# LiuZhu-CV/PAIF

Hardware: AMD Instinct MI355X
Metric: fused image-pairs/sec at 480x640 bs=8 per GPU (fusion-net forward) (higher is better)
Workload: dtype f16 (IEEE fp16 maps and conv weights, one fp16 MFMA per product, f32 accumulate; stems, guided filter and the last map fp32)

## Files before the change

### include/paif_hip.h

```cpp
#ifndef PAIF_HIP_H
#define PAIF_HIP_H

#include <stddef.h>
#include <stdint.h>

#ifdef __cplusplus
extern "C" {
#endif

#define PAIF_ABI_VERSION 1
#define PAIF_EINVAL (-1)
#define PAIF_ENOSUP (-2)

typedef void* paif_stream_t;

int paif_version(void);
const char* paif_last_error(void);
int paif_device_cus(void);


int paif_rgb2ycrcb_fwd(const float* rgb, float* ycc, int B, int H, int W, paif_stream_t stream);

int paif_ycrcb2rgb_fwd(const float* ycc, float* rgb, int B, int H, int W, paif_stream_t stream);

int paif_minmax_blocks(int B, int H, int W);
int paif_recompose_clamp_fwd(const float* fused, const float* ycc, float* rgb_out, float* minmax_partial,
                             int B, int H, int W, paif_stream_t stream);
int paif_fused_uint8_fwd(const float* rgb, const float* minmax_partial, int npartial, unsigned char* out, int B, int H, int W,
                         paif_stream_t stream);
int paif_minmax_normalize_fwd(const float* rgb, const float* minmax_partial, int npartial, float* out,
                              float* minmax_out, int B, int H, int W, paif_stream_t stream);


int paif_stem_fwd(const float* img, size_t img_bstride, const float* w, const float* prelu, float* feat, float* guide,
                  int B, int H, int W, paif_stream_t stream);
int paif_stem_fwd_twin(const float* img, size_t img_bstride, const float* w, const float* prelu, float* feat, float* feat_bf16,
                       float* guide, int B, int H, int W, paif_stream_t stream);
int paif_stem_fwd_twin_f16(const float* img, size_t img_bstride, const float* w, const float* prelu, float* feat, float* feat_f16,
                           float* guide, int B, int H, int W, paif_stream_t stream);
int paif_channel_residue_fwd(const float* x, float* guide, int B, int H, int W, paif_stream_t stream);

int paif_guided_filter_ab_fwd(const float* guide, const float* y, float* ab, float eps0, float eps1,
                              int B, int H, int W, paif_stream_t stream);
int paif_guided_filter_lf_fwd(const float* guide, const float* ab, float* lf, int B, int H, int W,
                              paif_stream_t stream);
int paif_guided_filter_taped_fits(int B, int H, int W);
int paif_guided_filter_taped_fwd(const float* guide, const float* y, float* mc, float* lf, float eps0, float eps1,
                                 float* workspace, int B, int H, int W, paif_stream_t stream);
size_t paif_guided_filter_fused_workspace_floats(int B, int H, int W);
int paif_guided_filter_fused_fwd(const float* guide, const float* y, float* lf, float eps0, float eps1, float* workspace,
                                 int B, int H, int W, paif_stream_t stream);
int paif_guided_filter_fused_fwd_bf16(const float* guide, const float* y, float* lf, float eps0, float eps1, float* workspace, int B,
                                      int H, int W, paif_stream_t stream);
int paif_guided_filter_fused_fwd_hf16(const float* guide, const float* y, float* hf, float eps0, float eps1, float* workspace, int B,
                                      int H, int W, paif_stream_t stream);

int paif_guided_filter_fused_fwd_hf16_y16(const float* guide, const float* y16, float* hf, float eps0, float eps1, float* workspace,
                                          int B, int H, int W, paif_stream_t stream);

typedef struct {
  const float* src[3];
  int nsrc;
  int cin;
  const float* wpk;
  int kh;
  int dil;
  int in_act;
  const float* in_prelu;
  const float* scale;
  const float* shift;
  int act;
  const float* prelu;
  float alpha;
  const float* res[3];
  float* out;
  int cout;
  float* pool_partial;
  int precision;
  float* aux_out;
  const float* in_aux;
  const float* in_scale;
  float in_alpha;
  const float* epi_aux;
  int epi_dact;
  int reverse_tiles;
  int storage;
  float* cpool;
} paif_conv_desc;
#define PAIF_ST_F32 0
#define PAIF_ST_BF16 1
#define PAIF_ST_F32_BF16 2
#define PAIF_ST_F16 3
#define PAIF_ST_F16_F32 4
#define PAIF_CONV_F32 0
#define PAIF_CONV_BF16X3 1
#define PAIF_CONV_BF16 2
#define PAIF_CONV_F16 4
#define PAIF_CONV_F16X2 5
#define PAIF_CONV_F16X3 6
#define PAIF_CONV_BF16X6 3

int paif_dwconv_fwd_bf16(const float* x, const float* w, float* out, int k, int dil, int in_relu, int B, int H, int W,
                         paif_stream_t stream);
int paif_channel_pool2_fwd_bf16(const float* ir, const float* vis, float* comp, int B, int H, int W, paif_stream_t stream);
int paif_spa_blend_fwd_bf16(const float* comp, const float* w, const float* ir, const float* vis, float* agg, int B, int H, int W,
                            paif_stream_t stream);
int paif_eca_finish_fwd_bf16(const float* o, const float* r, const float* pool_partial, const float* w1d, int k,
                             const float* prelu, float* gate, float* out, int B, int H, int W, paif_stream_t stream);
int paif_tail_fwd_bf16(const float* x, const float* w, const float* prelu, float* fused, int B, int H, int W, paif_stream_t stream);
int paif_add_fwd_bf16(const float* a, const float* b, float* out, size_t n, paif_stream_t stream);
int paif_cast_storage_fwd(const float* src, float* dst, size_t n, int mode, paif_stream_t stream);
int paif_dwconv_fwd_f16(const float* x, const float* w, float* out, int k, int dil, int in_relu, int B, int H, int W,
                        paif_stream_t stream);
int paif_channel_pool2_fwd_f16(const float* ir, const float* vis, float* comp, int B, int H, int W, paif_stream_t stream);
int paif_spa_blend_fwd_f16(const float* comp, const float* w, const float* ir, const float* vis, float* agg, int B, int H, int W,
                           paif_stream_t stream);
int paif_eca_finish_fwd_f16(const float* o, const float* r, const float* pool_partial, const float* w1d, int k,
                            const float* prelu, float* gate, float* out, int B, int H, int W, paif_stream_t stream);
int paif_tail_fwd_f16(const float* x, const float* w, const float* prelu, float* fused, int B, int H, int W, paif_stream_t stream);
int paif_add_fwd_f16(const float* a, const float* b, float* out, size_t n, paif_stream_t stream);

int paif_conv2d_blocks(int B, int H, int W);
int paif_conv2d_fwd(const paif_conv_desc* d, int B, int H, int W, paif_stream_t stream);
int paif_conv2d_can_cpool(const paif_conv_desc* d, int B, int H, int W);
int paif_channel_pool1_fwd(const float* x, float* comp_off, int B, int H, int W, paif_stream_t stream);
int paif_channel_pool1_fwd_bf16(const float* x, float* comp_off, int B, int H, int W, paif_stream_t stream);
int paif_channel_pool1_fwd_f16(const float* x, float* comp_off, int B, int H, int W, paif_stream_t stream);
int paif_conv2d_is_persistent(const paif_conv_desc* d, int B, int H, int W);
int paif_conv2d_kernel_name(const paif_conv_desc* d, int B, int H, int W, char* buf, int buflen);
size_t paif_conv_wpk_floats(int nsrc, int cin, int kh);
int paif_pack_conv_weight(const float* w, float* wpk, int cout, int nsrc, int cin, int kh, paif_stream_t stream);
int paif_pack_conv_weight_bf16x3(const float* w, float* wpk, int cout, int nsrc, int kh, paif_stream_t stream);
int paif_pack_conv_weight_f16x2(const float* w, float* wpk, int cout, int nsrc, int kh, paif_stream_t stream);
int paif_pack_conv_weight_bf16x6(const float* w, float* wpk, int cout, int nsrc, int kh, paif_stream_t stream);
int paif_compose_dw_pw_weight(const float* dw, const float* pw, float* out, int cout, int cin, int kh, paif_stream_t stream);
int paif_compose_pw_conv_weight(const float* pw, const float* w, float* out, int cout, int cmid, int cin, int kh, paif_stream_t stream);

size_t paif_rdb_fused_wpk_floats(void);
int paif_rdb_fused_pack(const float* w1, const float* w2, const float* w3, float* wpk, int f16, paif_stream_t stream);
int paif_rdb_fused_fwd(const float* x, const float* wpk, const float* prelu, float alpha, const float* res0, const float* res1, float* out,
                       float* cpool, int f16, int reverse_tiles, int B, int H, int W, paif_stream_t stream);

int paif_stem_out_pack_floats(void);
int paif_stem_out_pack(const float* w1, const float* w2, float* wpk, paif_stream_t stream);
int paif_stem_out_fwd_bf16(const float* x, const float* wpk, const float* prelu, float* fused, int B, int H, int W, paif_stream_t stream);
int paif_stem_out_fwd_f32(const float* x, const float* wpk, const float* prelu, float* fused, int B, int H, int W, paif_stream_t stream);
int paif_stem_out_fwd_guard(const float* x, int f32in, const float* wpk, const float* prelu, float* fused, unsigned* flag, int B, int H, int W,
                            paif_stream_t stream);
int paif_pack_decomp1x1_weight_bf16x6(const float* w, float* wpk, paif_stream_t stream);
int paif_pack_decomp1x1_weight_bf16x3(const float* w, float* wpk, paif_stream_t stream);
int paif_pack_decomp1x1_hf_weight_f16x2(const float* w, float* wpk, paif_stream_t stream);
int paif_pack_decomp1x1_weight(const float* w, float* wpk, paif_stream_t stream);
int paif_bn_fold(const float* gamma, const float* beta, const float* mean, const float* var, float eps,
                 float* scale, float* shift, int C, paif_stream_t stream);

int paif_dwconv_fwd(const float* x, const float* w, float* out, int k, int dil, int in_relu,
                    int B, int H, int W, paif_stream_t stream);

int paif_channel_pool2_fwd(const float* ir, const float* vis, float* comp, int B, int H, int W, paif_stream_t stream);
int paif_spa_blend_fwd(const float* comp, const float* w, const float* ir, const float* vis, float* agg,
                       float* scale_out, int B, int H, int W, paif_stream_t stream);

int paif_eca_finish_fwd(const float* o, const float* r, const float* pool_partial, const float* w1d, int k,
                        const float* prelu, float* gate , float* out,
                        float* u_out ,
                        int B, int H, int W, paif_stream_t stream);

int paif_tail_fwd(const float* x, const float* w, const float* prelu, float* fused,
                  float* z_out ,
                  int B, int H, int W, paif_stream_t stream);

int paif_add_fwd(const float* a, const float* b, float* out, size_t n, paif_stream_t stream);



int paif_gemm_fwd(const float* A, int lda, const float* W, const float* scale, const float* shift, int act,
                  const float* res, int ldres, float* C, int ldc, int M, int N, int K, int precision,
                  paif_stream_t stream);
int paif_gemm_splitk_plan(int M, int N, int K);
int paif_gemm_splitk_fwd(const float* A, int lda, const float* W, const float* scale, const float* shift, int act,
                         const float* res, int ldres, float* C, int ldc, int M, int N, int K, int splits,
                         float* workspace, paif_stream_t stream);
int paif_gemm_splitk_fwd_p(const float* A, int lda, const float* W, const float* scale, const float* shift, int act,
                         const float* res, int ldres, float* C, int ldc, int M, int N, int K, int splits,
                         float* workspace, int precision, paif_stream_t stream);

int paif_gemm_conv_fwd(const float* x, int B, int H, int W, int Cin, int k, int stride, int pad, const float* Wt,
                       const float* scale, const float* shift, int act, const float* res, int ldres, float* out, int ldc,
                       int N, int precision, int splits, float* workspace, paif_stream_t stream);

int paif_gemm_col2im_fwd(const float* dY, int lda, const float* Wt, float* dx, int B, int H, int W, int C, int sr, int K,
                         int precision, paif_stream_t stream);

int paif_timing_event_create(void** ev);
int paif_timing_event_record(void* ev, paif_stream_t stream);
int paif_timing_event_elapsed_ms(void* start, void* stop, float* ms);
int paif_timing_event_destroy(void* ev);

int paif_gemm2_plan(int M, int N, int K, int precision);
size_t paif_gemm2_packed_bytes(int N, int K, int precision);
int paif_gemm2_pack_weight(const float* W, void* out, int N, int K, int precision, paif_stream_t stream);
int paif_gemm2_fwd(const float* A, int lda, const void* W, const float* scale, const float* shift, int act,
                   const float* res, int ldres, float* C, int ldc, int M, int N, int K, int precision, int nt,
                   paif_stream_t stream);

int paif_layernorm_fwd(const float* x, const float* gamma, const float* beta, float* y, int M, int C, float eps,
                       paif_stream_t stream);

int paif_im2col_fwd(const float* x, float* col, int B, int H, int W, int Cin, int k, int stride, int pad, int Kpad,
                    paif_stream_t stream);
int paif_pack_conv_gemm_weight(const float* w, float* out, int Cout, int Cin, int k, int Kpad, paif_stream_t stream);

int paif_dwconv3_bias_gelu_fwd(const float* x, const float* w, const float* bias, float* y, int B, int H, int W, int C,
                               paif_stream_t stream);

int paif_sr_attention_fwd(const float* q, const float* kv, float* out, float* lse, int B, int N, int Nk, int C, int heads,
                          paif_stream_t stream);
int paif_sr_attention_split_fwd(const float* q, const float* kv, float* out, float* lse, int B, int N, int Nk, int C, int heads,
                                int precision, paif_stream_t stream);
int paif_sr_attention_bf16x3_fwd(const float* q, const float* kv, float* out, float* lse, int B, int N, int Nk, int C, int heads,
                          paif_stream_t stream);

int paif_resize_bilinear_into_fwd(const float* x, float* out, int B, int IH, int IW, int C, int OH, int OW, int ldo,
                                  int coff, paif_stream_t stream);

int paif_nhwc_to_nchw_fwd(const float* x, float* y, int B, int HW, int C, paif_stream_t stream);
int paif_nchw_to_nhwc_fwd(const float* x, float* y, int B, int HW, int C, paif_stream_t stream);
int paif_nchw_to_nhwc_pad_fwd(const float* x, float* y, int B, int HW, int C, int CP, paif_stream_t stream);


int paif_gemm_masked_fwd(const float* A, int lda, const float* a_mask, const float* a_scale, const float* W,
                         const float* scale, const float* shift, int act, const float* res, int ldres, float* C,
                         int ldc, int M, int N, int K, int precision, paif_stream_t stream);
int paif_transpose_pad_fwd(const float* w, float* wt, int N, int K, int Npad, paif_stream_t stream);

int paif_layernorm_bwd_input(const float* x, const float* gamma, const float* dy, const float* add, float* dx,
                             int M, int C, float eps, paif_stream_t stream);
int paif_dwconv3_bias_gelu_bwd_input(const float* x, const float* w, const float* bias, const float* dy, float* tmp,
                                     float* dx, int B, int H, int W, int C, paif_stream_t stream);
int paif_col2im_fwd(const float* dcol, float* dx, int B, int H, int W, int Cin, int k, int stride, int pad, int Kpad,
                    paif_stream_t stream);
int paif_resize_bilinear_adjoint_fwd(const float* dout, float* dx, int B, int IH, int IW, int C, int OH, int OW,
                                     int ldo, int coff, paif_stream_t stream);
int paif_sr_attention_bwd_chunks(int B, int N, int heads);
int paif_sr_attention_bwd_input(const float* q, const float* kv, const float* o, const float* dout, const float* lse,
                                float* delta, float* dq, float* dkv, float* dkv_partial, int B, int N, int Nk, int C,
                                int heads, paif_stream_t stream);
int paif_sr_attention_bwd_input_p(const float* q, const float* kv, const float* o, const float* dout, const float* lse,
                                float* delta, float* dq, float* dkv, float* dkv_partial, int B, int N, int Nk, int C,
                                int heads, int precision, paif_stream_t stream);

int paif_upsample_ce_blocks(int B, int OH, int OW);
int paif_upsample_ce_fwd(const float* logits, const long long* label, float* partial, float* loss_count, int B, int IH,
                         int IW, int C, int OH, int OW, int ignore_index, paif_stream_t stream);
int paif_upsample_ce_bwd(const float* logits, const long long* label, const float* gscale, float* dfull, int B, int IH,
                         int IW, int C, int OH, int OW, int ignore_index, int CP, paif_stream_t stream);

int paif_attack_loss_blocks(int B, int OH, int OW);
int paif_attack_loss_fwd(const float* logits, const long long* label, float* partial, float* coef, int way, float w_true,
                         float w_false, int B, int IH, int IW, int C, int OH, int OW, int ignore_index, paif_stream_t stream);
int paif_attack_loss_bwd(const float* logits, const long long* label, const float* coef, float* dfull, int way, float w_true,
                         float w_false, float upstream, int B, int IH, int IW, int C, int OH, int OW, int ignore_index, int CP,
                         paif_stream_t stream);

int paif_conv_weight_dgrad(const float* w, float* wt, int Co, int Ctot, int k, int coff, int cs, paif_stream_t stream);
int paif_fold_decomp1x1_weight(const float* w, float* wf, paif_stream_t stream);
int paif_tail_bwd_input(const float* dfused, const float* fused, const float* z, const float* w, const float* prelu,
                        float* dt16, int B, int H, int W, paif_stream_t stream);
int paif_stem_bwd_input(const float* dfeat, const float* feat, const float* w, const float* prelu, float* dimg,
                        int B, int H, int W, paif_stream_t stream);
int paif_dwconv_bwd_input(const float* dt, const float* w, const float* aux, const float* add, float* out, int k, int dil,
                          int B, int H, int W, paif_stream_t stream);
int paif_eca_bwd_blocks(int H, int W);
int paif_eca_bwd_input(const float* dout, const float* u, const float* o, const float* gate, const float* w1d, int k,
                       const float* prelu, float* partial, float* coef, float* d_o, float* d_r, int B, int H, int W,
                       paif_stream_t stream);
// ... 111 lines not shown
```

### paif_amd/_lib.py

```python
import ctypes
import os
from ctypes import POINTER, Structure, c_char_p, c_float, c_int, c_size_t, c_ulonglong, c_void_p

HERE = os.path.dirname(os.path.abspath(__file__))
LIB_PATH = os.environ.get("PAIF_LIB") or os.path.join(HERE, "lib", "libpaif_hip.so")

F = c_void_p


class ConvDesc(Structure):

    _fields_ = [
        ("src", F * 3), ("nsrc", c_int), ("cin", c_int), ("wpk", F), ("kh", c_int), ("dil", c_int),
        ("in_act", c_int), ("in_prelu", F), ("scale", F), ("shift", F), ("act", c_int), ("prelu", F),
        ("alpha", c_float), ("res", F * 3), ("out", F), ("cout", c_int), ("pool_partial", F),
        ("precision", c_int), ("aux_out", F), ("in_aux", F), ("in_scale", F), ("in_alpha", c_float), ("epi_aux", F),
        ("epi_dact", c_int), ("reverse_tiles", c_int), ("storage", c_int), ("cpool", F),
    ]


SIGNATURES = {
    "paif_version": (c_int, []),
    "paif_last_error": (c_char_p, []),
    "paif_device_cus": (c_int, []),
    "paif_rgb2ycrcb_fwd": (c_int, [F, F, c_int, c_int, c_int, F]),
    "paif_ycrcb2rgb_fwd": (c_int, [F, F, c_int, c_int, c_int, F]),
    "paif_minmax_blocks": (c_int, [c_int, c_int, c_int]),
    "paif_recompose_clamp_fwd": (c_int, [F, F, F, F, c_int, c_int, c_int, F]),
    "paif_fused_uint8_fwd": (c_int, [F, F, c_int, F, c_int, c_int, c_int, F]),
    "paif_minmax_normalize_fwd": (c_int, [F, F, c_int, F, F, c_int, c_int, c_int, F]),
    "paif_stem_fwd": (c_int, [F, c_size_t, F, F, F, F, c_int, c_int, c_int, F]),
    "paif_stem_fwd_twin": (c_int, [F, c_size_t, F, F, F, F, F, c_int, c_int, c_int, F]),
    "paif_stem_fwd_twin_f16": (c_int, [F, c_size_t, F, F, F, F, F, c_int, c_int, c_int, F]),
    "paif_channel_residue_fwd": (c_int, [F, F, c_int, c_int, c_int, F]),
    "paif_guided_filter_ab_fwd": (c_int, [F, F, F, c_float, c_float, c_int, c_int, c_int, F]),
    "paif_guided_filter_lf_fwd": (c_int, [F, F, F, c_int, c_int, c_int, F]),
    "paif_guided_filter_taped_fits": (c_int, [c_int, c_int, c_int]),
    "paif_guided_filter_taped_fwd": (c_int, [F, F, F, F, c_float, c_float, F, c_int, c_int, c_int, F]),
    "paif_guided_filter_fused_workspace_floats": (c_size_t, [c_int, c_int, c_int]),
    "paif_guided_filter_fused_fwd": (c_int, [F, F, F, c_float, c_float, F, c_int, c_int, c_int, F]),
    "paif_guided_filter_fused_fwd_bf16": (c_int, [F, F, F, c_float, c_float, F, c_int, c_int, c_int, F]),
    "paif_guided_filter_fused_fwd_hf16": (c_int, [F, F, F, c_float, c_float, F, c_int, c_int, c_int, F]),
    "paif_guided_filter_fused_fwd_hf16_y16": (c_int, [F, F, F, c_float, c_float, F, c_int, c_int, c_int, F]),
    "paif_conv2d_blocks": (c_int, [c_int, c_int, c_int]),
    "paif_conv2d_fwd": (c_int, [POINTER(ConvDesc), c_int, c_int, c_int, F]),
    "paif_conv2d_is_persistent": (c_int, [POINTER(ConvDesc), c_int, c_int, c_int]),
    "paif_conv2d_can_cpool": (c_int, [POINTER(ConvDesc), c_int, c_int, c_int]),
    "paif_rdb_fused_wpk_floats": (c_size_t, []),
    "paif_rdb_fused_pack": (c_int, [F, F, F, F, c_int, F]),
    "paif_rdb_fused_fwd": (c_int, [F, F, F, c_float, F, F, F, F, c_int, c_int, c_int, c_int, c_int, F]),
    "paif_channel_pool1_fwd": (c_int, [F, F, c_int, c_int, c_int, F]),
    "paif_channel_pool1_fwd_bf16": (c_int, [F, F, c_int, c_int, c_int, F]),
    "paif_channel_pool1_fwd_f16": (c_int, [F, F, c_int, c_int, c_int, F]),
    "paif_conv2d_kernel_name": (c_int, [POINTER(ConvDesc), c_int, c_int, c_int, c_char_p, c_int]),
    "paif_conv_wpk_floats": (c_size_t, [c_int, c_int, c_int]),
    "paif_pack_conv_weight": (c_int, [F, F, c_int, c_int, c_int, c_int, F]),
    "paif_pack_decomp1x1_weight": (c_int, [F, F, F]),
    "paif_pack_conv_weight_bf16x3": (c_int, [F, F, c_int, c_int, c_int, F]),
    "paif_pack_conv_weight_f16x2": (c_int, [F, F, c_int, c_int, c_int, F]),
    "paif_pack_conv_weight_bf16x6": (c_int, [F, F, c_int, c_int, c_int, F]),
    "paif_compose_dw_pw_weight": (c_int, [F, F, F, c_int, c_int, c_int, F]),
    "paif_compose_pw_conv_weight": (c_int, [F, F, F, c_int, c_int, c_int, c_int, F]),
    "paif_stem_out_pack_floats": (c_int, []),
    "paif_stem_out_pack": (c_int, [F, F, F, F]),
    "paif_stem_out_fwd_bf16": (c_int, [F, F, F, F, c_int, c_int, c_int, F]),
    "paif_stem_out_fwd_f32": (c_int, [F, F, F, F, c_int, c_int, c_int, F]),
    "paif_stem_out_fwd_guard": (c_int, [F, c_int, F, F, F, F, c_int, c_int, c_int, F]),
    "paif_pack_decomp1x1_weight_bf16x3": (c_int, [F, F, F]),
    "paif_pack_decomp1x1_hf_weight_f16x2": (c_int, [F, F, F]),
    "paif_pack_decomp1x1_weight_bf16x6": (c_int, [F, F, F]),
    "paif_bn_fold": (c_int, [F, F, F, F, c_float, F, F, c_int, F]),
    "paif_dwconv_fwd": (c_int, [F, F, F, c_int, c_int, c_int, c_int, c_int, c_int, F]),
    "paif_channel_pool2_fwd": (c_int, [F, F, F, c_int, c_int, c_int, F]),
    "paif_spa_blend_fwd": (c_int, [F, F, F, F, F, F, c_int, c_int, c_int, F]),
    "paif_eca_finish_fwd": (c_int, [F, F, F, F, c_int, F, F, F, F, c_int, c_int, c_int, F]),
    "paif_tail_fwd": (c_int, [F, F, F, F, F, c_int, c_int, c_int, F]),
    "paif_add_fwd": (c_int, [F, F, F, c_size_t, F]),
    "paif_gemm_fwd": (c_int, [F, c_int, F, F, F, c_int, F, c_int, F, c_int, c_int, c_int, c_int, c_int, F]),
    "paif_gemm_splitk_plan": (c_int, [c_int, c_int, c_int]),
    "paif_gemm_conv_fwd": (c_int, [F, c_int, c_int, c_int, c_int, c_int, c_int, c_int, F, F, F, c_int, F, c_int, F, c_int, c_int, c_int, c_int, F, F]),
    "paif_gemm_col2im_fwd": (c_int, [F, c_int, F, F, c_int, c_int, c_int, c_int, c_int, c_int, c_int, F]),
    "paif_timing_event_create": (c_int, [POINTER(c_void_p)]),
    "paif_timing_event_record": (c_int, [c_void_p, F]),
    "paif_timing_event_elapsed_ms": (c_int, [c_void_p, c_void_p, POINTER(c_float)]),
    "paif_timing_event_destroy": (c_int, [c_void_p]),
    "paif_gemm2_plan": (c_int, [c_int, c_int, c_int, c_int]),
    "paif_gemm2_packed_bytes": (c_size_t, [c_int, c_int, c_int]),
    "paif_gemm2_pack_weight": (c_int, [F, F, c_int, c_int, c_int, F]),
    "paif_gemm2_fwd": (c_int, [F, c_int, F, F, F, c_int, F, c_int, F, c_int, c_int, c_int, c_int, c_int, c_int, F]),
    "paif_conv2d_wgrad_workspace_floats": (c_size_t, [c_int, c_int, c_int, c_int]),
    "paif_conv2d_wgrad": (c_int, [POINTER(c_void_p), c_int, F, F, F, F, c_int, c_float, c_int, c_int, F, F, c_int, c_int, c_int, c_int, c_int, F]),
    "paif_gemm_wgrad_splits": (c_int, [c_int, c_int, c_int]),
    "paif_gemm_wgrad": (c_int, [F, c_int, F, c_int, F, F, c_int, c_int, c_int, c_int, F, c_int, F]),
    "paif_gemm_wgrad_p": (c_int, [F, c_int, F, c_int, F, F, c_int, c_int, c_int, c_int, F, c_int, c_int, c_float, F]),
    "paif_layernorm_wgrad_blocks": (c_int, [c_int]),
    "paif_layernorm_wgrad": (c_int, [F, F, F, F, F, c_int, c_int, c_float, c_int, F]),
    "paif_channel_affine_nchw_fwd": (c_int, [F, F, F, F, c_int, c_int, c_int, c_int, F]),
    "paif_image_loss_blocks": (c_int, []),
    "paif_image_loss_fwd": (c_int, [F, F, c_int, c_int, c_int, c_int, c_int, c_int, F, F, F]),
    "paif_image_loss_bwd": (c_int, [F, F, c_int, c_int, c_int, c_int, c_int, c_int, c_float, F, F]),
    "paif_ssim_l1_blocks": (c_int, [c_int, c_int, c_int]),
    "paif_ssim_l1_fwd": (c_int, [F, F, F, F, F, c_int, c_int, c_int, F]),
    "paif_ssim_l1_bwd_input": (c_int, [F, F, F, F, F, F, c_int, c_int, c_int, F]),
    "paif_gemm_splitk_fwd": (c_int, [F, c_int, F, F, F, c_int, F, c_int, F, c_int, c_int, c_int, c_int, c_int, F, F]),
    "paif_gemm_splitk_fwd_p": (c_int, [F, c_int, F, F, F, c_int, F, c_int, F, c_int, c_int, c_int, c_int, c_int, F, c_int, F]),
    "paif_layernorm_fwd": (c_int, [F, F, F, F, c_int, c_int, c_float, F]),
    "paif_im2col_fwd": (c_int, [F, F, c_int, c_int, c_int, c_int, c_int, c_int, c_int, c_int, F]),
    "paif_pack_conv_gemm_weight": (c_int, [F, F, c_int, c_int, c_int, c_int, F]),
    "paif_dwconv3_bias_gelu_fwd": (c_int, [F, F, F, F, c_int, c_int, c_int, c_int, F]),
    "paif_sr_attention_fwd": (c_int, [F, F, F, F, c_int, c_int, c_int, c_int, c_int, F]),
    "paif_sr_attention_bf16x3_fwd": (c_int, [F, F, F, F, c_int, c_int, c_int, c_int, c_int, F]),
    "paif_sr_attention_split_fwd": (c_int, [F, F, F, F, c_int, c_int, c_int, c_int, c_int, c_int, F]),
    "paif_resize_bilinear_into_fwd": (c_int, [F, F, c_int, c_int, c_int, c_int, c_int, c_int, c_int, c_int, F]),
    "paif_nhwc_to_nchw_fwd": (c_int, [F, F, c_int, c_int, c_int, F]),
    "paif_nchw_to_nhwc_fwd": (c_int, [F, F, c_int, c_int, c_int, F]),
    "paif_nchw_to_nhwc_pad_fwd": (c_int, [F, F, c_int, c_int, c_int, c_int, F]),
    "paif_gemm_masked_fwd": (c_int, [F, c_int, F, F, F, F, F, c_int, F, c_int, F, c_int, c_int, c_int, c_int, c_int, F]),
    "paif_transpose_pad_fwd": (c_int, [F, F, c_int, c_int, c_int, F]),
    "paif_layernorm_bwd_input": (c_int, [F, F, F, F, F, c_int, c_int, c_float, F]),
    "paif_dwconv3_bias_gelu_bwd_input": (c_int, [F, F, F, F, F, F, c_int, c_int, c_int, c_int, F]),
    "paif_col2im_fwd": (c_int, [F, F, c_int, c_int, c_int, c_int, c_int, c_int, c_int, c_int, F]),
    "paif_resize_bilinear_adjoint_fwd": (c_int, [F, F, c_int, c_int, c_int, c_int, c_int, c_int, c_int, c_int, F]),
    "paif_sr_attention_bwd_chunks": (c_int, [c_int, c_int, c_int]),
    "paif_sr_attention_bwd_input": (c_int, [F, F, F, F, F, F, F, F, F, c_int, c_int, c_int, c_int, c_int, F]),
    "paif_sr_attention_bwd_input_p": (c_int, [F, F, F, F, F, F, F, F, F, c_int, c_int, c_int, c_int, c_int, c_int, F]),
    "paif_upsample_ce_blocks": (c_int, [c_int, c_int, c_int]),
    "paif_upsample_ce_fwd": (c_int, [F, F, F, F, c_int, c_int, c_int, c_int, c_int, c_int, c_int, F]),
    "paif_dwconv_fwd_bf16": (c_int, [F, F, F, c_int, c_int, c_int, c_int, c_int, c_int, F]),
    "paif_channel_pool2_fwd_bf16": (c_int, [F, F, F, c_int, c_int, c_int, F]),
    "paif_spa_blend_fwd_bf16": (c_int, [F, F, F, F, F, c_int, c_int, c_int, F]),
    "paif_eca_finish_fwd_bf16": (c_int, [F, F, F, F, c_int, F, F, F, c_int, c_int, c_int, F]),
    "paif_tail_fwd_bf16": (c_int, [F, F, F, F, c_int, c_int, c_int, F]),
    "paif_add_fwd_bf16": (c_int, [F, F, F, c_size_t, F]),
    "paif_dwconv_fwd_f16": (c_int, [F, F, F, c_int, c_int, c_int, c_int, c_int, c_int, F]),
    "paif_channel_pool2_fwd_f16": (c_int, [F, F, F, c_int, c_int, c_int, F]),
    "paif_spa_blend_fwd_f16": (c_int, [F, F, F, F, F, c_int, c_int, c_int, F]),
    "paif_eca_finish_fwd_f16": (c_int, [F, F, F, F, c_int, F, F, F, c_int, c_int, c_int, F]),
    "paif_tail_fwd_f16": (c_int, [F, F, F, F, c_int, c_int, c_int, F]),
    "paif_add_fwd_f16": (c_int, [F, F, F, c_size_t, F]),
    "paif_cast_storage_fwd": (c_int, [F, F, c_size_t, c_int, F]),
    "paif_attack_loss_blocks": (c_int, [c_int, c_int, c_int]),
    "paif_attack_loss_fwd": (c_int, [F, F, F, F, c_int, c_float, c_float, c_int, c_int, c_int, c_int, c_int, c_int, c_int, F]),
    "paif_attack_loss_bwd": (c_int, [F, F, F, F, c_int, c_float, c_float, c_float, c_int, c_int, c_int, c_int, c_int, c_int, c_int, c_int, F]),
    "paif_conv_weight_dgrad": (c_int, [F, F, c_int, c_int, c_int, c_int, c_int, F]),
    "paif_fold_decomp1x1_weight": (c_int, [F, F, F]),
    "paif_tail_bwd_input": (c_int, [F, F, F, F, F, F, c_int, c_int, c_int, F]),
    "paif_stem_bwd_input": (c_int, [F, F, F, F, F, c_int, c_int, c_int, F]),
    "paif_dwconv_bwd_input": (c_int, [F, F, F, F, F, c_int, c_int, c_int, c_int, c_int, F]),
    "paif_eca_bwd_blocks": (c_int, [c_int, c_int]),
    "paif_eca_bwd_input": (c_int, [F, F, F, F, F, c_int, F, F, F, F, F, c_int, c_int, c_int, F]),
    "paif_spa_blend_bwd_input": (c_int, [F, F, F, F, F, F, F, F, F, F, c_int, c_int, c_int, F]),
    "paif_guided_filter_bwd_input": (c_int, [F, F, F, F, c_float, c_float, F, F, F, F, F, F, c_int, c_int, c_int, F]),
    "paif_guided_filter_bwd_input_mc": (c_int, [F, F, F, F, F, F, F, F, F, F, c_int, c_int, c_int, F]),
    "paif_upsample_argmax_fwd": (c_int, [F, F, c_int, c_int, c_int, c_int, c_int, c_int, F]),
    "paif_confusion_matrix_accum": (c_int, [F, F, F, c_size_t, c_int, F]),
    "paif_spa1_fwd": (c_int, [F, F, F, c_int, F, F, F, F, F, c_int, c_int, c_int, F]),
    "paif_spa1_bwd_input": (c_int, [F, F, F, F, F, c_int, F, F, F, F, c_int, c_int, c_int, F]),
    "paif_glue_bwd_blocks": (c_int, [c_int, c_int, c_int]),
    "paif_glue_bwd_input": (c_int, [F, F, F, F, F, F, F, F, c_int, c_int, c_int, F]),
    "paif_plane_minmax_blocks": (c_int, [c_size_t]),
    "paif_plane_clamp_minmax_fwd": (c_int, [F, F, F, F, c_size_t, F]),
    "paif_plane_clamp_minmax_bwd_input": (c_int, [F, F, F, F, F, c_size_t, F]),
    "paif_channel_sum_chunks_fwd": (c_int, [F, F, c_int, c_int, c_int, c_int, F]),
    "paif_rgb2ycrcb_bwd_input": (c_int, [F, F, F, c_int, c_int, c_int, F]),
    "paif_pgd_step": (c_int, [F, F, F, c_float, c_float, c_size_t, F]),
    "paif_axpy": (c_int, [F, F, c_float, c_size_t, F]),
    "paif_upsample_ce_bwd": (c_int, [F, F, F, F, c_int, c_int, c_int, c_int, c_int, c_int, c_int, c_int, F]),
    "paif_head_sum_fwd": (c_int, [F, F, F, F, POINTER(c_int), F, F, F, c_int, c_int, F]),
    "paif_relu_mask_scale_fwd": (c_int, [F, F, F, F, c_size_t, c_int, F]),
    "paif_u8_to_planes_fwd": (c_int, [F, F, c_int, c_int, c_int, F]),
    "paif_u8_to_i64_fwd": (c_int, [F, F, c_size_t, F]),
    "paif_nhwc_slice_to_nchw_fwd": (c_int, [F, F, c_int, c_int, c_int, c_int, F]),
    "paif_pad_channels_fwd": (c_int, [F, F, c_size_t, c_int, c_int, F]),
    "paif_decomp_cat_fwd": (c_int, [F, F, F, F, c_size_t, F]),
    "paif_row_reduce_workspace_floats": (c_size_t, [c_int, c_int, c_int]),
    "paif_bn_stats_fwd": (c_int, [F, c_int, c_int, F, F, c_float, c_float, F, F, F, F, F, F, F, F]),
    "paif_affine_act_res_fwd": (c_int, [F, F, F, c_int, F, F, F, F, F, c_size_t, c_int, F]),
    "paif_bn_act_bwd": (c_int, [F, F, F, F, F, F, c_int, F, F, F, F, F, F, F, c_int, c_int, c_int, F]),
    "paif_bn_eval_stats": (c_int, [F, F, F, F, c_float, c_int, F, F, F, F, F]),
    "paif_prelu_bwd": (c_int, [F, F, F, F, c_float, F, F, F, c_size_t, F]),
    "paif_tail_dz": (c_int, [F, F, F, F, F, F, F, c_size_t, F]),
    "paif_colsum": (c_int, [F, c_int, F, F, c_int, c_int, F]),
    "paif_dwconv_wgrad": (c_int, [F, F, F, F, F, c_int, c_int, c_int, c_int, c_int, c_int, c_int, F]),
    "paif_stem_wgrad": (c_int, [F, c_size_t, F, F, F, F, F, F, c_int, c_int, c_int, F]),
    "paif_corr1_wgrad": (c_int, [F, F, F, F, c_int, c_int, c_int, c_int, c_int, F]),
    "paif_eca_wgrad": (c_int, [F, F, c_int, F, c_int, F, F, c_int, c_int, c_int, F]),
    "paif_unfold_decomp1x1_wgrad": (c_int, [F, F, F]),
    "paif_unpack_conv_gemm_wgrad": (c_int, [F, F, c_int, c_int, c_int, c_int, F]),
    "paif_keep_mask": (c_int, [F, c_int, c_ulonglong, c_ulonglong, c_float, F]),
    "paif_rowscale_add_fwd": (c_int, [F, F, F, F, c_int, c_size_t, c_int, c_int, F]),
    "paif_adamw_step": (c_int, [F, F, F, F, F, c_size_t, c_int, POINTER(c_float), POINTER(c_float), c_float, c_float, c_float, c_float,
                                c_float, F]),
}

_lib = None


class PaifLibraryError(RuntimeError):
# ... 29 lines not shown
```

### paif_amd/csrc/conv_dma.h

```cpp
#pragma once
#include <hip/hip_runtime.h>

namespace paif_conv_dma {

struct Args {
  const void* src[3];
  const void* res[3];
  const void* wpk;
  const float* scale;
  const float* shift;
  const float* prelu;
  void* out;
  float alpha;
  int nsrc, nres, act, kh;
  int cout;
  int B, H, W, reverse;
  float* cpool;
  int f16;
  int dil;
  int in_relu;
};

bool eligible(int nsrc, int nres, int B, int H, int W, float alpha);
bool eligible16(int nsrc, int nres, int B, int H, int W, float alpha);
bool eligible7(int nsrc, int nres, int B, int H, int W, float alpha);
bool eligible_d2(int nsrc, int nres, int B, int H, int W, float alpha);
bool can_cpool(int nsrc, int nres, int kh, int cout, int dil);
int launch(const Args& a, hipStream_t st);

}
```

### paif_amd/csrc/conv_dma.hip

```cpp
#include <stdint.h>
#include <stdlib.h>

#include <type_traits>

#include "conv_dma.h"
#include "paif_common.h"

namespace paif_conv_dma {
namespace {

typedef float f32x16 __attribute__((ext_vector_type(16)));
typedef unsigned u32x4 __attribute__((ext_vector_type(4)));
constexpr int TW = 32, TH = 8;
#ifndef CD_PF
#define CD_PF 4
#endif
#ifndef CD_ST_AUX
#define CD_ST_AUX 2
#endif
#ifndef CD_EXP
#define CD_EXP 0
#endif
constexpr int PARK_WAVE = 2 * 32 * 32 * 4;
template <int DIL>
struct Geo {
  static constexpr int TWH = TW + 2 * DIL, THH = TH + 2 * DIL;
  static constexpr int NPIX = TWH * THH;
  static constexpr int DPW = (NPIX * 4 + 255) / 256;
  static constexpr int SLOT = 4 * DPW * 1024;
  static constexpr int PF = DIL == 1 ? CD_PF : 3;
  static constexpr int NSLOT = PF + 1;
  static constexpr int ROWB = TWH * 64;
  static constexpr int PARK_OFF = NSLOT * SLOT;
  static constexpr int LDS_BYTES = PARK_OFF + 4 * PARK_WAVE;
  static_assert(LDS_BYTES <= 160 * 1024, "ring + transposition buffers exceed LDS");
  static_assert(4 * DPW * 64 >= NPIX * 4, "DMA instructions do not cover the halo tile");
  static __device__ __forceinline__ int base_row(int w) { return DIL == 1 ? 2 * w : (w >> 1) * 4 + (w & 1); }
};
constexpr unsigned RSRC_W3 = 0x00020000u;
constexpr unsigned OOB = 0x80000000u;
constexpr int NSTORE = 4;
constexpr int VMCAP = 63;

#define CD_VMWAIT(n) asm volatile("s_waitcnt vmcnt(%0)" ::"n"((n) > VMCAP ? VMCAP : (n)) : "memory")
#define CD_RD128(dst, addr, off) asm volatile("ds_read_b128 %0, %1 offset:%2" : "=v"(dst) : "v"(addr), "n"(off) : "memory")
#define CD_WR32(addr, val, off) asm volatile("ds_write_b32 %0, %1 offset:%2" ::"v"(addr), "v"(val), "n"(off) : "memory")

__device__ __forceinline__ void dma16(__amdgpu_buffer_rsrc_t rsrc, unsigned voff, unsigned lds_off) {
  __builtin_amdgcn_raw_ptr_buffer_load_lds(rsrc, (__attribute__((address_space(3))) void*)(uintptr_t)lds_off, 16, voff, 0, 0, 0);
}

template <int NSRC, int NRES, int PF, int DPW>
struct Sched {
  static constexpr int RL = 4 * NRES;
  static constexpr int smod(int x) { return ((x % NSRC) + NSRC) % NSRC; }
  static constexpr int R_STAGE = smod(1 - PF);
  static constexpr int D = (R_STAGE + PF - 1 - NSRC) / NSRC;
  static constexpr int U = D + (R_STAGE == 0 ? 2 : 1);
  static_assert(PF >= 2 && D >= 0 && U <= 4, "prefetch distance out of the range the tile loop lists");
  static constexpr int n1 = DPW * (PF - 1);
};

template <int NSRC, int NRES, int F, bool CP = false, int DIL = 1, int IA = 0>
__global__ __launch_bounds__(256, 1) void conv3x3_h16_dma(Args a, int ntiles, int tilesX, int tilesY) {
  typedef Geo<DIL> G;
  constexpr int TWH = G::TWH, NPIX = G::NPIX, DPW = G::DPW, SLOT = G::SLOT, PF = G::PF, NSLOT = G::NSLOT, ROWB = G::ROWB, PARK_OFF = G::PARK_OFF;
  typedef Sched<NSRC, NRES, PF, DPW> SC;
  constexpr int U = SC::U, D = SC::D;
  __shared__ __attribute__((aligned(16))) unsigned char smem[G::LDS_BYTES];
  asm volatile("" ::"v"((unsigned)(uintptr_t)(__attribute__((address_space(3))) unsigned char*)smem) : "memory");

  const int tid = threadIdx.x, l = tid & 63;
  const int w = __builtin_amdgcn_readfirstlane(tid >> 6);
  const int p = l & 31, hh = l >> 5;
  const int wb = G::base_row(w);

  const int xcd = blockIdx.x & 7, wg = blockIdx.x >> 3, nwg = gridDim.x >> 3;
  const int tpx = (ntiles + 7) >> 3;
  const int t_beg = xcd * tpx, t_end = min(ntiles, t_beg + tpx);
  const int cnt = t_beg + wg < t_end ? (t_end - t_beg - wg + nwg - 1) / nwg : 0;
  if (cnt == 0) return;
  const int H = a.H, W = a.W;
  auto pack_tile = [&](int k) -> unsigned {
    const int pos = wg + min(k, cnt - 1) * nwg;
    int t = a.reverse ? t_end - 1 - pos : t_beg + pos;
    const int tx = t % tilesX;
    t /= tilesX;
    const int ty = t % tilesY;
    return ((unsigned)(t / tilesY) << 22) | ((unsigned)ty << 11) | (unsigned)tx;
  };
  const unsigned tab0 = pack_tile(l), tab1 = pack_tile(l + 64);
  auto tile_of = [&](int k, int& b, int& y0, int& x0) -> bool {
    const bool ok = k >= 0 && k < cnt;
    const int kk = ok ? k : 0;
    const unsigned lo = __builtin_amdgcn_readlane(tab0, kk & 63), hi = __builtin_amdgcn_readlane(tab1, kk & 63);
    const unsigned pk = kk < 64 ? lo : hi;
    b = pk >> 22; y0 = ((pk >> 11) & 2047) * TH; x0 = (pk & 2047) * TW;
    return ok;
  };

  const int map_bytes = a.B * H * W * 64;
  __amdgpu_buffer_rsrc_t rs_src[NSRC];
#pragma unroll
  for (int s = 0; s < NSRC; ++s) rs_src[s] = __builtin_amdgcn_make_buffer_rsrc(const_cast<void*>(a.src[s]), 0, map_bytes, RSRC_W3);
  __amdgpu_buffer_rsrc_t rs_res[NRES > 0 ? NRES : 1];
#pragma unroll
  for (int r = 0; r < NRES; ++r) rs_res[r] = __builtin_amdgcn_make_buffer_rsrc(const_cast<void*>(a.res[r]), 0, map_bytes, RSRC_W3);
  const int opitch = a.cout * 2;
  const __amdgpu_buffer_rsrc_t rs_out = __builtin_amdgcn_make_buffer_rsrc(a.out, 0, a.B * H * W * opitch, RSRC_W3);
  const __amdgpu_buffer_rsrc_t rs_null = __builtin_amdgcn_make_buffer_rsrc(a.out, 0, 0, RSRC_W3);
  const __amdgpu_buffer_rsrc_t rs_cp = __builtin_amdgcn_make_buffer_rsrc(CP ? (void*)a.cpool : a.out, 0, CP ? a.B * H * W * 16 - 8 : 0, RSRC_W3);

  u32x4 bw[NSRC][9][2];
  {
    const __amdgpu_buffer_rsrc_t rs_w = __builtin_amdgcn_make_buffer_rsrc(const_cast<void*>(a.wpk), 0, NSRC * 9 * 2 * 2 * 1024, RSRC_W3);
#pragma unroll
    for (int s = 0; s < NSRC; ++s)
#pragma unroll
      for (int tap = 0; tap < 9; ++tap)
#pragma unroll
        for (int ks = 0; ks < 2; ++ks)
          bw[s][tap][ks] = __builtin_amdgcn_raw_buffer_load_b128(rs_w, (unsigned)l * 16u, (((s * 9 + tap) * 2 + ks) * 2) * 1024, 0);
  }
  float esc[8], esh[8];
#pragma unroll
  for (int j = 0; j < 8; ++j) {
    const int c = 8 * (l & 3) + j;
    esc[j] = ((a.scale && c < a.cout) ? a.scale[c] : 1.f) * a.alpha;
    esh[j] = ((a.shift && c < a.cout) ? a.shift[c] : 0.f) * a.alpha;
  }
  const float e_slope = a.act == 1 ? *a.prelu : (a.act == 2 ? 0.f : 1.f);

  int d_rel[DPW];
  int d_rc[DPW];
#pragma unroll
  for (int i = 0; i < DPW; ++i) {
    const int n = (w * DPW + i) * 64 + l;
    const int pi = n >> 2;
    const int r = pi / TWH, c = pi - r * TWH;
    d_rel[i] = (r * W + c) * 64 + (((n & 3) ^ ((c >> 2) & 3)) * 16);
    d_rc[i] = pi < NPIX ? (r | (c << 8)) : -1;
  }
  unsigned d_voff[DPW];
  auto target = [&](int k) {
    int b, y0, x0;
    const bool ok = tile_of(k, b, y0, x0);
    const int org = ((b * H + y0 - DIL) * W + x0 - DIL) * 64;
#pragma unroll
    for (int i = 0; i < DPW; ++i) {
      const int gy = y0 - DIL + (d_rc[i] & 0xff), gx = x0 - DIL + (d_rc[i] >> 8);
      const bool in = !(CD_EXP & 4) && ok && d_rc[i] >= 0 && (unsigned)gy < (unsigned)H && (unsigned)gx < (unsigned)W;
      d_voff[i] = in ? (unsigned)(org + d_rel[i]) : OOB;
    }
  };
  unsigned a_rd[3][2];
#pragma unroll
  for (int dx = 0; dx < 3; ++dx)
#pragma unroll
    for (int ks = 0; ks < 2; ++ks) {
      const int c = p + dx * DIL;
      a_rd[dx][ks] = (unsigned)(wb * ROWB + c * 64 + (((2 * ks + hh) ^ ((c >> 2) & 3)) * 16));
    }
  const unsigned a_pw = PARK_OFF + w * PARK_WAVE + (4 * hh * 32 + p) * 4;
  const unsigned a_pr = PARK_OFF + w * PARK_WAVE + (l >> 2) * 128 + (l & 3) * 32;
  const unsigned e_lane = (unsigned)l * 16u;
  const unsigned o_lane = 8 * (l & 3) < a.cout ? (unsigned)((l >> 2) * opitch + (l & 3) * 16) : OOB;

  u32x4 rr[U][NRES > 0 ? NRES : 1][4];
  auto issue_res = [&](auto settag, int k) {
    constexpr int SET = decltype(settag)::value;
    int b, y0, x0;
    const bool ok = tile_of(k, b, y0, x0);
#pragma unroll
    for (int it = 0; it < 4; ++it) {
      const int y = y0 + wb + (it >> 1) * DIL, x = x0 + (it & 1) * 16 + (l >> 2);
      const bool in = ok && y < H && x < W;
      const unsigned soff = (unsigned)(((b * H + y) * W + x0 + (it & 1) * 16) * 64);
#pragma unroll
      for (int r = 0; r < NRES; ++r) rr[SET][r][it] = __builtin_amdgcn_raw_buffer_load_b128(rs_res[r], in ? e_lane : OOB, soff, 0);
    }
  };

  auto relu_frag = [](u32x4& f) {
    typedef short s16x8 __attribute__((ext_vector_type(8)));
    const s16x8 z = {0, 0, 0, 0, 0, 0, 0, 0};
    f = __builtin_bit_cast(u32x4, __builtin_elementwise_max(__builtin_bit_cast(s16x8, f), z));
  };
  f32x16 acc[2];
  u32x4 t[4][2];
#pragma unroll
  for (int it = 0; it < 4; ++it) t[it][0] = t[it][1] = u32x4{0, 0, 0, 0};
  float ev[8];
  float pmx = 0.f, psm = 0.f;
  int cur = NSLOT - PF;

  auto epi = [&](auto mtag, auto settag, bool pok, int pb, int py0, int px0) {
    constexpr int M = decltype(mtag)::value, SETP = decltype(settag)::value;
    constexpr int it = M / 9, j = M % 9;
    if constexpr (j < 8) {
      const unsigned raw = j < 4 ? t[it][0][j & 3] : t[it][1][j & 3];
      float v = __builtin_fmaf(__uint_as_float(raw), esc[j], esh[j]);
      v = __builtin_fmaf(e_slope, fminf(v, 0.f), fmaxf(v, 0.f));
#pragma unroll
      for (int r = 0; r < NRES; ++r) {
        const unsigned u = rr[SETP][r][it][j >> 1];
        if constexpr (F == 2) v += (float)__builtin_bit_cast(paif::f16x2_t, u)[j & 1];
        else v += __uint_as_float((j & 1) ? (u & 0xffff0000u) : (u << 16));
      }
      ev[j] = v;
      if constexpr (CP) {
        pmx = j == 0 ? v : fmaxf(pmx, v);
        psm = j == 0 ? v : psm + v;
      }
    } else {
      const uint2 o0 = paif::f32_to_h4<F>(make_float4(ev[0], ev[1], ev[2], ev[3]));
      const uint2 o1 = paif::f32_to_h4<F>(make_float4(ev[4], ev[5], ev[6], ev[7]));
      const int y = py0 + wb + (it >> 1) * DIL, x = px0 + (it & 1) * 16 + (l >> 2);
      const unsigned soff = (unsigned)(((pb * H + y) * W + px0 + (it & 1) * 16) * opitch);
      u32x4 od = {o0.x, o0.y, o1.x, o1.y};
      __builtin_amdgcn_raw_buffer_store_b128(od, rs_out, (!(CD_EXP & 1) && pok && y < H && x < W) ? o_lane : OOB, soff, CD_ST_AUX);
      asm volatile("s_nop 2" : "+v"(od));
      if constexpr (CP) {
        float mx = pmx, sm = psm;
        mx = fmaxf(mx, paif::dpp_f<0xB1>(mx)); sm += paif::dpp_f<0xB1>(sm);
        mx = fmaxf(mx, paif::dpp_f<0x4E>(mx)); sm += paif::dpp_f<0x4E>(sm);
        typedef float f32x2v __attribute__((ext_vector_type(2)));
        const f32x2v pv = {mx, sm * (1.0f / 32.0f)};
        const unsigned poff = (unsigned)(((pb * H + y) * W + px0 + (it & 1) * 16) * 16);
        __builtin_amdgcn_raw_buffer_store_b64(__builtin_bit_cast(unsigned __attribute__((ext_vector_type(2))), pv), rs_cp,
                                              (pok && y < H && x < W && (l & 3) == 0) ? (unsigned)((l >> 2) * 16) : OOB, poff, 0);
      }
    }
  };

  auto stage = [&](auto ktag, auto stag, auto virt, int k) {
    constexpr int K = decltype(ktag)::value, S = decltype(stag)::value;
    constexpr bool VIRT = decltype(virt)::value;
    constexpr int SETP = (K + U - 1) % U;
    const unsigned sb = (unsigned)cur * SLOT;
    const int fill = cur == 0 ? NSLOT - 1 : cur - 1;
    u32x4 A[2][4];
    unsigned ad[3][2];
    if constexpr (!VIRT) {
      CD_VMWAIT(SC::n1);
      asm volatile("s_barrier" ::: "memory");
#pragma unroll
      for (int dx = 0; dx < 3; ++dx)
#pragma unroll
        for (int ks = 0; ks < 2; ++ks) ad[dx][ks] = a_rd[dx][ks] + sb;
      if constexpr (S == 0) {
#pragma unroll
        for (int it = 0; it < 4; ++it) {
          CD_RD128(t[it][0], a_pr, it * 2048);
          CD_RD128(t[it][1], a_pr, it * 2048 + 16);
        }
      }
#pragma unroll
      for (int r = 0; r < 4; ++r) CD_RD128(A[0][r], ad[0][0], r * DIL * ROWB);
    }
    if constexpr (NRES > 0 && S == SC::R_STAGE) issue_res(std::integral_constant<int, (K + D) % U>{}, k + D);
    asm volatile("" ::: "memory");
    if constexpr ((S + PF) % NSRC == 0) target(k + (S + PF) / NSRC);
#pragma unroll
    for (int i = 0; i < DPW; ++i) dma16(rs_src[(S + PF) % NSRC], d_voff[i], (unsigned)(fill * SLOT + (w * DPW + i) * 1024));
    if constexpr (VIRT) {
      if constexpr (S == 0) {
#pragma unroll
        for (int it = 0; it < NSTORE; ++it) __builtin_amdgcn_raw_buffer_store_b128(u32x4{0, 0, 0, 0}, rs_null, 0, 0, 0);
      }
    } else {
      int pb = 0, py0 = 0, px0 = 0;
      bool pok = false;
      if constexpr (S == 0) pok = tile_of(k - 1, pb, py0, px0);
      auto mma = [&](auto gitag, auto dytag, auto jtag) {
        constexpr int gi = decltype(gitag)::value, dy = decltype(dytag)::value, j = decltype(jtag)::value;
        constexpr int ks = gi / 3, dx = gi % 3;
        if constexpr (!((CD_EXP & 2) && (dy > 0 || j > 0))) {
          const u32x4 av = A[gi & 1][j + dy], bv = bw[S][dy * 3 + dx][ks];
          if constexpr (S == 0 && gi == 0 && dy == 0) {
            const f32x16 z = {0.f, 0.f, 0.f, 0.f, 0.f, 0.f, 0.f, 0.f, 0.f, 0.f, 0.f, 0.f, 0.f, 0.f, 0.f, 0.f};
            acc[j] = paif::mfma16<F>(av, bv, z);
          } else {
            acc[j] = paif::mfma16<F>(av, bv, acc[j]);
          }
        }
        if constexpr (S == 0) epi(std::integral_constant<int, gi * 6 + dy * 2 + j>{}, std::integral_constant<int, SETP>{}, pok, pb, py0, px0);
        if constexpr (IA == 2) {
          constexpr int call = dy * 2 + j;
          if constexpr (call == 0) relu_frag(A[gi & 1][1]);
          if constexpr (call == 2) relu_frag(A[gi & 1][2]);
          if constexpr (call == 4) relu_frag(A[gi & 1][3]);
        }
        __builtin_amdgcn_sched_barrier(0);
      };
      auto group = [&](auto gitag) {
        constexpr int gi = decltype(gitag)::value;
        if constexpr (gi + 1 < 6) {
          constexpr int ks1 = (gi + 1) / 3, dx1 = (gi + 1) % 3;
#pragma unroll
          for (int r = 0; r < 4; ++r) CD_RD128(A[(gi + 1) & 1][r], ad[dx1][ks1], r * DIL * ROWB);
        }
        if constexpr (S == 0 && gi == 0) {
          asm volatile("s_waitcnt lgkmcnt(4)"
                       : "+v"(A[0][0]), "+v"(A[0][1]), "+v"(A[0][2]), "+v"(A[0][3]), "+v"(t[0][0]), "+v"(t[0][1]), "+v"(t[1][0]), "+v"(t[1][1]),
                         "+v"(t[2][0]), "+v"(t[2][1]), "+v"(t[3][0]), "+v"(t[3][1])::"memory");
        } else if constexpr (gi + 1 < 6) {
          asm volatile("s_waitcnt lgkmcnt(4)" : "+v"(A[gi & 1][0]), "+v"(A[gi & 1][1]), "+v"(A[gi & 1][2]), "+v"(A[gi & 1][3])::"memory");
        } else {
          asm volatile("s_waitcnt lgkmcnt(0)" : "+v"(A[gi & 1][0]), "+v"(A[gi & 1][1]), "+v"(A[gi & 1][2]), "+v"(A[gi & 1][3])::"memory");
        }
        if constexpr (IA == 2) relu_frag(A[gi & 1][0]);
        __builtin_amdgcn_sched_barrier(0);
        typedef std::integral_constant<int, 0> I0;
        typedef std::integral_constant<int, 1> I1;
        typedef std::integral_constant<int, 2> I2;
        mma(gitag, I0{}, I0{}); mma(gitag, I0{}, I1{});
        mma(gitag, I1{}, I0{}); mma(gitag, I1{}, I1{});
        mma(gitag, I2{}, I0{}); mma(gitag, I2{}, I1{});
      };
      group(std::integral_constant<int, 0>{});
      group(std::integral_constant<int, 1>{});
      group(std::integral_constant<int, 2>{});
      group(std::integral_constant<int, 3>{});
      group(std::integral_constant<int, 4>{});
      group(std::integral_constant<int, 5>{});
      if constexpr (S == NSRC - 1) {
        asm volatile("s_nop 15\n\ts_nop 7" ::: "memory");
#pragma unroll
        for (int j = 0; j < 2; ++j)
#pragma unroll
          for (int r = 0; r < 16; ++r) {
            const float v = acc[j][r];
            CD_WR32(a_pw, v, (j * 32 + (r & 3) + 8 * (r >> 2)) * 128);
          }
      }
    }
    cur = cur == NSLOT - 1 ? 0 : cur + 1;
  };
  auto drain = [&](auto ktag, int k) {
    constexpr int K = decltype(ktag)::value;
#pragma unroll
    for (int it = 0; it < 4; ++it) {
      CD_RD128(t[it][0], a_pr, it * 2048);
      CD_RD128(t[it][1], a_pr, it * 2048 + 16);
    }
    asm volatile("s_waitcnt lgkmcnt(0)"
                 : "+v"(t[0][0]), "+v"(t[0][1]), "+v"(t[1][0]), "+v"(t[1][1]), "+v"(t[2][0]), "+v"(t[2][1]), "+v"(t[3][0]), "+v"(t[3][1])::"memory");
    int pb, py0, px0;
    const bool pok = tile_of(k, pb, py0, px0);
#define CD_M(m) epi(std::integral_constant<int, m>{}, std::integral_constant<int, K>{}, pok, pb, py0, px0);
    CD_M(0) CD_M(1) CD_M(2) CD_M(3) CD_M(4) CD_M(5) CD_M(6) CD_M(7) CD_M(8) CD_M(9) CD_M(10) CD_M(11)
    CD_M(12) CD_M(13) CD_M(14) CD_M(15) CD_M(16) CD_M(17) CD_M(18) CD_M(19) CD_M(20) CD_M(21) CD_M(22) CD_M(23)
    CD_M(24) CD_M(25) CD_M(26) CD_M(27) CD_M(28) CD_M(29) CD_M(30) CD_M(31) CD_M(32) CD_M(33) CD_M(34) CD_M(35)
#undef CD_M
  };

  auto vstage = [&](auto jtag) {
    constexpr int J = decltype(jtag)::value;
    constexpr int T = (J - (NSRC - 1)) / NSRC;
    constexpr int S = J - T * NSRC;
    constexpr int K = ((T % U) + U) % U;
    stage(std::integral_constant<int, K>{}, std::integral_constant<int, S>{}, std::true_type{}, T);
  };
  static_assert(PF >= 1 && PF <= 4, "the prologue lists up to 4 virtual stages");
  if constexpr (PF >= 4) vstage(std::integral_constant<int, -4>{});
  if constexpr (PF >= 3) vstage(std::integral_constant<int, -3>{});
  if constexpr (PF >= 2) vstage(std::integral_constant<int, -2>{});
  vstage(std::integral_constant<int, -1>{});

  auto tile_step = [&](auto ktag, int k) {
    stage(ktag, std::integral_constant<int, 0>{}, std::false_type{}, k);
    if constexpr (NSRC > 1) stage(ktag, std::integral_constant<int, 1>{}, std::false_type{}, k);
    if constexpr (NSRC > 2) stage(ktag, std::integral_constant<int, 2>{}, std::false_type{}, k);
  };
  for (int k = 0;; k += U) {
    tile_step(std::integral_constant<int, 0>{}, k);
    if (k + 1 >= cnt) { drain(std::integral_constant<int, 0>{}, k); break; }
    if constexpr (U > 1) {
      tile_step(std::integral_constant<int, 1 % U>{}, k + 1);
      if (k + 2 >= cnt) { drain(std::integral_constant<int, 1 % U>{}, k + 1); break; }
    }
    if constexpr (U > 2) {
      tile_step(std::integral_constant<int, 2 % U>{}, k + 2);
      if (k + 3 >= cnt) { drain(std::integral_constant<int, 2 % U>{}, k + 2); break; }
    }
    if constexpr (U > 3) {
      tile_step(std::integral_constant<int, 3 % U>{}, k + 3);
      if (k + 4 >= cnt) { drain(std::integral_constant<int, 3 % U>{}, k + 3); break; }
    }
  }
  CD_VMWAIT(0);
}

namespace k7 {
constexpr int P = 3;
constexpr int TWH = TW + 2 * P, THH = TH + 2 * P;
constexpr int NPIX = TWH * THH;
constexpr int DPW = 9;
constexpr int SLOT = 4 * DPW * 1024;
constexpr int NSLOT = 2;
constexpr int ROWB = TWH * 64;
constexpr int WB_OFF = NSLOT * SLOT;
constexpr int WB_BYTES = 49 * 1024;
constexpr int PARK_OFF = WB_OFF + WB_BYTES;
constexpr int LDS_BYTES = PARK_OFF + 4 * PARK_WAVE;
static_assert(LDS_BYTES <= 160 * 1024, "7x7: ring + weights + transposition buffers exceed LDS");
static_assert(4 * DPW * 64 >= NPIX * 4, "7x7: DMA instructions do not cover the halo tile");
}

#define CD_WR128(addr, val, off) asm volatile("ds_write_b128 %0, %1 offset:%2" ::"v"(addr), "v"(val), "n"(off) : "memory")

template <int F>
__global__ __launch_bounds__(256, 1) void conv7x7_h16_dma(Args a, int ntiles, int tilesX, int tilesY) {
  constexpr int P = k7::P, TWH = k7::TWH, NPIX = k7::NPIX, DPW = k7::DPW, SLOT = k7::SLOT, ROWB = k7::ROWB, WB_OFF = k7::WB_OFF,
                PARK_OFF = k7::PARK_OFF;
  __shared__ __attribute__((aligned(16))) unsigned char smem[k7::LDS_BYTES];
  asm volatile("" ::"v"((unsigned)(uintptr_t)(__attribute__((address_space(3))) unsigned char*)smem) : "memory");

  const int tid = threadIdx.x, l = tid & 63;
  const int w = __builtin_amdgcn_readfirstlane(tid >> 6);
  const int p = l & 31, hh = l >> 5;
  const int xcd = blockIdx.x & 7, wg = blockIdx.x >> 3, nwg = gridDim.x >> 3;
  const int tpx = (ntiles + 7) >> 3;
  const int t_beg = xcd * tpx, t_end = min(ntiles, t_beg + tpx);
  const int cnt = t_beg + wg < t_end ? (t_end - t_beg - wg + nwg - 1) / nwg : 0;
  if (cnt == 0) return;
  const int H = a.H, W = a.W;
  auto pack_tile = [&](int k) -> unsigned {
    const int pos = wg + min(k, cnt - 1) * nwg;
    int t = a.reverse ? t_end - 1 - pos : t_beg + pos;
    const int tx = t % tilesX;
    t /= tilesX;
    const int ty = t % tilesY;
    return ((unsigned)(t / tilesY) << 22) | ((unsigned)ty << 11) | (unsigned)tx;
  };
  const unsigned tab0 = pack_tile(l), tab1 = pack_tile(l + 64);
  auto tile_of = [&](int k, int& b, int& y0, int& x0) -> bool {
    const bool ok = k >= 0 && k < cnt;
    const int kk = ok ? k : 0;
    const unsigned lo = __builtin_amdgcn_readlane(tab0, kk & 63), hi = __builtin_amdgcn_readlane(tab1, kk & 63);
    const unsigned pk = kk < 64 ? lo : hi;
    b = pk >> 22; y0 = ((pk >> 11) & 2047) * TH; x0 = (pk & 2047) * TW;
    return ok;
  };
  const int map_bytes = a.B * H * W * 64;
  const __amdgpu_buffer_rsrc_t rs_src = __builtin_amdgcn_make_buffer_rsrc(const_cast<void*>(a.src[0]), 0, map_bytes, RSRC_W3);
  const __amdgpu_buffer_rsrc_t rs_out = __builtin_amdgcn_make_buffer_rsrc(a.out, 0, map_bytes, RSRC_W3);
  const __amdgpu_buffer_rsrc_t rs_w = __builtin_amdgcn_make_buffer_rsrc(const_cast<void*>(a.wpk), 0, 49 * 2 * 2 * 1024, RSRC_W3);

  u32x4 bw0[49];
#pragma unroll
  for (int tap = 0; tap < 49; ++tap) bw0[tap] = __builtin_amdgcn_raw_buffer_load_b128(rs_w, (unsigned)l * 16u, ((tap * 2 + 0) * 2) * 1024, 0);
#pragma unroll 1
  for (int i = tid; i < 49 * 64; i += 256) {
    const int tap = i >> 6, ln = i & 63;
    const u32x4 v = __builtin_amdgcn_raw_buffer_load_b128(rs_w, (unsigned)ln * 16u, ((tap * 2 + 1) * 2) * 1024, 0);
    const unsigned dst = WB_OFF + (unsigned)i * 16u;
    CD_WR128(dst, v, 0);
  }
  float esc[8], esh[8];
#pragma unroll
  for (int j = 0; j < 8; ++j) {
    const int c = 8 * (l & 3) + j;
    esc[j] = (a.scale ? a.scale[c] : 1.f) * a.alpha;
    esh[j] = (a.shift ? a.shift[c] : 0.f) * a.alpha;
  }
  const float e_slope = a.act == 1 ? *a.prelu : (a.act == 2 ? 0.f : 1.f);

  int d_rel[DPW], d_rc[DPW];
#pragma unroll
  for (int i = 0; i < DPW; ++i) {
    const int n = (w * DPW + i) * 64 + l;
    const int pi = n >> 2;
    const int r = pi / TWH, c = pi - r * TWH;
    d_rel[i] = (r * W + c) * 64 + (((n & 3) ^ ((c >> 2) & 3)) * 16);
    d_rc[i] = pi < NPIX ? (r | (c << 8)) : -1;
  }
  unsigned d_voff[DPW];
  auto target = [&](int k) {
    int b, y0, x0;
    const bool ok = tile_of(k, b, y0, x0);
    const int org = ((b * H + y0 - P) * W + x0 - P) * 64;
#pragma unroll
    for (int i = 0; i < DPW; ++i) {
      const int gy = y0 - P + (d_rc[i] & 0xff), gx = x0 - P + (d_rc[i] >> 8);
      const bool in = ok && d_rc[i] >= 0 && (unsigned)gy < (unsigned)H && (unsigned)gx < (unsigned)W;
      d_voff[i] = in ? (unsigned)(org + d_rel[i]) : OOB;
    }
  };
  unsigned a_rd[7][2];
#pragma unroll
  for (int dx = 0; dx < 7; ++dx)
#pragma unroll
    for (int ks = 0; ks < 2; ++ks) {
      const int c = p + dx;
      a_rd[dx][ks] = (unsigned)(2 * w * ROWB + c * 64 + (((2 * ks + hh) ^ ((c >> 2) & 3)) * 16));
    }
  const unsigned a_wb = WB_OFF + (unsigned)l * 16u;
  const unsigned a_pw = PARK_OFF + w * PARK_WAVE + (4 * hh * 32 + p) * 4;
  const unsigned a_pr = PARK_OFF + w * PARK_WAVE + (l >> 2) * 128 + (l & 3) * 32;
  const unsigned e_lane = (unsigned)l * 16u;

  f32x16 acc[2];
  u32x4 t[4][2];
#pragma unroll
  for (int it = 0; it < 4; ++it) t[it][0] = t[it][1] = u32x4{0, 0, 0, 0};
  float ev[8];
  auto epi = [&](auto mtag, bool pok, int pb, int py0, int px0) {
    constexpr int M = decltype(mtag)::value;
    constexpr int it = M / 9, j = M % 9;
    if constexpr (j < 8) {
      const unsigned raw = j < 4 ? t[it][0][j & 3] : t[it][1][j & 3];
      float v = __builtin_fmaf(__uint_as_float(raw), esc[j], esh[j]);
      ev[j] = __builtin_fmaf(e_slope, fminf(v, 0.f), fmaxf(v, 0.f));
    } else {
      const uint2 o0 = paif::f32_to_h4<F>(make_float4(ev[0], ev[1], ev[2], ev[3]));
      const uint2 o1 = paif::f32_to_h4<F>(make_float4(ev[4], ev[5], ev[6], ev[7]));
      const int y = py0 + 2 * w + (it >> 1), x = px0 + (it & 1) * 16 + (l >> 2);
      const unsigned soff = (unsigned)(((pb * H + y) * W + px0 + (it & 1) * 16) * 64);
      u32x4 od = {o0.x, o0.y, o1.x, o1.y};
      __builtin_amdgcn_raw_buffer_store_b128(od, rs_out, (pok && y < H && x < W) ? e_lane : OOB, soff, CD_ST_AUX);
      asm volatile("s_nop 2" : "+v"(od));
    }
  };

  asm volatile("s_waitcnt lgkmcnt(0)" ::: "memory");
  target(0);
#pragma unroll
  for (int i = 0; i < DPW; ++i) dma16(rs_src, d_voff[i], (unsigned)((w * DPW + i) * 1024));
  int cur = 0;
  for (int k = 0; k < cnt; ++k) {
    const unsigned sb = (unsigned)cur * SLOT;
    CD_VMWAIT(0);
    asm volatile("s_barrier" ::: "memory");
    unsigned ad[7][2];
#pragma unroll
    for (int dx = 0; dx < 7; ++dx)
#pragma unroll
      for (int ks = 0; ks < 2; ++ks) ad[dx][ks] = a_rd[dx][ks] + sb;
    u32x4 A[2][8], BL[7];
#pragma unroll
    for (int it = 0; it < 4; ++it) {
      CD_RD128(t[it][0], a_pr, it * 2048);
      CD_RD128(t[it][1], a_pr, it * 2048 + 16);
    }
#pragma unroll
    for (int r = 0; r < 8; ++r) CD_RD128(A[0][r], ad[0][0], r * ROWB);
    target(k + 1);
#pragma unroll
    for (int i = 0; i < DPW; ++i) dma16(rs_src, d_voff[i], (unsigned)((cur ^ 1) * SLOT + (w * DPW + i) * 1024));
    int pb, py0, px0;
    const bool pok = tile_of(k - 1, pb, py0, px0);
    auto mma = [&](auto gitag, auto dytag, auto jtag) {
      constexpr int gi = decltype(gitag)::value, dy = decltype(dytag)::value, j = decltype(jtag)::value;
      constexpr int dx = gi >> 1, ks = gi & 1;
      const u32x4 av = A[gi & 1][j + dy];
      const u32x4 bv = ks == 0 ? bw0[dy * 7 + dx] : BL[dy];
      if constexpr (gi == 0 && dy == 0) {
        const f32x16 z = {0.f, 0.f, 0.f, 0.f, 0.f, 0.f, 0.f, 0.f, 0.f, 0.f, 0.f, 0.f, 0.f, 0.f, 0.f, 0.f};
        acc[j] = paif::mfma16<F>(av, bv, z);
      } else {
        acc[j] = paif::mfma16<F>(av, bv, acc[j]);
      }
      constexpr int m = gi * 14 + dy * 2 + j;
      if constexpr (m < 36) epi(std::integral_constant<int, m>{}, pok, pb, py0, px0);
      __builtin_amdgcn_sched_barrier(0);
    };
    auto group = [&](auto gitag) {
      constexpr int gi = decltype(gitag)::value;
      if constexpr (gi + 1 < 14) {
        constexpr int dx1 = (gi + 1) >> 1, ks1 = (gi + 1) & 1;
#pragma unroll
        for (int r = 0; r < 8; ++r) CD_RD128(A[(gi + 1) & 1][r], ad[dx1][ks1], r * ROWB);
        if constexpr (ks1 == 1) {
#pragma unroll
          for (int dy = 0; dy < 7; ++dy) CD_RD128(BL[dy], a_wb, (dy * 7 + dx1) * 1024);
        }
      }
      if constexpr (gi == 0) {
        asm volatile("s_waitcnt lgkmcnt(15)"
                     : "+v"(A[0][0]), "+v"(A[0][1]), "+v"(A[0][2]), "+v"(A[0][3]), "+v"(A[0][4]), "+v"(A[0][5]), "+v"(A[0][6]), "+v"(A[0][7]),
                       "+v"(t[0][0]), "+v"(t[0][1]), "+v"(t[1][0]), "+v"(t[1][1]), "+v"(t[2][0]), "+v"(t[2][1]), "+v"(t[3][0])::"memory");
        asm volatile("" : "+v"(t[3][1])::"memory");
      } else if constexpr (gi + 1 >= 14) {
        asm volatile("s_waitcnt lgkmcnt(0)"
                     : "+v"(A[1][0]), "+v"(A[1][1]), "+v"(A[1][2]), "+v"(A[1][3]), "+v"(A[1][4]), "+v"(A[1][5]), "+v"(A[1][6]), "+v"(A[1][7]),
                       "+v"(BL[0]), "+v"(BL[1]), "+v"(BL[2]), "+v"(BL[3]), "+v"(BL[4]), "+v"(BL[5]), "+v"(BL[6])::"memory");
      } else if constexpr ((gi & 1) == 1) {
        asm volatile("s_waitcnt lgkmcnt(8)"
                     : "+v"(A[1][0]), "+v"(A[1][1]), "+v"(A[1][2]), "+v"(A[1][3]), "+v"(A[1][4]), "+v"(A[1][5]), "+v"(A[1][6]), "+v"(A[1][7]),
                       "+v"(BL[0]), "+v"(BL[1]), "+v"(BL[2]), "+v"(BL[3]), "+v"(BL[4]), "+v"(BL[5]), "+v"(BL[6])::"memory");
      } else {
        asm volatile("s_waitcnt lgkmcnt(15)"
                     : "+v"(A[0][0]), "+v"(A[0][1]), "+v"(A[0][2]), "+v"(A[0][3]), "+v"(A[0][4]), "+v"(A[0][5]), "+v"(A[0][6]), "+v"(A[0][7])::"memory");
      }
      __builtin_amdgcn_sched_barrier(0);
      typedef std::integral_constant<int, 0> J0;
      typedef std::integral_constant<int, 1> J1;
#define CD_DY(d) mma(gitag, std::integral_constant<int, d>{}, J0{}); mma(gitag, std::integral_constant<int, d>{}, J1{});
      CD_DY(0) CD_DY(1) CD_DY(2) CD_DY(3) CD_DY(4) CD_DY(5) CD_DY(6)
#undef CD_DY
    };
#define CD_G(g) group(std::integral_constant<int, g>{});
    CD_G(0) CD_G(1) CD_G(2) CD_G(3) CD_G(4) CD_G(5) CD_G(6) CD_G(7) CD_G(8) CD_G(9) CD_G(10) CD_G(11) CD_G(12) CD_G(13)
#undef CD_G
    asm volatile("s_nop 15\n\ts_nop 7" ::: "memory");
#pragma unroll
    for (int j = 0; j < 2; ++j)
#pragma unroll
      for (int r = 0; r < 16; ++r) {
        const float v = acc[j][r];
        CD_WR32(a_pw, v, (j * 32 + (r & 3) + 8 * (r >> 2)) * 128);
      }
    cur ^= 1;
  }
  {
#pragma unroll
    for (int it = 0; it < 4; ++it) {
      CD_RD128(t[it][0], a_pr, it * 2048);
      CD_RD128(t[it][1], a_pr, it * 2048 + 16);
    }
    asm volatile("s_waitcnt lgkmcnt(0)"
                 : "+v"(t[0][0]), "+v"(t[0][1]), "+v"(t[1][0]), "+v"(t[1][1]), "+v"(t[2][0]), "+v"(t[2][1]), "+v"(t[3][0]), "+v"(t[3][1])::"memory");
    int pb, py0, px0;
    const bool pok = tile_of(cnt - 1, pb, py0, px0);
#define CD_M(m) epi(std::integral_constant<int, m>{}, pok, pb, py0, px0);
    CD_M(0) CD_M(1) CD_M(2) CD_M(3) CD_M(4) CD_M(5) CD_M(6) CD_M(7) CD_M(8) CD_M(9) CD_M(10) CD_M(11)
    CD_M(12) CD_M(13) CD_M(14) CD_M(15) CD_M(16) CD_M(17) CD_M(18) CD_M(19) CD_M(20) CD_M(21) CD_M(22) CD_M(23)
    CD_M(24) CD_M(25) CD_M(26) CD_M(27) CD_M(28) CD_M(29) CD_M(30) CD_M(31) CD_M(32) CD_M(33) CD_M(34) CD_M(35)
#undef CD_M
  }
  CD_VMWAIT(0);
}

int launch_7(const Args& a, hipStream_t st) {
  const int tilesX = (a.W + TW - 1) / TW, tilesY = (a.H + TH - 1) / TH;
  if (a.f16) hipLaunchKernelGGL(conv7x7_h16_dma<2>, dim3(256), dim3(256), 0, st, a, a.B * tilesX * tilesY, tilesX, tilesY);
  else hipLaunchKernelGGL(conv7x7_h16_dma<1>, dim3(256), dim3(256), 0, st, a, a.B * tilesX * tilesY, tilesX, tilesY);
  hipError_t e = hipGetLastError();
  if (e != hipSuccess) {
    paif::set_error("conv2d(bf16 dma 7x7): launch failed: %s", hipGetErrorString(e));
    return (int)e;
  }
  return 0;
}

template <int NSRC, int NRES>
int launch_n(const Args& a, hipStream_t st) {
  const int tilesX = (a.W + TW - 1) / TW, tilesY = (a.H + TH - 1) / TH;
  if (a.cpool) {
    if constexpr (NSRC == 3 && (NRES == 1 || NRES == 3)) {
      if (a.f16) hipLaunchKernelGGL((conv3x3_h16_dma<NSRC, NRES, 2, true>), dim3(256), dim3(256), 0, st, a, a.B * tilesX * tilesY, tilesX, tilesY);
      else hipLaunchKernelGGL((conv3x3_h16_dma<NSRC, NRES, 1, true>), dim3(256), dim3(256), 0, st, a, a.B * tilesX * tilesY, tilesX, tilesY);
    } else {
      paif::set_error("conv2d(dma): the fused ChannelPool is built for 3 sources with 1 or 3 residual maps");
      return PAIF_ENOSUP;
    }
  } else if (a.f16) hipLaunchKernelGGL((conv3x3_h16_dma<NSRC, NRES, 2>), dim3(256), dim3(256), 0, st, a, a.B * tilesX * tilesY, tilesX, tilesY);
  else hipLaunchKernelGGL((conv3x3_h16_dma<NSRC, NRES, 1>), dim3(256), dim3(256), 0, st, a, a.B * tilesX * tilesY, tilesX, tilesY);
  hipError_t e = hipGetLastError();
  if (e != hipSuccess) {
    paif::set_error("conv2d(h16 dma): launch failed: %s", hipGetErrorString(e));
    return (int)e;
  }
  return 0;
}

template <int NRES, bool CP>
int launch_d2(const Args& a, hipStream_t st) {
  const int tilesX = (a.W + TW - 1) / TW, tilesY = (a.H + TH - 1) / TH;
  if (a.f16) hipLaunchKernelGGL((conv3x3_h16_dma<1, NRES, 2, CP, 2, 2>), dim3(256), dim3(256), 0, st, a, a.B * tilesX * tilesY, tilesX, tilesY);
  else hipLaunchKernelGGL((conv3x3_h16_dma<1, NRES, 1, CP, 2, 2>), dim3(256), dim3(256), 0, st, a, a.B * tilesX * tilesY, tilesX, tilesY);
  hipError_t e = hipGetLastError();
  if (e != hipSuccess) {
    paif::set_error("conv2d(h16 dma, dilation 2): launch failed: %s", hipGetErrorString(e));
    return (int)e;
  }
  return 0;
}

}

bool eligible(int nsrc, int nres, int B, int H, int W, float alpha) {
  static const bool on = [] {
    const char* e = getenv("PAIF_CONV_DMA");
    return !(e && e[0] == '0');
  }();
  if (!on || nsrc < 1 || nsrc > 3 || nres < 0 || nres > 3 || !(alpha > 0.f)) return false;
  if (nsrc == 1 && nres > 1) return false;
  const long long tiles = (long long)B * ((H + TH - 1) / TH) * ((W + TW - 1) / TW);
  return tiles >= 1024 && tiles <= 128 * 256 && B < 1024 && H < 2048 * TH && W < 2048 * TW && (long long)B * H * W * 64 < (1ll << 31);
}

bool eligible_d2(int nsrc, int nres, int B, int H, int W, float alpha) {
  static const bool on = [] {
    const char* e = getenv("PAIF_CONV_DMA_D2");
    return !(e && e[0] == '0');
  }();
  return on && nsrc == 1 && (nres == 1 || nres == 3) && eligible(1, 1, B, H, W, alpha);
}

bool eligible16(int nsrc, int nres, int B, int H, int W, float alpha) { return nsrc == 1 && nres == 0 && eligible(1, 0, B, H, W, alpha); }
bool eligible7(int nsrc, int nres, int B, int H, int W, float alpha) { return nsrc == 1 && nres == 0 && eligible(1, 0, B, H, W, alpha); }

bool can_cpool(int nsrc, int nres, int kh, int cout, int dil) {
  return kh == 3 && cout == 32 && ((dil == 1 && nsrc == 3 && (nres == 1 || nres == 3)) || (dil == 2 && nsrc == 1 && (nres == 1 || nres == 3)));
}

int launch(const Args& a, hipStream_t st) {
  if (a.cpool && !can_cpool(a.nsrc, a.nres, a.kh, a.cout, a.dil)) {
    paif::set_error("conv2d(dma): no fused ChannelPool for this form");
    return PAIF_ENOSUP;
  }
  if (a.kh == 7) return launch_7(a, st);
  if (a.dil == 2) {
    if (a.nsrc == 1 && a.in_relu && a.nres == 1) return a.cpool ? launch_d2<1, true>(a, st) : launch_d2<1, false>(a, st);
    if (a.nsrc == 1 && a.in_relu && a.nres == 3) return a.cpool ? launch_d2<3, true>(a, st) : launch_d2<3, false>(a, st);
    paif::set_error("conv2d(h16 dma): dilation 2 is built for one source behind an input ReLU with 1 or 3 residual maps");
    return PAIF_ENOSUP;
  }
  if (a.in_relu) {
    paif::set_error("conv2d(h16 dma): the input ReLU is built for the dilation-2 form");
    return PAIF_ENOSUP;
  }
  switch (a.nsrc * 10 + a.nres) {
    case 10: return launch_n<1, 0>(a, st);
    case 11: return launch_n<1, 1>(a, st);
    case 20: return launch_n<2, 0>(a, st);
    case 21: return launch_n<2, 1>(a, st);
    case 22: return launch_n<2, 2>(a, st);
    case 23: return launch_n<2, 3>(a, st);
    case 30: return launch_n<3, 0>(a, st);
    case 31: return launch_n<3, 1>(a, st);
    case 32: return launch_n<3, 2>(a, st);
    case 33: return launch_n<3, 3>(a, st);
    default: break;
  }
  paif::set_error("conv2d(bf16 dma): %d sources / %d residual maps not built", a.nsrc, a.nres);
  return PAIF_ENOSUP;
}

}
```

### paif_amd/csrc/conv_mfma.hip

```cpp
#include <stdlib.h>

#include "conv_dma.h"
#include "paif_common.h"
#include <type_traits>

#ifndef PAIF_UB_HOOKS
#define PAIF_UB_HOOKS 3
#endif
#ifndef PAIF_UB
#define PAIF_UB 11
#endif

namespace {

typedef float f32x16 __attribute__((ext_vector_type(16)));

#ifndef PAIF_TH
#define PAIF_TH 8
#endif
constexpr int TH = PAIF_TH;
constexpr int TW = 32;
constexpr int NTHREADS = 256;
constexpr int SEGS_PER_WAVE = TH / 4;

struct ConvArgs {
  const float* src[3];
  const float* res[3];
  const float4* wpk;
  const float* in_prelu;
  const float* scale;
  const float* shift;
  const float* prelu;
  float* out;
  float* pool_partial;
  float* cpool;
  float* aux_out;
  const float* in_aux;
  const float* in_scale;
  const float* epi_aux;
  float alpha, in_alpha;
  int nsrc, in_act, act, cout, epi_dact;
  int B, H, W, tilesX, tilesY, nblk;
  int reverse;
  int st;
  int wl0;
};

template <bool HOOKS>
__device__ __forceinline__ float4 stage_xform(const ConvArgs& a, float4 v, float4 aux, float slope, int q) {
  if (a.in_act == 0) return v;
  if (a.in_act == 1) {
    v.x = paif::prelu_f(v.x, slope); v.y = paif::prelu_f(v.y, slope);
    v.z = paif::prelu_f(v.z, slope); v.w = paif::prelu_f(v.w, slope);
    return v;
  }
  if (a.in_act == 2) {
    v.x = fmaxf(v.x, 0.f); v.y = fmaxf(v.y, 0.f); v.z = fmaxf(v.z, 0.f); v.w = fmaxf(v.w, 0.f);
    return v;
  }
  if (!HOOKS) return v;
  float4 f = make_float4(a.in_alpha, a.in_alpha, a.in_alpha, a.in_alpha);
  if (a.in_scale) {
    const float4 s4 = *reinterpret_cast<const float4*>(a.in_scale + q * 4);
    f.x *= s4.x; f.y *= s4.y; f.z *= s4.z; f.w *= s4.w;
  }
  if (a.in_act == 3) {
    f.x *= aux.x >= 0.f ? 1.f : slope; f.y *= aux.y >= 0.f ? 1.f : slope;
    f.z *= aux.z >= 0.f ? 1.f : slope; f.w *= aux.w >= 0.f ? 1.f : slope;
  } else if (a.in_act == 4) {
    f.x *= aux.x > 0.f ? 1.f : 0.f; f.y *= aux.y > 0.f ? 1.f : 0.f;
    f.z *= aux.z > 0.f ? 1.f : 0.f; f.w *= aux.w > 0.f ? 1.f : 0.f;
  }
  return make_float4(v.x * f.x, v.y * f.y, v.z * f.z, v.w * f.w);
}

struct EpiParams {
  float4 sc, sh;
  float slope;
};
__device__ const float k_ones[32] = {1.f, 1.f, 1.f, 1.f, 1.f, 1.f, 1.f, 1.f, 1.f, 1.f, 1.f, 1.f, 1.f, 1.f, 1.f, 1.f,
                                     1.f, 1.f, 1.f, 1.f, 1.f, 1.f, 1.f, 1.f, 1.f, 1.f, 1.f, 1.f, 1.f, 1.f, 1.f, 1.f};
__device__ const float k_zeros[32] = {};

template <bool HOOKS>
__device__ __forceinline__ EpiParams load_epi_params(const ConvArgs& a, int lane) {
  const int q = lane & 7;
  EpiParams e;
  const bool want_slope = a.act == 1 || (HOOKS && a.epi_dact == 1);
  const float* pp = want_slope ? a.prelu : k_zeros;
  if (a.cout == 32) {
    const float* sp = a.scale ? a.scale : k_ones;
    const float* hp = a.shift ? a.shift : k_zeros;
    e.sc = *reinterpret_cast<const float4*>(sp + 4 * q);
    e.sh = *reinterpret_cast<const float4*>(hp + 4 * q);
  } else {
    float scv[4], shv[4];
#pragma unroll
    for (int j = 0; j < 4; ++j) {
      const int c = 4 * q + j;
      scv[j] = (a.scale && c < a.cout) ? a.scale[c] : 1.f;
      shv[j] = (a.shift && c < a.cout) ? a.shift[c] : 0.f;
    }
    e.sc = make_float4(scv[0], scv[1], scv[2], scv[3]);
    e.sh = make_float4(shv[0], shv[1], shv[2], shv[3]);
  }
  e.slope = *pp;
  return e;
}

template <bool FULL, bool HOOKS, int NRES, int SEGS, int CH = SEGS * 32 * 8 / 64, int BFO = 0, int BFR = BFO>
__device__ __forceinline__ float4 epilogue_lds_n(const ConvArgs& a, const EpiParams& ep_par, const f32x16 (&acc)[SEGS],
                                                 float* lds, int b, int y0, int x0, int wave, int lane) {
  float* ep = lds + wave * (SEGS * 32 * 32);
  const int h = lane >> 5, n = lane & 31;
#pragma unroll
  for (int sg = 0; sg < SEGS; ++sg)
#pragma unroll
    for (int r = 0; r < 16; ++r) ep[(sg * 32 + (r & 3) + 8 * (r >> 2) + 4 * h) * 32 + n] = acc[sg][r];
  const int q = lane & 7;
  const bool qvalid = FULL || (4 * q < a.cout);
  const float4 sc = ep_par.sc, sh = ep_par.sh;
  const float slope = ep_par.slope;
  constexpr int nres = NRES;
  float4 psum = make_float4(0.f, 0.f, 0.f, 0.f);
  constexpr int NITER = SEGS * 32 * 8 / 64;
  static_assert(NITER % CH == 0, "chunk must divide the element count");
  float4 r0[CH], r1[CH], r2[CH], ea[CH];
  const unsigned lane_off = (unsigned)(lane >> 3) * 32u + 4u * (unsigned)q;
  auto locate = [&](int it, size_t& off) -> bool {
    if constexpr (FULL) {
      const int sg = it >> 2;
      const size_t rowbase = ((size_t)(b * a.H + y0 + wave * SEGS + sg) * a.W + x0) * 32;
      off = rowbase + (size_t)((it & 3) * 256) + lane_off;
      return true;
    } else {
      const int pix = it * 8 + (lane >> 3);
      const int sg = pix >> 5, px = pix & 31;
      const int y = y0 + wave * SEGS + sg, x = x0 + px;
      off = ((size_t)(b * a.H + y) * a.W + x) * a.cout + 4 * q;
      return qvalid && y < a.H && x < a.W;
    }
  };
#pragma unroll
  for (int it0 = 0; it0 < NITER; it0 += CH) {
#pragma unroll
  for (int it = it0; it < it0 + CH; ++it) {
    size_t off;
    const bool ok = locate(it, off);
    const float4 z4 = make_float4(0.f, 0.f, 0.f, 0.f);
    r0[it - it0] = (nres > 0 && ok) ? paif::ldq_nt<BFR>(a.res[0], off) : z4;
    r1[it - it0] = (nres > 1 && ok) ? paif::ldq_nt<BFR>(a.res[1], off) : z4;
    r2[it - it0] = (nres > 2 && ok) ? paif::ldq_nt<BFR>(a.res[2], off) : z4;
    ea[it - it0] = (HOOKS && a.epi_dact && ok) ? *reinterpret_cast<const float4*>(a.epi_aux + off) : z4;
  }
#pragma unroll
  for (int it = it0; it < it0 + CH; ++it) {
    size_t off;
    const bool ok = locate(it, off);
    const int pix = it * 8 + (lane >> 3);
    float4 v = *reinterpret_cast<const float4*>(ep + pix * 32 + 4 * q);
    v.x = v.x * sc.x + sh.x; v.y = v.y * sc.y + sh.y; v.z = v.z * sc.z + sh.z; v.w = v.w * sc.w + sh.w;
    if (HOOKS && a.aux_out && ok) *reinterpret_cast<float4*>(a.aux_out + off) = v;
    if (a.act == 1) {
      v.x = paif::prelu_f(v.x, slope); v.y = paif::prelu_f(v.y, slope); v.z = paif::prelu_f(v.z, slope); v.w = paif::prelu_f(v.w, slope);
    } else if (a.act == 2) {
      v.x = fmaxf(v.x, 0.f); v.y = fmaxf(v.y, 0.f); v.z = fmaxf(v.z, 0.f); v.w = fmaxf(v.w, 0.f);
    }
    v.x *= a.alpha; v.y *= a.alpha; v.z *= a.alpha; v.w *= a.alpha;
    if (HOOKS && a.epi_dact == 1) {
      v.x *= ea[it - it0].x >= 0.f ? 1.f : slope; v.y *= ea[it - it0].y >= 0.f ? 1.f : slope;
      v.z *= ea[it - it0].z >= 0.f ? 1.f : slope; v.w *= ea[it - it0].w >= 0.f ? 1.f : slope;
    } else if (HOOKS && a.epi_dact == 2) {
      v.x *= ea[it - it0].x > 0.f ? 1.f : 0.f; v.y *= ea[it - it0].y > 0.f ? 1.f : 0.f;
      v.z *= ea[it - it0].z > 0.f ? 1.f : 0.f; v.w *= ea[it - it0].w > 0.f ? 1.f : 0.f;
    }
    if (nres > 0) { v.x += r0[it - it0].x; v.y += r0[it - it0].y; v.z += r0[it - it0].z; v.w += r0[it - it0].w; }
    if (nres > 1) { v.x += r1[it - it0].x; v.y += r1[it - it0].y; v.z += r1[it - it0].z; v.w += r1[it - it0].w; }
    if (nres > 2) { v.x += r2[it - it0].x; v.y += r2[it - it0].y; v.z += r2[it - it0].z; v.w += r2[it - it0].w; }
    if (ok) {
      paif::stq_nt<BFO>(a.out, off, v);
      psum.x += v.x; psum.y += v.y; psum.z += v.z; psum.w += v.w;
    }
    if (a.cpool) {
      float mx = fmaxf(fmaxf(v.x, v.y), fmaxf(v.z, v.w)), sm = (v.x + v.y) + (v.z + v.w);
      paif::pix8_max_sum(mx, sm);
      if (ok && q == 0) *reinterpret_cast<float2*>(a.cpool + (off >> 5) * 4) = make_float2(mx, sm * (1.0f / 32.0f));
    }
  }
  }
  return psum;
}

template <bool FULL, bool HOOKS, int SEGS = SEGS_PER_WAVE, int CH = SEGS * 32 * 8 / 64, int BFO = 0, int BFR = BFO>
__device__ __forceinline__ float4 epilogue_lds(const ConvArgs& a, const EpiParams& ep_par, const f32x16 (&acc)[SEGS], float* lds,
                                               int b, int y0, int x0, int wave, int lane) {
  if (!a.res[0]) return epilogue_lds_n<FULL, HOOKS, 0, SEGS, CH, BFO, BFR>(a, ep_par, acc, lds, b, y0, x0, wave, lane);
  if (!a.res[1]) return epilogue_lds_n<FULL, HOOKS, 1, SEGS, CH, BFO, BFR>(a, ep_par, acc, lds, b, y0, x0, wave, lane);
  if (!a.res[2]) return epilogue_lds_n<FULL, HOOKS, 2, SEGS, CH, BFO, BFR>(a, ep_par, acc, lds, b, y0, x0, wave, lane);
// ... 1120 lines not shown
    const int q = t & 7, px = t >> 3;
    const float4 sc = *reinterpret_cast<const float4*>((a.scale ? a.scale : k_ones) + 4 * q);
    const float4 sh = *reinterpret_cast<const float4*>((a.shift ? a.shift : k_zeros) + 4 * q);
    const float slope = *(a.act == 1 ? a.prelu : k_zeros);
    const int nres = a.res[0] ? (a.res[1] ? (a.res[2] ? 3 : 2) : 1) : 0;
    const unsigned lane_off = (unsigned)px * 32u + 4u * (unsigned)q;
    auto run = [&](auto nres_c) {
      constexpr int NR = decltype(nres_c)::value;
      float4 r[NR > 0 ? NR : 1][8];
      auto request = [&](int i) {
        int b, y0, x0;
        tile_of(min(i, cnt - 1), b, y0, x0);
        const size_t base = ((size_t)(b * a.H + y0) * a.W + x0) * 32;
        const unsigned lo = x0 + px < a.W ? lane_off : 0u;
#pragma unroll
        for (int k = 0; k < NR; ++k)
#pragma unroll
          for (int j = 0; j < 8; ++j) {
            const int yy = min(y0 + j, a.H - 1) - y0;
            r[k][j] = paif::ldq_nt<BFR>(a.res[k], base + (size_t)yy * a.W * 32 + lo);
          }
      };
      if (cnt > 0) request(0);
      int s2 = 0, i2 = 0;
      for (int g = 0; g <= S + 1; ++g) {
        if (g >= 2) {
          if (s2 == nsrc - 1) {
            int b, y0, x0;
            tile_of(i2, b, y0, x0);
            float4 o[8];
#pragma unroll
            for (int j = 0; j < 8; ++j) o[j] = *reinterpret_cast<const float4*>(outbuf + (j * 32 + px) * 32 + 4 * q);
            const size_t base = ((size_t)(b * a.H + y0) * a.W + x0) * 32;
            const bool colok = x0 + px < a.W;
#pragma unroll
            for (int j = 0; j < 8; ++j) {
              float4 v = o[j];
              v.x = v.x * sc.x + sh.x; v.y = v.y * sc.y + sh.y; v.z = v.z * sc.z + sh.z; v.w = v.w * sc.w + sh.w;
              if (a.act == 1) {
                v.x = paif::prelu_f(v.x, slope); v.y = paif::prelu_f(v.y, slope);
                v.z = paif::prelu_f(v.z, slope); v.w = paif::prelu_f(v.w, slope);
              } else if (a.act == 2) {
                v.x = fmaxf(v.x, 0.f); v.y = fmaxf(v.y, 0.f); v.z = fmaxf(v.z, 0.f); v.w = fmaxf(v.w, 0.f);
              }
              v.x *= a.alpha; v.y *= a.alpha; v.z *= a.alpha; v.w *= a.alpha;
#pragma unroll
              for (int k = 0; k < NR; ++k) { v.x += r[k][j].x; v.y += r[k][j].y; v.z += r[k][j].z; v.w += r[k][j].w; }
              if (colok && y0 + j < a.H)
                paif::stq_nt<BFO>(a.out, base + (size_t)j * a.W * 32 + lane_off, v);
              if (a.cpool) {
                float mx = fmaxf(fmaxf(v.x, v.y), fmaxf(v.z, v.w)), sm = (v.x + v.y) + (v.z + v.w);
                paif::pix8_max_sum(mx, sm);
                if (colok && y0 + j < a.H && q == 0)
                  *reinterpret_cast<float2*>(a.cpool + ((base + (size_t)j * a.W * 32) >> 5) * 4 + (size_t)px * 4) = make_float2(mx, sm * (1.0f / 32.0f));
              }
            }
            if (NR > 0) request(i2 + 1);
          }
          if (++s2 == nsrc) { s2 = 0; ++i2; }
        }
        lds_barrier();
        lds_barrier();
      }
    };
    if (nres == 0) run(std::integral_constant<int, 0>{});
    else if (nres == 1) run(std::integral_constant<int, 1>{});
    else if (nres == 2) run(std::integral_constant<int, 2>{});
    else run(std::integral_constant<int, 3>{});
  }
}

template <int KH, int DIL, int ST = 0>
__global__ __launch_bounds__(WS_THREADS, 1) void conv_bf16x3_ws(ConvArgs a, int ntiles) { conv_ws_body<KH, DIL, ST, false>(a, ntiles); }
template <int KH, int DIL, int ST = 0>
__global__ __launch_bounds__(WS_THREADS, 1) void conv_bf16x3_wsr(ConvArgs a, int ntiles) { conv_ws_body<KH, DIL, ST, true>(a, ntiles); }

template <int KH, int DIL, int ST = 0>
int launch_bf16x3_ws(const ConvArgs& a, hipStream_t st) {
  constexpr int P = DIL * (KH - 1) / 2;
  constexpr size_t lds_bytes = 2 * (size_t)(TH + 2 * P) * (TW + 2 * P) * 144 + 8 * 32 * 32 * 4;
  static_assert(lds_bytes <= 160 * 1024, "two tile buffers + the parked tile do not fit LDS");
  static bool raised = false;
  constexpr bool HAS_RELU = KH == 3 && DIL == 2 && paif::st_in(ST) != 0 && paif::st_low(ST) != 7;
  if (!raised) {
    hipError_t e = hipFuncSetAttribute(reinterpret_cast<const void*>(&conv_bf16x3_ws<KH, DIL, ST>),
                                       hipFuncAttributeMaxDynamicSharedMemorySize, (int)lds_bytes);
    if constexpr (HAS_RELU) {
      if (e == hipSuccess)
        e = hipFuncSetAttribute(reinterpret_cast<const void*>(&conv_bf16x3_wsr<KH, DIL, ST>), hipFuncAttributeMaxDynamicSharedMemorySize,
                                (int)lds_bytes);
    }
    if (e != hipSuccess) {
      paif::set_error("conv2d(bf16x3 ws): cannot raise dynamic LDS to %zu: %s", lds_bytes, hipGetErrorString(e));
      return (int)e;
    }
    raised = true;
  }
  if (a.in_act == 2) {
    if constexpr (HAS_RELU) {
      hipLaunchKernelGGL((conv_bf16x3_wsr<KH, DIL, ST>), dim3(256), dim3(WS_THREADS), lds_bytes, st, a, a.nblk);
      PAIF_LAUNCH_CHECK("conv2d(bf16x3 wsr)");
      return 0;
    }
    paif::set_error("conv2d(bf16x3 ws): input ReLU is built for the bf16-stored dilation-2 3x3 only");
    return PAIF_ENOSUP;
  }
  hipLaunchKernelGGL((conv_bf16x3_ws<KH, DIL, ST>), dim3(256), dim3(WS_THREADS), lds_bytes, st, a, a.nblk);
  PAIF_LAUNCH_CHECK("conv2d(bf16x3 ws)");
  return 0;
}

static inline bool ws_enabled() {
  static const bool on = [] {
    const char* e = getenv("PAIF_CONV_WS");
    return !(e && e[0] == '0');
  }();
  return on;
}
static inline bool st_h16(const ConvArgs& a) { return a.st == 1 || a.st == 3; }
static inline bool st_is_f16(const ConvArgs& a) { return a.st >= 3; }
static inline bool ws_eligible(const ConvArgs& a) {
  return ws_enabled() && a.nblk >= 1024 && !a.pool_partial && a.cout == 32 && (a.in_act == 0 || (a.in_act == 2 && st_h16(a))) &&
         (size_t)a.H * a.W * 128 < ((size_t)1 << 32);
}

static inline bool res_eligible(const ConvArgs& a) {
  static const bool on = [] {
    const char* e = getenv("PAIF_CONV_RES");
    return !(e && e[0] == '0');
  }();
  static const int ms_res = [] {
    const char* e = getenv("PAIF_CONV_RES_NSRC");
    return e ? atoi(e) : 1;
  }();
  return on && !st_is_f16(a) && (a.nsrc == 1 || (a.wl0 && a.st == 1 && a.in_act == 0 && a.nsrc <= ms_res)) && a.nblk >= 2048 && a.cout == 32 && a.in_act <= 2 && (PAIF_RES_ROWS == 8 || !a.pool_partial) &&
         (size_t)a.B * a.H * a.W * 128 < ((size_t)1 << 31);
}

static inline bool needs_hooks(const ConvArgs& a) { return a.in_act >= 3 || a.aux_out || a.epi_dact; }

static inline bool takes_ws(const ConvArgs& a, int kh, int dil) {
#if PAIF_TH == 8
  if (needs_hooks(a) || kh > 3 || !ws_eligible(a)) return false;
  if (a.st == 4) return dil == 2 && a.nsrc == 1 && a.in_act == 0;
  if (kh == 1) return !a.res[0] && a.in_act == 0;
  return dil == 2 && a.nsrc == 1 && st_h16(a);
#else
  return false;
#endif
}

enum ConvVariant { CV_PLAIN, CV_HOOKS, CV_WS, CV_RES, CV_MS, CV_DMA };
static inline int res_count(const ConvArgs& a) { return a.res[0] ? (a.res[1] ? (a.res[2] ? 3 : 2) : 1) : 0; }
static inline ConvVariant bf16x3_variant(const ConvArgs& a, int kh, int dil) {
  if (needs_hooks(a)) return CV_HOOKS;
  if (dil == 1 && st_h16(a) && a.wl0 && a.in_act == 0 && !a.pool_partial &&
      ((kh == 3 && a.cout == 32 && paif_conv_dma::eligible(a.nsrc, res_count(a), a.B, a.H, a.W, a.alpha)) ||
       (kh == 3 && a.cout == 16 && paif_conv_dma::eligible16(a.nsrc, res_count(a), a.B, a.H, a.W, a.alpha)) ||
       (kh == 7 && a.cout == 32 && paif_conv_dma::eligible7(a.nsrc, res_count(a), a.B, a.H, a.W, a.alpha))))
    return CV_DMA;
  if (kh == 3 && dil == 2 && st_h16(a) && a.wl0 && a.in_act == 2 && !a.pool_partial && a.cout == 32 &&
      paif_conv_dma::eligible_d2(a.nsrc, res_count(a), a.B, a.H, a.W, a.alpha))
    return CV_DMA;
  if (takes_ws(a, kh, dil)) return CV_WS;
  if (kh == 3 && dil == 1 && !st_is_f16(a)) {
    if (res_eligible(a)) return CV_RES;
    if (ms_enabled() && a.nsrc >= 2 && a.cout == 32 && a.in_act == 0 && !a.pool_partial &&
        (size_t)a.B * a.H * a.W * 128 < ((size_t)1 << 32))
      return CV_MS;
  }
  return CV_PLAIN;
}

static inline bool variant_can_cpool(const ConvArgs& a, int kh, int dil) {
  if (a.cout != 32 || needs_hooks(a)) return false;
  if (bf16x3_variant(a, kh, dil) == CV_DMA) return paif_conv_dma::can_cpool(a.nsrc, res_count(a), kh, a.cout, dil);
  return true;
}

template <int KH, int DIL, int ST>
int launch_bf16x3_st(const ConvArgs& a, hipStream_t st) {
  switch (bf16x3_variant(a, KH, DIL)) {
    case CV_DMA: {
      paif_conv_dma::Args d{};
      for (int s = 0; s < 3; ++s) { d.src[s] = a.src[s]; d.res[s] = a.res[s]; }
      d.wpk = a.wpk; d.scale = a.scale; d.shift = a.shift; d.prelu = a.prelu; d.out = a.out; d.alpha = a.alpha;
      d.nsrc = a.nsrc; d.nres = res_count(a); d.act = a.act; d.B = a.B; d.H = a.H; d.W = a.W; d.reverse = a.reverse; d.kh = KH; d.cout = a.cout;
      d.f16 = paif::st_f16(ST) ? 1 : 0;
      d.cpool = a.cpool;
      d.dil = DIL; d.in_relu = a.in_act == 2 ? 1 : 0;
      return paif_conv_dma::launch(d, st);
    }
    case CV_HOOKS:
      if constexpr (ST == 0) return launch_bf16x3_h<KH, DIL, true>(a, st);
      paif::set_error("conv2d: the gradient hooks (in_act >= 3, aux_out, epi_dact) are built for fp32 storage only");
      return PAIF_ENOSUP;
    case CV_WS:
#if PAIF_TH == 8
      if constexpr (KH <= 3) return launch_bf16x3_ws<KH, DIL, ST>(a, st);
#endif
      break;
    case CV_RES:
      if constexpr (KH == 3 && DIL == 1 && !paif::st_f16(ST)) {
        if constexpr (ST == 4) {
          if (a.nsrc == 2) return launch_bf16x3_res<3, 1, 2, ST>(a, st);
          if (a.nsrc == 3) return launch_bf16x3_res<3, 1, 3, ST>(a, st);
        }
        return launch_bf16x3_res<3, 1, 1, ST>(a, st);
      }
      break;
    case CV_MS:
      if constexpr (KH == 3 && DIL == 1 && !paif::st_f16(ST)) return a.nsrc == 2 ? launch_bf16x3_ms<3, 1, 2, ST>(a, st) : launch_bf16x3_ms<3, 1, 3, ST>(a, st);
      break;
    default: break;
  }
  return launch_bf16x3_h<KH, DIL, false, ST>(a, st);
}

static inline int kernel_st(const ConvArgs& a) {
  if (a.st == 4) return 15;
  const int st = a.st == 3 ? 1 : a.st;
  const int base = st == 1 ? (a.in_act == 1 ? 3 : 1) : st;
  const int code = (a.wl0 && base) ? base + 3 : base;
  return a.st >= 3 ? code + 8 : code;
}

template <int KH, int DIL>
int launch_bf16x6(const ConvArgs& a, hipStream_t st) {
  if (a.st != 0) {
    paif::set_error("conv2d: precision bf16x6 is built for fp32-stored maps");
    return PAIF_ENOSUP;
  }
  return needs_hooks(a) ? launch_bf16x3_h<KH, DIL, true, 0, 3>(a, st) : launch_bf16x3_h<KH, DIL, false, 0, 3>(a, st);
}

template <int KH, int DIL>
int launch_f16x3(const ConvArgs& a, hipStream_t st) {
  if (a.st != 0) {
    paif::set_error("conv2d: precision f16x3 is built for fp32-stored maps");
    return PAIF_ENOSUP;
  }
  return needs_hooks(a) ? launch_bf16x3_h<KH, DIL, true, 0, 2, 1>(a, st) : launch_bf16x3_h<KH, DIL, false, 0, 2, 1>(a, st);
}

template <int KH, int DIL>
int launch_bf16x3(const ConvArgs& a, hipStream_t st) {
  const int code = kernel_st(a);
  if (code == 0) return launch_bf16x3_st<KH, DIL, 0>(a, st);
  if constexpr ((KH == 1 || KH == 3 || KH == 7) && (DIL == 1 || (KH == 3 && DIL == 2))) {
    switch (code) {
      case 1: return launch_bf16x3_st<KH, DIL, 1>(a, st);
      case 3: return launch_bf16x3_st<KH, DIL, 3>(a, st);
      case 4: return launch_bf16x3_st<KH, DIL, 4>(a, st);
      case 6: return launch_bf16x3_st<KH, DIL, 6>(a, st);
      default: break;
    }
    if constexpr (KH == 1) {
      if (code == 2) return launch_bf16x3_st<KH, DIL, 2>(a, st);
      if (code == 5) return launch_bf16x3_st<KH, DIL, 5>(a, st);
    }
    switch (code) {
      case 12: return launch_bf16x3_st<KH, DIL, 12>(a, st);
      case 14: return launch_bf16x3_st<KH, DIL, 14>(a, st);
      default: break;
    }
    if constexpr (KH == 1) {
      if (code == 9) return launch_bf16x3_st<KH, DIL, 9>(a, st);
    }
    if constexpr (KH == 3 && DIL == 2) {
      if (code == 15) return launch_bf16x3_st<KH, DIL, 15>(a, st);
    }
  }
  paif::set_error("conv2d: storage %d is not built for the %dx%d dilation-%d kernel", a.st, KH, KH, DIL);
  return PAIF_ENOSUP;
}

__global__ void pack_weight_bf16x3_kernel(const float* __restrict__ w, unsigned short* __restrict__ wpk, int cout, int nsrc,
                                          int kh) {
  const int ntap = kh * kh;
  const int total = nsrc * ntap * 2 * 2 * 64 * 8;
  for (int idx = blockIdx.x * blockDim.x + threadIdx.x; idx < total; idx += gridDim.x * blockDim.x) {
    const int j = idx & 7, lane = (idx >> 3) & 63, part = (idx >> 9) & 1, ks = (idx >> 10) & 1;
    int rest = idx >> 11;
    const int tap = rest % ntap;
    const int s = rest / ntap;
    const int n = lane & 31, hh = lane >> 5;
    const int c = s * 32 + 16 * ks + 8 * hh + j;
    const float v = (n < cout) ? w[((size_t)n * (nsrc * 32) + c) * ntap + tap] : 0.f;
    const __bf16 hi = (__bf16)v;
    const __bf16 out = part == 0 ? hi : (__bf16)(v - (float)hi);
    wpk[idx] = __builtin_bit_cast(unsigned short, out);
  }
}

__global__ void compose_dw_pw_kernel(const float* __restrict__ dw, const float* __restrict__ pw, float* __restrict__ out, int cout,
                                     int cin, int ntap) {
  const int total = cout * cin * ntap;
  for (int idx = blockIdx.x * blockDim.x + threadIdx.x; idx < total; idx += gridDim.x * blockDim.x) {
    const int tap = idx % ntap, ci = (idx / ntap) % cin, co = idx / (ntap * cin);
    out[idx] = pw[co * cin + ci] * dw[ci * ntap + tap];
  }
}

__global__ void compose_pw_conv_kernel(const float* __restrict__ pw, const float* __restrict__ w, float* __restrict__ out, int cout, int cmid,
                                       int cin, int ntap) {
  const int total = cout * cin * ntap;
  for (int idx = blockIdx.x * blockDim.x + threadIdx.x; idx < total; idx += gridDim.x * blockDim.x) {
    const int rest = idx % (cin * ntap), co = idx / (cin * ntap);
    double acc = 0.0;
    for (int m = 0; m < cmid; ++m) acc = fma((double)pw[co * cmid + m], (double)w[(size_t)m * cin * ntap + rest], acc);
    out[idx] = (float)acc;
  }
}

__device__ __forceinline__ unsigned short bf16x6_piece(float v, int part) {
  const __bf16 hi = (__bf16)v;
  const float r1 = v - (float)hi;
  const __bf16 mid = (__bf16)r1;
  const __bf16 out = part == 0 ? hi : (part == 1 ? mid : (__bf16)(r1 - (float)mid));
  return __builtin_bit_cast(unsigned short, out);
}
__global__ void pack_weight_bf16x6_kernel(const float* __restrict__ w, unsigned short* __restrict__ wpk, int cout, int nsrc, int kh) {
  const int ntap = kh * kh;
  const int total = nsrc * ntap * 2 * 3 * 64 * 8;
  for (int idx = blockIdx.x * blockDim.x + threadIdx.x; idx < total; idx += gridDim.x * blockDim.x) {
    const int j = idx & 7, lane = (idx >> 3) & 63;
    int rest = idx >> 9;
    const int part = rest % 3; rest /= 3;
    const int ks = rest & 1; rest >>= 1;
    const int tap = rest % ntap;
    const int s = rest / ntap;
    const int n = lane & 31, hh = lane >> 5;
    const int c = s * 32 + 16 * ks + 8 * hh + j;
    const float v = (n < cout) ? w[((size_t)n * (nsrc * 32) + c) * ntap + tap] : 0.f;
    wpk[idx] = bf16x6_piece(v, part);
  }
}
__global__ void pack_decomp1x1_bf16x6_kernel(const float* __restrict__ w, unsigned short* __restrict__ wpk) {
  const int total = 3 * 2 * 3 * 64 * 8;
  for (int idx = blockIdx.x * blockDim.x + threadIdx.x; idx < total; idx += gridDim.x * blockDim.x) {
    const int j = idx & 7, lane = (idx >> 3) & 63;
    int rest = idx >> 9;
    const int part = rest % 3; rest /= 3;
    const int ks = rest & 1;
    const int s = rest >> 1;
    const int n = lane & 31, hh = lane >> 5;
    const int c = 16 * ks + 8 * hh + j;
    const float* wn = w + n * 128;
    float v;
    if (s == 0) v = wn[64 + c] + wn[96 + c];
    else if (s == 1) v = wn[c] - wn[64 + c];
    else v = wn[32 + c] - wn[96 + c];
    wpk[idx] = bf16x6_piece(v, part);
  }
}

__global__ void pack_decomp1x1_bf16x3_kernel(const float* __restrict__ w, unsigned short* __restrict__ wpk) {
  const int total = 3 * 2 * 2 * 64 * 8;
  for (int idx = blockIdx.x * blockDim.x + threadIdx.x; idx < total; idx += gridDim.x * blockDim.x) {
    const int j = idx & 7, lane = (idx >> 3) & 63, part = (idx >> 9) & 1, ks = (idx >> 10) & 1, s = idx >> 11;
    const int n = lane & 31, hh = lane >> 5;
    const int c = 16 * ks + 8 * hh + j;
    const float* wn = w + n * 128;
    float v;
    if (s == 0) v = wn[64 + c] + wn[96 + c];
    else if (s == 1) v = wn[c] - wn[64 + c];
    else v = wn[32 + c] - wn[96 + c];
    const __bf16 hi = (__bf16)v;
    const __bf16 out = part == 0 ? hi : (__bf16)(v - (float)hi);
    wpk[idx] = __builtin_bit_cast(unsigned short, out);
  }
}

__device__ __forceinline__ unsigned short f16x2_piece(float v, int part) {
  const _Float16 hi = (_Float16)v;
  const _Float16 out = part == 0 ? hi : (_Float16)(v - (float)hi);
  return __builtin_bit_cast(unsigned short, out);
}
__global__ void pack_weight_f16x2_kernel(const float* __restrict__ w, unsigned short* __restrict__ wpk, int cout, int nsrc, int kh) {
  const int ntap = kh * kh;
  const int total = nsrc * ntap * 2 * 2 * 64 * 8;
  for (int idx = blockIdx.x * blockDim.x + threadIdx.x; idx < total; idx += gridDim.x * blockDim.x) {
    const int j = idx & 7, lane = (idx >> 3) & 63, part = (idx >> 9) & 1, ks = (idx >> 10) & 1;
    int rest = idx >> 11;
    const int tap = rest % ntap;
    const int s = rest / ntap;
    const int n = lane & 31, hh = lane >> 5;
    const int c = s * 32 + 16 * ks + 8 * hh + j;
    const float v = (n < cout) ? w[((size_t)n * (nsrc * 32) + c) * ntap + tap] : 0.f;
    wpk[idx] = f16x2_piece(v, part);
  }
}
__global__ void pack_decomp1x1_hf_f16x2_kernel(const float* __restrict__ w, unsigned short* __restrict__ wpk) {
  const int total = 3 * 2 * 2 * 64 * 8;
  for (int idx = blockIdx.x * blockDim.x + threadIdx.x; idx < total; idx += gridDim.x * blockDim.x) {
    const int j = idx & 7, lane = (idx >> 3) & 63, part = (idx >> 9) & 1, ks = (idx >> 10) & 1, s = idx >> 11;
    const int n = lane & 31, hh = lane >> 5;
    const int c = 16 * ks + 8 * hh + j;
    const float* wn = w + n * 128;
    float v;
    if (s == 0) v = wn[c] + wn[32 + c];
    else if (s == 1) v = wn[64 + c] - wn[c];
    else v = wn[96 + c] - wn[32 + c];
    wpk[idx] = f16x2_piece(v, part);
  }
}

template <int KH, int DIL, int CIN, bool HOOKS>
int launch_h(const ConvArgs& a, hipStream_t st) {
  constexpr int P = DIL * (KH - 1) / 2;
  constexpr size_t tile_bytes = (size_t)(TH + 2 * P) * (TW + 2 * P) * (CIN + 4) * 4;
  constexpr size_t epi_bytes = (size_t)TH * 32 * 32 * 4;
  constexpr size_t lds_bytes = tile_bytes > epi_bytes ? tile_bytes : epi_bytes;
  static_assert(lds_bytes <= 160 * 1024, "tile does not fit LDS");
  if (lds_bytes > 64 * 1024) {
    hipError_t e = hipFuncSetAttribute(reinterpret_cast<const void*>(&conv_mfma_f32<KH, DIL, CIN, HOOKS>),
                                       hipFuncAttributeMaxDynamicSharedMemorySize, (int)lds_bytes);
    if (e != hipSuccess) {
      paif::set_error("conv2d: cannot raise dynamic LDS to %zu: %s", lds_bytes, hipGetErrorString(e));
      return (int)e;
    }
  }
  hipLaunchKernelGGL((conv_mfma_f32<KH, DIL, CIN, HOOKS>), dim3(a.nblk), dim3(NTHREADS), lds_bytes, st, a);
  PAIF_LAUNCH_CHECK("conv2d");
  return 0;
}

template <int KH, int DIL, int CIN>
int launch(const ConvArgs& a, hipStream_t st) {
  return needs_hooks(a) ? launch_h<KH, DIL, CIN, true>(a, st) : launch_h<KH, DIL, CIN, false>(a, st);
}

__global__ void pack_weight_kernel(const float* __restrict__ w, float* __restrict__ wpk, int cout, int nsrc, int cin,
                                   int kh) {
  const int ntap = kh * kh, no = cin / 8;
  const int total = nsrc * ntap * no * 256;
  for (int idx = blockIdx.x * blockDim.x + threadIdx.x; idx < total; idx += gridDim.x * blockDim.x) {
    const int i = idx & 3, lane = (idx >> 2) & 63;
    int rest = idx >> 8;
    const int o = rest % no; rest /= no;
    const int tap = rest % ntap;
    const int s = rest / ntap;
    const int n = lane & 31, h = lane >> 5;
    const int c = s * cin + 8 * o + 4 * h + i;
    wpk[idx] = (n < cout) ? w[((size_t)n * (nsrc * cin) + c) * ntap + tap] : 0.f;
  }
}

__global__ void pack_decomp1x1_kernel(const float* __restrict__ w, float* __restrict__ wpk) {
  const int total = 3 * 4 * 256;
  for (int idx = blockIdx.x * blockDim.x + threadIdx.x; idx < total; idx += gridDim.x * blockDim.x) {
    const int i = idx & 3, lane = (idx >> 2) & 63;
    const int o = (idx >> 8) & 3, s = idx >> 10;
    const int n = lane & 31, h = lane >> 5;
    const int c = 8 * o + 4 * h + i;
    const float* wn = w + n * 128;
    float v;
    if (s == 0) v = wn[64 + c] + wn[96 + c];
    else if (s == 1) v = wn[c] - wn[64 + c];
    else v = wn[32 + c] - wn[96 + c];
    wpk[idx] = v;
  }
}

__global__ void bn_fold_kernel(const float* g, const float* bta, const float* mean, const float* var, float eps,
                               float* scale, float* shift, int C) {
  const int c = blockIdx.x * blockDim.x + threadIdx.x;
  if (c < C) {
    const float s = g[c] / sqrtf(var[c] + eps);
    scale[c] = s;
    shift[c] = bta[c] - mean[c] * s;
  }
}

}

extern "C" {

int paif_conv2d_blocks(int B, int H, int W) { return B * ((H + TH - 1) / TH) * ((W + TW - 1) / TW); }

size_t paif_conv_wpk_floats(int nsrc, int cin, int kh) { return (size_t)nsrc * kh * kh * (cin / 8) * 256; }

int paif_conv2d_is_persistent(const paif_conv_desc* d, int B, int H, int W) {
  if (!d || (d->precision != PAIF_CONV_BF16X3 && d->precision != PAIF_CONV_BF16 && d->precision != PAIF_CONV_F16 && d->precision != PAIF_CONV_F16X2) ||
      d->cin != 32 || B <= 0 || H <= 0 || W <= 0)
    return 0;
  ConvArgs a{};
  for (int s = 0; s < 3; ++s) a.res[s] = d->res[s];
  a.pool_partial = d->pool_partial; a.nsrc = d->nsrc; a.in_act = d->in_act; a.cout = d->cout;
  a.aux_out = d->aux_out; a.epi_dact = d->epi_dact; a.st = d->storage;
  a.H = H; a.W = W;
  a.nblk = B * ((W + TW - 1) / TW) * ((H + TH - 1) / TH);
  return takes_ws(a, d->kh, d->dil) ? 1 : 0;
}

int paif_conv2d_can_cpool(const paif_conv_desc* d, int B, int H, int W) {
  if (!d || d->cout != 32 || d->cin != 32 || B <= 0 || H <= 0 || W <= 0 || d->precision == PAIF_CONV_F32 || d->precision == PAIF_CONV_BF16X6 || d->precision == PAIF_CONV_F16X3) return 0;
  ConvArgs a{};
  for (int s = 0; s < 3; ++s) a.res[s] = d->res[s];
  a.pool_partial = d->pool_partial; a.nsrc = d->nsrc; a.in_act = d->in_act; a.cout = d->cout;
  a.aux_out = d->aux_out; a.epi_dact = d->epi_dact;
  a.B = B; a.H = H; a.W = W;
  a.nblk = B * ((W + TW - 1) / TW) * ((H + TH - 1) / TH);
  a.st = d->storage; a.wl0 = (d->precision == PAIF_CONV_BF16 || d->precision == PAIF_CONV_F16) ? 1 : 0; a.alpha = d->alpha;
  return variant_can_cpool(a, d->kh, d->dil) ? 1 : 0;
}

int paif_conv2d_kernel_name(const paif_conv_desc* d, int B, int H, int W, char* buf, int buflen) {
  PAIF_REQUIRE(d && buf && buflen > 0 && B > 0 && H > 0 && W > 0, PAIF_EINVAL, "conv2d_kernel_name: bad arguments");
  ConvArgs a{};
  for (int s = 0; s < 3; ++s) a.res[s] = d->res[s];
  a.pool_partial = d->pool_partial; a.nsrc = d->nsrc; a.in_act = d->in_act; a.cout = d->cout;
  a.aux_out = d->aux_out; a.epi_dact = d->epi_dact;
  a.B = B; a.H = H; a.W = W;
  a.nblk = B * ((W + TW - 1) / TW) * ((H + TH - 1) / TH);
  a.st = d->storage; a.wl0 = (d->precision == PAIF_CONV_BF16 || d->precision == PAIF_CONV_F16) ? 1 : 0; a.alpha = d->alpha;
  const int code = kernel_st(a);
  if (d->precision == PAIF_CONV_BF16X6 && d->cin == 32) {
    snprintf(buf, buflen, "conv_mfma_bf16x6<%d, %d, %s, 0>", d->kh, d->dil, needs_hooks(a) ? "true" : "false");
    return 0;
  }
  if (d->precision == PAIF_CONV_F16X3 && d->cin == 32) {
    snprintf(buf, buflen, "conv_mfma_f16x3<%d, %d, %s, 0>", d->kh, d->dil, needs_hooks(a) ? "true" : "false");
    return 0;
  }
  if (d->precision != PAIF_CONV_BF16X3 && d->precision != PAIF_CONV_BF16 && d->precision != PAIF_CONV_F16 && d->precision != PAIF_CONV_F16X2) {
    snprintf(buf, buflen, "conv_mfma_f32<%d, %d, %d, %s>", d->kh, d->dil, d->cin, needs_hooks(a) ? "true" : "false");
    return 0;
  }
  if (d->cin != 32) {
    snprintf(buf, buflen, "conv_mfma_f32<%d, %d, %d, %s>", d->kh, d->dil, d->cin, needs_hooks(a) ? "true" : "false");
    return 0;
  }
  switch (bf16x3_variant(a, d->kh, d->dil)) {
    case CV_DMA:
      if (d->kh == 7) snprintf(buf, buflen, "conv7x7_h16_dma<%d>", a.st >= 3 ? 2 : 1);
      else snprintf(buf, buflen, "conv3x3_h16_dma<%d, %d, %d, %s, %d, %d>", d->nsrc, res_count(a), a.st >= 3 ? 2 : 1, d->cpool ? "true" : "false",
                    d->dil, d->dil == 2 ? 2 : 0);
      break;
    case CV_WS: snprintf(buf, buflen, "conv_bf16x3_ws%s<%d, %d, %d>", d->in_act == 2 ? "r" : "", d->kh, d->dil, code); break;
    case CV_RES: snprintf(buf, buflen, "conv_bf16x3_res<%d, %d, %d, %d, %d>", d->kh, d->dil, d->nsrc, PAIF_RES_ROWS, code); break;
    case CV_MS: snprintf(buf, buflen, "conv_bf16x3_ms<%d, %d, %d, %d>", d->kh, d->dil, d->nsrc, code); break;
    case CV_HOOKS: snprintf(buf, buflen, "conv_mfma_bf16x3<%d, %d, true, %d>", d->kh, d->dil, code); break;
    default: snprintf(buf, buflen, "conv_mfma_bf16x3<%d, %d, false, %d>", d->kh, d->dil, code); break;
  }
  return 0;
}

int paif_conv2d_fwd(const paif_conv_desc* d, int B, int H, int W, paif_stream_t stream) {
  PAIF_REQUIRE(d && d->out && d->wpk, PAIF_EINVAL, "conv2d: null descriptor/out/wpk");
  PAIF_REQUIRE(d->nsrc >= 1 && d->nsrc <= 3, PAIF_EINVAL, "conv2d: nsrc=%d", d->nsrc);
  for (int s = 0; s < d->nsrc; ++s) PAIF_REQUIRE(d->src[s], PAIF_EINVAL, "conv2d: src[%d] null", s);
  PAIF_REQUIRE(d->cout == 32 || d->cout == 16, PAIF_ENOSUP, "conv2d: cout=%d", d->cout);
  PAIF_REQUIRE(B > 0 && H > 0 && W > 0, PAIF_EINVAL, "conv2d: empty shape %dx%dx%d", B, H, W);
  PAIF_REQUIRE(d->in_act != 1 || d->in_prelu, PAIF_EINVAL, "conv2d: in_act=PReLU without slope");
  PAIF_REQUIRE(d->act != 1 || d->prelu, PAIF_EINVAL, "conv2d: act=PReLU without slope");
  ConvArgs a;
  for (int s = 0; s < 3; ++s) {
    a.src[s] = s < d->nsrc ? d->src[s] : nullptr;
    a.res[s] = d->res[s];
  }
  a.wpk = reinterpret_cast<const float4*>(d->wpk);
  a.in_prelu = d->in_prelu; a.scale = d->scale; a.shift = d->shift; a.prelu = d->prelu;
  a.out = d->out; a.pool_partial = d->pool_partial; a.cpool = d->cpool; a.alpha = d->alpha;
  a.nsrc = d->nsrc; a.in_act = d->in_act; a.act = d->act; a.cout = d->cout;
  a.aux_out = d->aux_out; a.in_aux = d->in_aux; a.in_scale = d->in_scale; a.in_alpha = d->in_alpha;
  a.epi_aux = d->epi_aux; a.epi_dact = d->epi_dact;
  PAIF_REQUIRE(d->in_act >= 0 && d->in_act <= 5, PAIF_EINVAL, "conv2d: in_act=%d", d->in_act);
  PAIF_REQUIRE(!(d->in_act == 3 || d->in_act == 4) || (d->in_aux && d->nsrc == 1), PAIF_EINVAL,
               "conv2d: in_act=%d needs in_aux and a single source", d->in_act);
  PAIF_REQUIRE(d->in_act != 3 || d->in_prelu, PAIF_EINVAL, "conv2d: in_act=3 without slope");
  PAIF_REQUIRE(d->epi_dact >= 0 && d->epi_dact <= 2 && (!d->epi_dact || d->epi_aux), PAIF_EINVAL, "conv2d: epi_dact=%d", d->epi_dact);
  PAIF_REQUIRE(d->epi_dact != 1 || d->prelu, PAIF_EINVAL, "conv2d: epi_dact=PReLU without slope");
  a.B = B; a.H = H; a.W = W;
  a.tilesX = (W + TW - 1) / TW; a.tilesY = (H + TH - 1) / TH; a.nblk = B * a.tilesX * a.tilesY;
  a.reverse = d->reverse_tiles ? 1 : 0;
  a.st = d->storage;
  a.wl0 = (d->precision == PAIF_CONV_BF16 || d->precision == PAIF_CONV_F16) ? 1 : 0;
  PAIF_REQUIRE(d->storage >= 0 && d->storage <= 4, PAIF_EINVAL, "conv2d: storage=%d", d->storage);
  const bool st_bf = d->storage == PAIF_ST_BF16 || d->storage == PAIF_ST_F32_BF16, st_hf = d->storage == PAIF_ST_F16 || d->storage == PAIF_ST_F16_F32;
  PAIF_REQUIRE(!st_bf || ((d->precision == PAIF_CONV_BF16X3 || d->precision == PAIF_CONV_BF16) && d->cin == 32), PAIF_ENOSUP,
               "conv2d: bf16 storage needs the split-bf16 kernels (cin 32)");
  PAIF_REQUIRE(!st_hf || ((d->precision == PAIF_CONV_F16 || d->precision == PAIF_CONV_F16X2) && d->cin == 32), PAIF_ENOSUP,
               "conv2d: fp16 storage takes precision F16 / F16X2 (cin 32)");
  PAIF_REQUIRE(d->precision != PAIF_CONV_BF16 || st_bf, PAIF_ENOSUP, "conv2d: precision bf16 is built for bf16-stored maps only");
  PAIF_REQUIRE((d->precision != PAIF_CONV_F16 && d->precision != PAIF_CONV_F16X2) || st_hf, PAIF_ENOSUP,
               "conv2d: precision fp16 is built for fp16-stored maps only");
  PAIF_REQUIRE(d->storage != PAIF_ST_F16_F32 || d->precision == PAIF_CONV_F16, PAIF_ENOSUP, "conv2d: fp16 in / fp32 out takes plain fp16 weights");
  hipStream_t st = paif::as_stream(stream);
  PAIF_REQUIRE(!d->cpool || paif_conv2d_can_cpool(d, B, H, W), PAIF_ENOSUP, "conv2d: no fused ChannelPool for this descriptor (paif_conv2d_can_cpool)");
  PAIF_REQUIRE(d->cin == 32 || d->cin == 16, PAIF_ENOSUP, "conv2d: cin=%d", d->cin);
  PAIF_REQUIRE(d->precision == PAIF_CONV_F32 || d->precision == PAIF_CONV_BF16X3 || d->precision == PAIF_CONV_BF16 ||
                   d->precision == PAIF_CONV_BF16X6 || d->precision == PAIF_CONV_F16 || d->precision == PAIF_CONV_F16X2 ||
                   d->precision == PAIF_CONV_F16X3, PAIF_EINVAL,
               "conv2d: precision=%d", d->precision);
  PAIF_REQUIRE((d->precision != PAIF_CONV_BF16X6 && d->precision != PAIF_CONV_F16X3) || d->cin == 32, PAIF_ENOSUP, "conv2d: bf16x6 / f16x3 need 32-channel sources");
  const int key = d->kh * 100 + d->dil * 10 + (d->cin == 32 ? 0 : 1);
  if (d->precision == PAIF_CONV_F16X3) {
    switch (key) {
      case 110: return launch_f16x3<1, 1>(a, st);
      case 310: return launch_f16x3<3, 1>(a, st);
      case 320: return launch_f16x3<3, 2>(a, st);
      case 510: return launch_f16x3<5, 1>(a, st);
      case 710: return launch_f16x3<7, 1>(a, st);
      default: break;
    }
    paif::set_error("conv2d(f16x3): kernel %dx%d dil %d cin %d not built", d->kh, d->kh, d->dil, d->cin);
    return PAIF_ENOSUP;
  }
  if (d->precision == PAIF_CONV_BF16X6) {
    switch (key) {
      case 110: return launch_bf16x6<1, 1>(a, st);
      case 310: return launch_bf16x6<3, 1>(a, st);
      case 320: return launch_bf16x6<3, 2>(a, st);
      case 510: return launch_bf16x6<5, 1>(a, st);
      case 710: return launch_bf16x6<7, 1>(a, st);
      default: break;
    }
    paif::set_error("conv2d(bf16x6): kernel %dx%d dil %d cin %d not built", d->kh, d->kh, d->dil, d->cin);
    return PAIF_ENOSUP;
  }
  if (d->precision == PAIF_CONV_BF16X3 || d->precision == PAIF_CONV_BF16 || d->precision == PAIF_CONV_F16 || d->precision == PAIF_CONV_F16X2) {
    switch (key) {
      case 110: return launch_bf16x3<1, 1>(a, st);
      case 310: return launch_bf16x3<3, 1>(a, st);
      case 320: return launch_bf16x3<3, 2>(a, st);
      case 510: return launch_bf16x3<5, 1>(a, st);
      case 520: return launch_bf16x3<5, 2>(a, st);
      case 710: return launch_bf16x3<7, 1>(a, st);
      case 720: return launch_bf16x3<7, 2>(a, st);
      default: break;
    }
    paif::set_error("conv2d(bf16x3): kernel %dx%d dil %d cin %d not built", d->kh, d->kh, d->dil, d->cin);
    return PAIF_ENOSUP;
  }
  switch (key) {
    case 110: return launch<1, 1, 32>(a, st);
    case 310: return launch<3, 1, 32>(a, st);
    case 320: return launch<3, 2, 32>(a, st);
    case 510: return launch<5, 1, 32>(a, st);
    case 520: return launch<5, 2, 32>(a, st);
    case 710: return launch<7, 1, 32>(a, st);
    case 720: return launch<7, 2, 32>(a, st);
    case 311: return launch<3, 1, 16>(a, st);
    default: break;
  }
  paif::set_error("conv2d: kernel %dx%d dil %d cin %d not built", d->kh, d->kh, d->dil, d->cin);
  return PAIF_ENOSUP;
}

int paif_pack_conv_weight_bf16x3(const float* w, float* wpk, int cout, int nsrc, int kh, paif_stream_t stream) {
  PAIF_REQUIRE(w && wpk, PAIF_EINVAL, "pack_conv_weight_bf16x3: null pointer");
  PAIF_REQUIRE(cout >= 1 && cout <= 32 && nsrc >= 1 && nsrc <= 3 && kh >= 1 && kh <= 7, PAIF_ENOSUP,
               "pack_conv_weight_bf16x3: cout=%d nsrc=%d kh=%d", cout, nsrc, kh);
  const int total = nsrc * kh * kh * 2048;
  hipLaunchKernelGGL(pack_weight_bf16x3_kernel, dim3((total + 255) / 256), dim3(256), 0, paif::as_stream(stream), w,
                     reinterpret_cast<unsigned short*>(wpk), cout, nsrc, kh);
  PAIF_LAUNCH_CHECK("pack_conv_weight_bf16x3");
  return 0;
}

int paif_pack_conv_weight_f16x2(const float* w, float* wpk, int cout, int nsrc, int kh, paif_stream_t stream) {
  PAIF_REQUIRE(w && wpk, PAIF_EINVAL, "pack_conv_weight_f16x2: null pointer");
  PAIF_REQUIRE(cout >= 1 && cout <= 32 && nsrc >= 1 && nsrc <= 3 && kh >= 1 && kh <= 7, PAIF_ENOSUP,
               "pack_conv_weight_f16x2: cout=%d nsrc=%d kh=%d", cout, nsrc, kh);
  const int total = nsrc * kh * kh * 2048;
  hipLaunchKernelGGL(pack_weight_f16x2_kernel, dim3((total + 255) / 256), dim3(256), 0, paif::as_stream(stream), w,
                     reinterpret_cast<unsigned short*>(wpk), cout, nsrc, kh);
  PAIF_LAUNCH_CHECK("pack_conv_weight_f16x2");
  return 0;
}

int paif_pack_decomp1x1_hf_weight_f16x2(const float* w, float* wpk, paif_stream_t stream) {
  PAIF_REQUIRE(w && wpk, PAIF_EINVAL, "pack_decomp1x1_hf_weight_f16x2: null pointer");
  hipLaunchKernelGGL(pack_decomp1x1_hf_f16x2_kernel, dim3(24), dim3(256), 0, paif::as_stream(stream), w,
                     reinterpret_cast<unsigned short*>(wpk));
  PAIF_LAUNCH_CHECK("pack_decomp1x1_hf_weight_f16x2");
  return 0;
}

int paif_pack_conv_weight_bf16x6(const float* w, float* wpk, int cout, int nsrc, int kh, paif_stream_t stream) {
  PAIF_REQUIRE(w && wpk, PAIF_EINVAL, "pack_conv_weight_bf16x6: null pointer");
  PAIF_REQUIRE(cout >= 1 && cout <= 32 && nsrc >= 1 && nsrc <= 3 && kh >= 1 && kh <= 7, PAIF_ENOSUP,
               "pack_conv_weight_bf16x6: cout=%d nsrc=%d kh=%d", cout, nsrc, kh);
  const int total = nsrc * kh * kh * 3072;
  hipLaunchKernelGGL(pack_weight_bf16x6_kernel, dim3((total + 255) / 256), dim3(256), 0, paif::as_stream(stream), w,
                     reinterpret_cast<unsigned short*>(wpk), cout, nsrc, kh);
  PAIF_LAUNCH_CHECK("pack_conv_weight_bf16x6");
  return 0;
}

int paif_compose_dw_pw_weight(const float* dw, const float* pw, float* out, int cout, int cin, int kh, paif_stream_t stream) {
  PAIF_REQUIRE(dw && pw && out && cout >= 1 && cin >= 1 && kh >= 1 && kh <= 7, PAIF_EINVAL, "compose_dw_pw_weight: bad arguments");
  const int total = cout * cin * kh * kh;
  hipLaunchKernelGGL(compose_dw_pw_kernel, dim3((total + 255) / 256), dim3(256), 0, paif::as_stream(stream), dw, pw, out, cout, cin, kh * kh);
  PAIF_LAUNCH_CHECK("compose_dw_pw_weight");
  return 0;
}

int paif_compose_pw_conv_weight(const float* pw, const float* w, float* out, int cout, int cmid, int cin, int kh, paif_stream_t stream) {
  PAIF_REQUIRE(pw && w && out && cout >= 1 && cmid >= 1 && cin >= 1 && kh >= 1 && kh <= 7, PAIF_EINVAL, "compose_pw_conv_weight: bad arguments");
  const int total = cout * cin * kh * kh;
  hipLaunchKernelGGL(compose_pw_conv_kernel, dim3((total + 255) / 256), dim3(256), 0, paif::as_stream(stream), pw, w, out, cout, cmid, cin, kh * kh);
  PAIF_LAUNCH_CHECK("compose_pw_conv_weight");
  return 0;
}

int paif_pack_decomp1x1_weight_bf16x6(const float* w, float* wpk, paif_stream_t stream) {
  PAIF_REQUIRE(w && wpk, PAIF_EINVAL, "pack_decomp1x1_weight_bf16x6: null pointer");
  hipLaunchKernelGGL(pack_decomp1x1_bf16x6_kernel, dim3(36), dim3(256), 0, paif::as_stream(stream), w,
                     reinterpret_cast<unsigned short*>(wpk));
  PAIF_LAUNCH_CHECK("pack_decomp1x1_weight_bf16x6");
  return 0;
}

int paif_pack_decomp1x1_weight_bf16x3(const float* w, float* wpk, paif_stream_t stream) {
  PAIF_REQUIRE(w && wpk, PAIF_EINVAL, "pack_decomp1x1_weight_bf16x3: null pointer");
  hipLaunchKernelGGL(pack_decomp1x1_bf16x3_kernel, dim3(24), dim3(256), 0, paif::as_stream(stream), w,
                     reinterpret_cast<unsigned short*>(wpk));
  PAIF_LAUNCH_CHECK("pack_decomp1x1_weight_bf16x3");
// ... 32 lines not shown
```

### paif_amd/operations_m.py

```python
import torch
import torch.nn as nn

from . import ops


class _NeverCalled:
    def forward(self, *a, **k):
        raise RuntimeError("%s is a parameter holder; the HIP path must be used" % type(self).__name__)


class Conv2dParams(_NeverCalled, nn.Conv2d):
    pass


class Conv1dParams(_NeverCalled, nn.Conv1d):
    pass


class BatchNormParams(_NeverCalled, nn.BatchNorm2d):
    pass


class PReLUParams(_NeverCalled, nn.PReLU):
    pass
# ... 314 lines not shown
            tape.append(dict(x=x))
        return ops.conv2d([t], w, 1, 1, scale=scale, shift=shift, res=(x,) + tuple(res), cpool=cpool)

    def backward_nhwc(self, g, t, wgrad=False):
        op = self.op
        if "c" in t:
            bn = op[3]
            d_c = ops.bn_act_bwd(g, t["c"], t["stats"], ops.ACT_NONE, None,
                                 ops.grad_of(bn.weight) if wgrad and bn.affine else None,
                                 ops.grad_of(bn.bias) if wgrad and bn.affine else None, None, training=t["bn_training"])
            d_t = ops.conv2d([d_c], self._dgrad_w("c1x1", op[2].weight), 1, 1)
            if wgrad:
                gw = ops.grad_of(op[2].weight)
                if gw is not None:
                    ops.conv2d_wgrad([t["t"]], d_c, 1, 1, out=gw)
                gd = ops.grad_of(op[1].conv.weight)
                if gd is not None:
                    ops.dwconv_wgrad(t["x"], d_t, self.k, self.d, True, gd)
            return ops.dwconv_bwd(d_t, op[1].conv.weight, self.k, self.d, aux=t["x"], add=g)
        scale, _ = _bn_scale_shift(op[3], self._packs)
        d_t = ops.conv2d([g], self._dgrad_w("c1x1", op[2].weight), 1, 1, in_act=ops.IN_SCALE, in_scale=scale)
        return ops.dwconv_bwd(d_t, op[1].conv.weight, self.k, self.d, aux=t["x"], add=g)


def _bn_split(bn, c, act, slope, res):
    g, b = (bn.weight, bn.bias) if bn.affine else (None, None)
    if bn.training:
        if bn.momentum is None or not bn.track_running_stats:
            raise NotImplementedError("BatchNorm with momentum=None / track_running_stats=False is not used by the reference")
        stats = ops.bn_stats(c, g, b, bn.eps, bn.momentum, bn.running_mean, bn.running_var)
        bn.num_batches_tracked.add_(1)
    else:
        stats = ops.bn_eval_stats(g, b, bn.running_mean, bn.running_var, bn.eps)
    return ops.affine_act_res(c, stats[2], stats[3], act, slope, res), stats


def _bn_scale_shift(bn, cache=None, name="bn"):
    if bn.training:
        raise RuntimeError("_bn_scale_shift folds RUNNING statistics: train-mode BatchNorm goes through _bn_split (batch statistics)")

    def build():
        if bn.affine:
            return ops.bn_fold(bn.weight, bn.bias, bn.running_mean, bn.running_var, bn.eps)
        one = torch.ones_like(bn.running_mean)
        return ops.bn_fold(one, torch.zeros_like(one), bn.running_mean, bn.running_var, bn.eps)

    if cache is None:
        return build()
    keys = [bn.running_mean, bn.running_var] + ([bn.weight, bn.bias] if bn.affine else [])
    return cache.get(name, keys, build)


class SepConv(_HipOp):

    def __init__(self, C_in, C_out, kernel_size, stride, padding, affine=True):
        super().__init__()
        if stride != 1 or padding != kernel_size // 2:
            raise NotImplementedError("SepConv is only reachable with stride 1, padding k//2 (OPS registry)")
        self.k = kernel_size
        self.op = nn.Sequential(
            nn.ReLU(inplace=False),
            Conv2dParams(C_in, C_in, kernel_size=kernel_size, stride=stride, padding=padding, groups=C_in, bias=False),
            Conv2dParams(C_in, C_in, kernel_size=1, padding=0, bias=False),
            BatchNormParams(C_in, affine=affine),
            nn.ReLU(inplace=False),
            Conv2dParams(C_in, C_in, kernel_size=kernel_size, stride=1, padding=padding, groups=C_in, bias=False),
            Conv2dParams(C_in, C_out, kernel_size=1, padding=0, bias=False),
            BatchNormParams(C_out, affine=affine),
        )

    def backward_nhwc(self, g, t, wgrad=False):
        op = self.op
        if "c2" in t:
            go = lambda p_: ops.grad_of(p_) if wgrad else None
            aff = lambda bn: (go(bn.weight), go(bn.bias)) if bn.affine else (None, None)
            d_c2 = ops.bn_act_bwd(g, t["c2"], t["stats2"], ops.ACT_NONE, None, *aff(op[7]), None, training=t["bn_training"])
            d_t2 = ops.conv2d([d_c2], self._dgrad_w("c6", op[6].weight), 1, 1)
            d_a = ops.dwconv_bwd(d_t2, op[5].weight, self.k, 1)
            d_c1 = ops.bn_act_bwd(d_a, t["c1"], t["stats1"], ops.ACT_RELU, None, *aff(op[3]), None, training=t["bn_training"])
            d_t = ops.conv2d([d_c1], self._dgrad_w("c2", op[2].weight), 1, 1)
            if wgrad:
                for w, src, dout in ((op[6].weight, t["t2"], d_c2), (op[2].weight, t["t"], d_c1)):
                    gw = ops.grad_of(w)
                    if gw is not None:
                        ops.conv2d_wgrad([src], dout, 1, 1, out=gw)
                for w, src, dout, relu in ((op[5].weight, t["a"], d_t2, False), (op[1].weight, t["x"], d_t, True)):
                    gw = ops.grad_of(w)
                    if gw is not None:
                        ops.dwconv_wgrad(src, dout, self.k, 1, relu, gw)
            return ops.dwconv_bwd(d_t, op[1].weight, self.k, 1, aux=t["x"])
        s1, _ = _bn_scale_shift(op[3], self._packs, 'bn1')
        s2, _ = _bn_scale_shift(op[7], self._packs, 'bn2')
        d_t5 = ops.conv2d([g], self._dgrad_w("c6", op[6].weight), 1, 1, in_act=ops.IN_SCALE, in_scale=s2)
        d_z3 = ops.dwconv_bwd(d_t5, op[5].weight, self.k, 1, aux=t["z3"])
        d_t1 = ops.conv2d([d_z3], self._dgrad_w("c2", op[2].weight), 1, 1, in_act=ops.IN_SCALE, in_scale=s1)
        return ops.dwconv_bwd(d_t1, op[1].weight, self.k, 1, aux=t["x"])

    def forward_nhwc(self, x, res=(), tape=None):
        op = self.op
        t = ops.dwconv(x, op[1].weight, self.k, 1, in_relu=True)
        w1 = self._packs.get("w1", [op[2].weight], lambda: ops.pack_conv_weight(op[2].weight, 1, 32, 1))
        w2 = self._packs.get("w2", [op[6].weight], lambda: ops.pack_conv_weight(op[6].weight, 1, 32, 1))
        if op[3].training or (tape is not None and ops.taping_wgrad()):
            c1 = ops.conv2d([t], w1, 1, 1)
            a, stats1 = _bn_split(op[3], c1, ops.ACT_RELU, None, ())
            t2 = ops.dwconv(a, op[5].weight, self.k, 1, in_relu=False)
            c2 = ops.conv2d([t2], w2, 1, 1)
            out, stats2 = _bn_split(op[7], c2, ops.ACT_NONE, None, tuple(res))
            if tape is not None:
                tape.append(dict(x=x, t=t, c1=c1, a=a, t2=t2, c2=c2, stats1=stats1, stats2=stats2, bn_training=op[3].training))
            return out
        s1, b1 = _bn_scale_shift(op[3], self._packs, 'bn1')
        if tape is not None:
            t, z3 = ops.conv2d([t], w1, 1, 1, scale=s1, shift=b1, act=ops.ACT_RELU, want_aux=True)
            tape.append(dict(x=x, z3=z3))
        else:
            t = ops.conv2d([t], w1, 1, 1, scale=s1, shift=b1, act=ops.ACT_RELU)
        t = ops.dwconv(t, op[5].weight, self.k, 1, in_relu=False)
        s2, b2 = _bn_scale_shift(op[7], self._packs, 'bn2')
        return ops.conv2d([t], w2, 1, 1, scale=s2, shift=b2, res=res)


class eca_layer(nn.Module):

    def __init__(self, channel, c_out, stride, k_size=3):
        super().__init__()
        self.k_size = k_size
        self.conv = Conv1dParams(1, 1, kernel_size=k_size, padding=(k_size - 1) // 2, bias=False)

    def forward(self, x):
        ops.require_no_grad(x)
        if x.shape[1] != 32:
            raise NotImplementedError("eca_layer: the HIP kernels are built for the 32-channel maps of the search space")
        with torch.no_grad():
            return ops.to_nchw_view(ops.eca_layer_fwd(ops.to_nhwc(x), self.conv.weight, self.k_size))


class ECABasicBlock(_HipOp):

    def __init__(self, inplanes, planes, kernel=3, dilation=1, stride=1, reduction=64, with_norm=False):
        super().__init__()
        if with_norm:
            raise NotImplementedError("ECABasicBlock(with_norm=True) is never constructed by the reference")
        self.with_norm = with_norm
        self.k = kernel
        self.conv1 = conv3x3(inplanes, planes, stride)
        self.conv2 = BasicConv(inplanes, inplanes, kernel, relu=False)
        self.se = eca_layer(planes, planes, stride, k_size=kernel)
        self.relu = PReLUParams()

    def forward_nhwc(self, x, res=(), tape=None):
        a = self.relu.weight
        w1 = self._packs.get("w1", [self.conv1.weight], lambda: ops.pack_conv_weight(self.conv1.weight, 1, 32, 3))
        r = ops.conv2d([x], w1, 3, 1)
        o, partial = ops.conv2d([r], self.conv2.wpk(1, 32), self.k, 1, in_act=ops.ACT_PRELU, in_prelu=a, pool=True)
        if tape is None:
            out = ops.eca_finish(o, r, partial, self.se.conv.weight, self.k, a)
        else:
            out, u, gate = ops.eca_finish(o, r, partial, self.se.conv.weight, self.k, a, save=True)
            tape.append(dict(r=r, o=o, u=u, gate=gate, x=x, pool=partial) if ops.taping_wgrad() else dict(r=r, o=o, u=u, gate=gate))
        return self._add_res(out, res)

    bwd_takes_res = True

    def backward_nhwc(self, g, t, wgrad=False, res=()):
        a = self.relu.weight
        if not wgrad:
            d_o, d_r = ops.eca_bwd(g, t["u"], t["o"], t["gate"], self.se.conv.weight, self.k, a)
            d_r = ops.conv2d([d_o], self._dgrad_w("c2", self.conv2.conv.weight), self.k, 1, epi_dact=1, epi_aux=t["r"], prelu=a, res=(d_r,))
            return ops.conv2d([d_r], self._dgrad_w("c1", self.conv1.weight), 3, 1, res=tuple(res))
        B, H, W, _ = g.shape
        ds = ops.grad_of(a)
        if ds is not None:
            ops.prelu_bwd(g, t["u"], a, ds)
        d_o, d_r, dgate = ops.eca_bwd(g, t["u"], t["o"], t["gate"], self.se.conv.weight, self.k, a, want_partial=True)
        g1d = ops.grad_of(self.se.conv.weight)
        if g1d is not None:
            ops.eca_wgrad(t["pool"], dgate, t["gate"], self.k, g1d, B, H, W)
        gw2 = ops.grad_of(self.conv2.conv.weight)
        if gw2 is not None:
            ops.conv2d_wgrad([ops.affine_act_res(t["r"], None, None, ops.ACT_PRELU, a)], d_o, self.k, 1, out=gw2)
        tt = ops.conv2d([d_o], self._dgrad_w("c2", self.conv2.conv.weight), self.k, 1)
        d_r = ops.prelu_bwd(tt, t["r"], a, ds, add=d_r, want_dx=True)
        gw1 = ops.grad_of(self.conv1.weight)
        if gw1 is not None:
            ops.conv2d_wgrad([t["x"]], d_r, 3, 1, out=gw1)
        return ops.conv2d([d_r], self._dgrad_w("c1", self.conv1.weight), 3, 1, res=tuple(res))


class Spatial_BasicBlock(_HipOp):

    def __init__(self, inplanes, planes, kernel=3, dilation=1, stride=1, reduction=64, with_norm=False):
        super().__init__()
        self.k = kernel
        self.conv1 = conv3x3(inplanes, planes, stride)
        self.conv2 = BasicConv(inplanes, inplanes, kernel, relu=False)
        self.se = spatial_attn_layer(kernel)
        self.relu = PReLUParams()

    def forward_nhwc(self, x, res=(), tape=None):
        a = self.relu.weight
        w1 = self._packs.get("w1", [self.conv1.weight], lambda: ops.pack_conv_weight(self.conv1.weight, 1, 32, 3))
        r = ops.conv2d([x], w1, 3, 1)
        o = ops.conv2d([r], self.conv2.wpk(1, 32), self.k, 1, in_act=ops.ACT_PRELU, in_prelu=a)
        wsp = self.se.spatial.conv.weight
        if tape is None:
            out = ops.spa1(o, r, wsp, self.k, a)
        elif ops.taping_wgrad():
            out, u, s, comp = ops.spa1(o, r, wsp, self.k, a, save=True, want_comp=True)
            tape.append(dict(r=r, o=o, u=u, s=s, x=x, comp=comp))
        else:
            out, u, s = ops.spa1(o, r, wsp, self.k, a, save=True)
            tape.append(dict(r=r, o=o, u=u, s=s))
        return self._add_res(out, res)

    def backward_nhwc(self, g, t, wgrad=False):
        a = self.relu.weight
        wsp = self.se.spatial.conv.weight
        if not wgrad:
            d_o, d_r = ops.spa1_bwd(g, t["u"], t["o"], t["s"], wsp, self.k, a)
            d_r = ops.conv2d([d_o], self._dgrad_w("c2", self.conv2.conv.weight), self.k, 1, epi_dact=1, epi_aux=t["r"], prelu=a, res=(d_r,))
            return ops.conv2d([d_r], self._dgrad_w("c1", self.conv1.weight), 3, 1)
        ds = ops.grad_of(a)
        if ds is not None:
            ops.prelu_bwd(g, t["u"], a, ds)
        d_o, d_r, dpre = ops.spa1_bwd(g, t["u"], t["o"], t["s"], wsp, self.k, a, want_dpre=True)
        gsp = ops.grad_of(wsp)
        if gsp is not None:
            tmp = torch.zeros(4 * self.k * self.k, device=g.device, dtype=torch.float32)
            ops.corr1_wgrad(dpre, ops.pad_channels(t["comp"], 4), self.k, tmp)
            ops.axpy_(gsp.view(-1), tmp[:2 * self.k * self.k])
        gw2 = ops.grad_of(self.conv2.conv.weight)
        if gw2 is not None:
            ops.conv2d_wgrad([ops.affine_act_res(t["r"], None, None, ops.ACT_PRELU, a)], d_o, self.k, 1, out=gw2)
        tt = ops.conv2d([d_o], self._dgrad_w("c2", self.conv2.conv.weight), self.k, 1)
        d_r = ops.prelu_bwd(tt, t["r"], a, ds, add=d_r, want_dx=True)
        gw1 = ops.grad_of(self.conv1.weight)
        if gw1 is not None:
            ops.conv2d_wgrad([t["x"]], d_r, 3, 1, out=gw1)
        return ops.conv2d([d_r], self._dgrad_w("c1", self.conv1.weight), 3, 1)


class ChannelPool(nn.Module):

    def forward(self, x):
        ops.require_no_grad(x)
        if x.shape[1] != 32:
            raise NotImplementedError("ChannelPool: the HIP kernels are built for the 32-channel maps of the search space")
        with torch.no_grad():
            xh = ops.to_nhwc(x)
            one = torch.ones(1, device=x.device, dtype=torch.float32)
            comp = ops.spa1(xh, torch.zeros_like(xh), torch.zeros(1, 2, 3, 3, device=x.device), 3, one, save=True, want_comp=True)[3]
            return comp.permute(0, 3, 1, 2).contiguous()


class spatial_attn_layer(nn.Module):

    def __init__(self, kernel_size=5):
        super().__init__()
        self.compress = ChannelPool()
        self.spatial = BasicConv(2, 1, kernel_size, relu=False)

    def forward(self, x):
        ops.require_no_grad(x)
        if x.shape[1] != 32:
            raise NotImplementedError("spatial_attn_layer: the HIP kernels are built for the 32-channel maps of the search space")
        with torch.no_grad():
            xh = ops.to_nhwc(x)
            one = torch.ones(1, device=x.device, dtype=torch.float32)
            k = self.spatial.conv.weight.shape[-1]
            return ops.to_nchw_view(ops.spa1(xh, torch.zeros_like(xh), self.spatial.conv.weight, k, one))


def _selfpath(*a, **k):
    raise NotImplementedError("SelAttention/SelfPath is unreachable from MixedOp in the reference (SURVEY.md 8(a) F4)")


OPS = {
    'Denseblocks': lambda C, kernel, dialtion, affine: ResidualDenseBlock(C, kernel, dialtion),
    'Residualblocks': lambda C, kernel, dialtion, affine: ResidualModule(C, kernel, dialtion),
    'ECAattention': lambda C, kernel, dialtion, affine: ECABasicBlock(C, C, kernel, dialtion),
    'SPAattention': lambda C, kernel, dialtion, affine: Spatial_BasicBlock(C, C, kernel, dialtion),
    'DilConv': lambda C, kernel, dialtion, affine: DilConv(C, C, kernel, dialtion),
    'SepConv': lambda C, kernel, dialtion, affine: SepConv(C, C, kernel, 1, kernel // 2),
    'SelAttention': lambda C, kernel, dialtion, affine: _selfpath(),
}
```

### paif_amd/ops.py

```python
import ctypes
import weakref
import os

import torch

from . import _lib

ACT_NONE, ACT_PRELU, ACT_RELU = 0, 1, 2
ACT_GELU = 1

def _env_switch(name, default="1"):
    v = os.environ.get(name, default)
    if v not in ("0", "1", "gemm"):
        raise ValueError("%s=%r: expected 0, 1 or gemm" % (name, v))
    return {"0": False, "1": True, "gemm": "gemm"}[v]


GEMM_PRECISIONS = ("f32", "bf16x3", "auto", "bf16x6", "auto6", "f16x3", "auto6h")


def _env_gemm_precision():
    v = os.environ.get("PAIF_GEMM_PRECISION", "auto")
    if v not in GEMM_PRECISIONS:
        raise ValueError("PAIF_GEMM_PRECISION=%r: expected one of %s" % (v, GEMM_PRECISIONS))
# ... 518 lines not shown
            raise NotImplementedError("guided filter: an fp16 target map is built for the fp16 configuration's high-frequency output only")
        fn = (L.paif_guided_filter_fused_fwd_hf16_y16 if y16 else L.paif_guided_filter_fused_fwd_hf16 if hf16 else
              L.paif_guided_filter_fused_fwd_bf16 if out_bf16 else L.paif_guided_filter_fused_fwd)
        _lib.check(fn(_p(guide), _pa(y) if y16 else _p(y), _pa(lf), eps[0], eps[1], _p(ws), B, H, W, _stream()), "guided_filter_fused")
        if e0 is not None:
            TIMER.stop(tag, e0, 650 * B * H * W * 32, B * H * W * (4 + (2 if y16 else 4) * 32 + (2 if out_bf16 else 4) * 64))
        return lf
    assert not out_bf16, "bf16 low-frequency maps are an inference (fused-form) output"
    lf = torch.empty((2, B, H, W, 32), device=y.device, dtype=torch.float32)
    import os
    assert tape in (None, "mc", "ab"), tape
    if tape is None:
        tape = os.environ.get("PAIF_GF_TAPE")
        if tape not in (None, "mc", "ab"):
            raise ValueError("PAIF_GF_TAPE must be 'mc' or 'ab', got %r" % tape)
    if tape is None:
        tape = "mc" if os.environ.get("PAIF_GF_BWD") != "v1" and L.paif_guided_filter_taped_fits(B, H, W) else "ab"
    if want_ab and tape == "mc":
        mc = torch.empty((2, B, H, W, 32), device=y.device, dtype=torch.float32)
        stats = torch.empty(L.paif_guided_filter_fused_workspace_floats(B, H, W), device=y.device, dtype=torch.float32)
        _lib.check(L.paif_guided_filter_taped_fwd(_p(guide), _p(y), _p(mc), _p(lf), eps[0], eps[1], _p(stats), B, H, W, _stream()),
                   "guided_filter_taped")
        return lf, GfTape(mc, stats)
    ab = torch.empty((4, B, H, W, 32), device=y.device, dtype=torch.float32)
    _lib.check(L.paif_guided_filter_ab_fwd(_p(guide), _p(y), _p(ab), eps[0], eps[1], B, H, W, _stream()), "guided_filter_ab")
    _lib.check(L.paif_guided_filter_lf_fwd(_p(guide), _p(ab), _p(lf), B, H, W, _stream()), "guided_filter_lf")
    return (lf, ab) if want_ab else lf


def pack_conv_weight(w, nsrc, cin, kh, precision=None):
    cout = w.shape[0]
    assert tuple(w.shape) == (cout, nsrc * cin, kh, kh), (tuple(w.shape), nsrc, cin, kh)
    precision = precision or pack_precision()
    if cin != 32:
        precision = "f32"
    L = lib()
    nfl = L.paif_conv_wpk_floats(nsrc, cin, kh)
    wpk = torch.empty(nfl * 3 // 2 if precision == "bf16x6" else nfl, device=w.device, dtype=torch.float32)
    wc = w.detach().contiguous()
    if precision in ("f16", "f16x2"):
        _lib.check(L.paif_pack_conv_weight_f16x2(_p(wc), _p(wpk), cout, nsrc, kh, _stream()), "pack_conv_weight_f16x2")
    elif precision == "f16x3":
        _lib.check(L.paif_pack_conv_weight_f16x2(_p(wc * F16X3_WSCALE), _p(wpk), cout, nsrc, kh, _stream()), "pack_conv_weight_f16x2")
    elif precision == "bf16x6":
        _lib.check(L.paif_pack_conv_weight_bf16x6(_p(wc), _p(wpk), cout, nsrc, kh, _stream()), "pack_conv_weight_bf16x6")
    elif precision == "bf16x3":
        _lib.check(L.paif_pack_conv_weight_bf16x3(_p(wc), _p(wpk), cout, nsrc, kh, _stream()), "pack_conv_weight_bf16x3")
    else:
        _lib.check(L.paif_pack_conv_weight(_p(wc), _p(wpk), cout, nsrc, cin, kh, _stream()), "pack_conv_weight")
    return PackedWeight(wpk, precision)


def compose_dw_pw_weight(dw, pw):
    C, _, k, _ = dw.shape
    Co = pw.shape[0]
    assert tuple(dw.shape) == (C, 1, k, k) and tuple(pw.shape) == (Co, C, 1, 1)
    out = torch.empty((Co, C, k, k), device=dw.device, dtype=torch.float32)
    _lib.check(lib().paif_compose_dw_pw_weight(_p(dw.detach().contiguous()), _p(pw.detach().contiguous()), _p(out), Co, C, k, _stream()),
               "compose_dw_pw_weight")
    return out


def compose_pw_conv_weight(pw, w):
    Cm, Ci, k, _ = w.shape
    Co = pw.shape[0]
    assert tuple(pw.shape) == (Co, Cm, 1, 1)
    out = torch.empty((Co, Ci, k, k), device=w.device, dtype=torch.float32)
    _lib.check(lib().paif_compose_pw_conv_weight(_p(pw.detach().contiguous()), _p(w.detach().contiguous()), _p(out), Co, Cm, Ci, k, _stream()),
               "compose_pw_conv_weight")
    return out


def pack_decomp1x1_weight(w, precision=None):
    assert tuple(w.shape) == (32, 128, 1, 1)
    precision = precision or CONFIG["conv_precision"]
    L = lib()
    nfl = L.paif_conv_wpk_floats(3, 32, 1)
    wpk = torch.empty(nfl * 3 // 2 if precision == "bf16x6" else nfl, device=w.device, dtype=torch.float32)
    wc = w.detach().contiguous()
    if precision == "f16x3":
        w2 = wc.view(32, 128)
        fold = torch.cat([w2[:, 64:96] + w2[:, 96:128], w2[:, 0:32] - w2[:, 64:96], w2[:, 32:64] - w2[:, 96:128]], dim=1).contiguous()
        _lib.check(L.paif_pack_conv_weight_f16x2(_p(fold * F16X3_WSCALE), _p(wpk), 32, 3, 1, _stream()), "pack_conv_weight_f16x2")
    elif precision == "bf16x6":
        _lib.check(L.paif_pack_decomp1x1_weight_bf16x6(_p(wc), _p(wpk), _stream()), "pack_decomp1x1_weight_bf16x6")
    elif precision == "bf16x3":
        _lib.check(L.paif_pack_decomp1x1_weight_bf16x3(_p(wc), _p(wpk), _stream()), "pack_decomp1x1_weight_bf16x3")
    else:
        _lib.check(L.paif_pack_decomp1x1_weight(_p(wc), _p(wpk), _stream()), "pack_decomp1x1_weight")
    return PackedWeight(wpk, precision)


def rdb_fused_pack(w1, w2, w3, dtype):
    assert tuple(w1.shape) == (32, 32, 3, 3) and tuple(w2.shape) == (32, 64, 3, 3) and tuple(w3.shape) == (32, 96, 3, 3) and dtype in H16
    L = lib()
    wpk = torch.empty(L.paif_rdb_fused_wpk_floats(), device=w1.device, dtype=torch.float32)
    _lib.check(L.paif_rdb_fused_pack(_p(w1.detach().contiguous()), _p(w2.detach().contiguous()), _p(w3.detach().contiguous()), _p(wpk),
                                     int(dtype == torch.float16), _stream()), "rdb_fused_pack")
    return PackedWeight(wpk, "rdb_f16" if dtype == torch.float16 else "rdb_bf16")


def rdb_fused(x, wpk, prelu, alpha=0.333333, res=(), cpool=None):
    B, H, W, C = x.shape
    assert C == 32 and x.dtype in H16 and x.is_contiguous() and len(res) <= 2
    assert wpk.precision == ("rdb_f16" if x.dtype == torch.float16 else "rdb_bf16")
    res = [cast_storage(r, x.dtype) for r in res]
    out = torch.empty_like(x)
    cp = None
    if cpool is not None:
        comp, coff = cpool
        assert comp.dtype == torch.float32 and tuple(comp.shape) == (B, H, W, 4) and comp.is_contiguous() and coff in (0, 2)
        cp = ctypes.c_void_p(comp.data_ptr() + 4 * coff)
    if CONFIG.get("serpentine", True):
        _SERP[0] ^= 1
    tag = "rdb_fused_kernel"
    e0 = TIMER.start(tag) if TIMER is not None else None
    _lib.check(lib().paif_rdb_fused_fwd(_pa(x), _p(wpk.data), _p(prelu), float(alpha), _pa(res[0]) if len(res) > 0 else None,
                                        _pa(res[1]) if len(res) > 1 else None, _pa(out), cp, int(x.dtype == torch.float16),
                                        _SERP[0] if CONFIG.get("serpentine", True) else 0, B, H, W, _stream()), "rdb_fused")
    if e0 is not None:
        px = B * H * W
        TIMER.stop(tag, e0, 2 * px * 9 * 32 * 32 * 6, px * 2 * 32 * 9, px * 2 * 32 * len(res))
    return out


def pack_decomp1x1_hf_weight(w):
    assert tuple(w.shape) == (32, 128, 1, 1)
    L = lib()
    wpk = torch.empty(L.paif_conv_wpk_floats(3, 32, 1), device=w.device, dtype=torch.float32)
    _lib.check(L.paif_pack_decomp1x1_hf_weight_f16x2(_p(w.detach().contiguous()), _p(wpk), _stream()), "pack_decomp1x1_hf_weight_f16x2")
    return PackedWeight(wpk, "f16x2" if CONFIG.get("f16_decomp_split", False) else "f16")


def bn_fold(weight, bias, mean, var, eps):
    C = weight.shape[0]
    scale = torch.empty(C, device=weight.device, dtype=torch.float32)
    shift = torch.empty(C, device=weight.device, dtype=torch.float32)
    _lib.check(lib().paif_bn_fold(_p(weight.detach()), _p(bias.detach()), _p(mean), _p(var), eps, _p(scale), _p(shift), C, _stream()),
               "bn_fold")
    return scale, shift


IN_DPRELU, IN_DRELU, IN_SCALE = 3, 4, 5


def conv2d_kernel_name(desc, B, H, W):
    buf = ctypes.create_string_buffer(96)
    _lib.check(lib().paif_conv2d_kernel_name(ctypes.byref(desc), B, H, W, buf, len(buf)), "conv2d_kernel_name")
    return buf.value.decode()


def conv2d(srcs, wpk, kh, dil=1, cin=32, cout=32, in_act=ACT_NONE, in_prelu=None, scale=None, shift=None,
           act=ACT_NONE, prelu=None, alpha=1.0, res=(), pool=False, want_aux=False, in_aux=None, in_scale=None,
           in_alpha=1.0, epi_dact=0, epi_aux=None, out=None, out_f32=False, cpool=None):
    B, H, W, C = srcs[0].shape
    assert C == cin and 1 <= len(srcs) <= 3
    res = [r for r in res if r is not None]
    extra = res[3:]
    res = res[:3]
    sdt = srcs[0].dtype
    src16 = sdt in H16
    assert all(s_.dtype == sdt for s_ in srcs), "mixed source storage"
    if out is not None:
        odt = out.dtype
    elif src16:
        want32 = (out_f32 and sdt == torch.float16 and kh == 3 and dil == 2 and len(srcs) == 1 and in_act == ACT_NONE and not pool and cout == 32
                  and wpk.precision == "f16")
        odt = torch.float32 if want32 else sdt
    else:
        odt = torch.bfloat16 if (_ACT_BF16[0] is torch.bfloat16 and kh == 1 and not want_aux and in_act < 3 and not epi_dact) else torch.float32
    out16 = odt in H16
    if src16:
        storage = (3 if out16 else 4) if sdt == torch.float16 else 1
        if not out16 and sdt != torch.float16:
            raise NotImplementedError("bf16 sources with an fp32 output are not built")
    else:
        storage = 0 if not out16 else 2
        if odt == torch.float16:
            raise NotImplementedError("fp32 sources with an fp16 output are not built (the fp16 forward hands the 1x1 fp16 maps)")
    if storage and (want_aux or in_act >= 3 or epi_dact or in_aux is not None):
        raise NotImplementedError("16-bit activation storage is built for the inference forward (no gradient hooks)")
    if wpk.precision == "f16x3" and storage:
        raise NotImplementedError("the fp16-pair conv arithmetic is built for fp32 maps")
    if (sdt == torch.float16) != (wpk.precision in ("f16", "f16x2")):
        raise RuntimeError("conv2d: fp16 maps need an fp16 weight pack and vice versa (sources %s, pack %s)" % (sdt, wpk.precision))
    if out is None:
        out = torch.empty((B, H, W, cout), device=srcs[0].device, dtype=odt)
    else:
        assert tuple(out.shape) == (B, H, W, cout) and out.is_contiguous()
    rdt = sdt if storage == 4 else odt
    res = [cast_storage(r, rdt) for r in res]
    extra = [cast_storage(r, odt) for r in extra]
    src_bf, out_bf = src16, out16
    L = lib()
    d = _lib.ConvDesc()
    d.storage = storage
    for i in range(3):
        d.src[i] = _pa(srcs[i]) if i < len(srcs) else None
        d.res[i] = _pa(res[i]) if i < len(res) else None
    for r in res:
        assert tuple(r.shape) == (B, H, W, cout)
    d.nsrc, d.cin, d.wpk, d.kh, d.dil = len(srcs), cin, _p(wpk.data), kh, dil
    d.precision = _PREC_CODE[wpk.precision]
    if storage in (1, 2) and wpk.precision == "bf16x3" and CONFIG["storage"] == "bf16":
        d.precision = PREC_BF16
    d.in_act, d.in_prelu = in_act, _p(in_prelu)
    d.scale, d.shift = _p(scale), _p(shift)
    d.act, d.prelu, d.alpha = act, _p(prelu), alpha
    d.out, d.cout = _pa(out), cout
    partial = None
    if pool:
        partial = torch.empty((L.paif_conv2d_blocks(B, H, W), 32), device=out.device, dtype=torch.float32)
    d.pool_partial = _p(partial)
    aux = torch.empty_like(out) if want_aux else None
    d.aux_out, d.in_aux, d.in_scale, d.in_alpha = _p(aux), _p(in_aux), _p(in_scale), in_alpha
    d.epi_aux, d.epi_dact = _p(epi_aux), epi_dact
    pool_after = None
    if cpool is not None:
        comp, coff = cpool
        assert cout == 32 and comp.dtype == torch.float32 and tuple(comp.shape) == (B, H, W, 4) and comp.is_contiguous() and coff in (0, 2)
        if not extra and CONFIG.get("cpool_fused", True) and L.paif_conv2d_can_cpool(ctypes.byref(d), B, H, W):
            d.cpool = ctypes.c_void_p(comp.data_ptr() + 4 * coff)
        else:
            pool_after = (comp, coff)
    if CONFIG.get("serpentine", True):
        _SERP[0] ^= 1
        d.reverse_tiles = _SERP[0]
    e0 = None
    if TIMER is not None:
        tag = conv2d_kernel_name(d, B, H, W)
        e0 = TIMER.start(tag)
    _lib.check(L.paif_conv2d_fwd(ctypes.byref(d), B, H, W, _stream()), "conv2d")
    if e0 is not None:
        px = B * H * W
        eb_in, eb_out = (2 if src_bf else 4), (2 if out_bf else 4)
        eb_res = 2 if (res and res[0].dtype in H16) else 4
        TIMER.stop(tag, e0, 2 * px * kh * kh * cin * len(srcs) * cout, px * (eb_in * cin * len(srcs) + eb_out * cout), px * eb_res * cout * len(res))
    for r in extra:
        out = add(out, r)
    if pool_after is not None:
        channel_pool1(out, *pool_after)
    if pool and want_aux:
        return out, partial, aux
    if want_aux:
        return out, aux
    return (out, partial) if pool else out


def pack_conv_dgrad_weight(w, coff, cs, precision=None):
    Co, Ctot, k, _ = w.shape
    wt = torch.empty((cs, Co, k, k), device=w.device, dtype=torch.float32)
    _lib.check(lib().paif_conv_weight_dgrad(_p(w.detach().contiguous()), _p(wt), Co, Ctot, k, coff, cs, _stream()), "conv_weight_dgrad")
    return pack_conv_weight(wt, 1, Co, k, precision)


def fold_decomp1x1_weight(w):
    wf = torch.empty((32, 96, 1, 1), device=w.device, dtype=torch.float32)
    _lib.check(lib().paif_fold_decomp1x1_weight(_p(w.detach().contiguous()), _p(wf), _stream()), "fold_decomp1x1_weight")
    return wf


def dwconv(x, w, k, dil, in_relu):
    B, H, W, C = x.shape
    assert C == 32
    out = torch.empty_like(x)
    fn = {torch.bfloat16: lib().paif_dwconv_fwd_bf16, torch.float16: lib().paif_dwconv_fwd_f16}.get(x.dtype, lib().paif_dwconv_fwd)
    _lib.check(fn(_pa(x), _p(w.detach().contiguous()), _pa(out), k, dil, int(in_relu), B, H, W, _stream()), "dwconv")
    return out


def channel_pool2(ir, vis):
    B, H, W, _ = ir.shape
    comp = torch.empty((B, H, W, 4), device=ir.device, dtype=torch.float32)
    assert ir.dtype == vis.dtype
    fn = {torch.bfloat16: lib().paif_channel_pool2_fwd_bf16, torch.float16: lib().paif_channel_pool2_fwd_f16}.get(ir.dtype, lib().paif_channel_pool2_fwd)
    _lib.check(fn(_pa(ir), _pa(vis), _p(comp), B, H, W, _stream()), "channel_pool2")
    return comp


def channel_pool1(x, comp, coff):
    B, H, W, C = x.shape
    assert C == 32 and tuple(comp.shape) == (B, H, W, 4) and comp.dtype == torch.float32 and coff in (0, 2)
    fn = {torch.bfloat16: lib().paif_channel_pool1_fwd_bf16, torch.float16: lib().paif_channel_pool1_fwd_f16}.get(x.dtype, lib().paif_channel_pool1_fwd)
    _lib.check(fn(_pa(x), ctypes.c_void_p(comp.data_ptr() + 4 * coff), B, H, W, _stream()), "channel_pool1")
    return comp


def spa_blend(comp, w, ir, vis, want_scale=False):
    B, H, W, _ = ir.shape
    agg = torch.empty_like(ir)
    if ir.dtype in H16:
        assert not want_scale and vis.dtype == ir.dtype
        fn = lib().paif_spa_blend_fwd_f16 if ir.dtype == torch.float16 else lib().paif_spa_blend_fwd_bf16
        _lib.check(fn(_p(comp), _p(w.detach().contiguous()), _pa(ir), _pa(vis), _pa(agg), B, H, W, _stream()), "spa_blend")
        return agg
    scale = torch.empty((B, H, W), device=ir.device, dtype=torch.float32) if want_scale else None
    _lib.check(lib().paif_spa_blend_fwd(_p(comp), _p(w.detach().contiguous()), _p(ir), _p(vis), _p(agg), _p(scale), B, H, W, _stream()),
               "spa_blend")
    return (agg, scale) if want_scale else agg


def eca_finish(o, r, partial, w1d, k, prelu, save=False):
    B, H, W, _ = o.shape
    out = torch.empty_like(o)
    gate = torch.empty((B, 32), device=o.device, dtype=torch.float32)
    if o.dtype in H16:
        assert not save and r.dtype == o.dtype
        fn = lib().paif_eca_finish_fwd_f16 if o.dtype == torch.float16 else lib().paif_eca_finish_fwd_bf16
        _lib.check(fn(_pa(o), _pa(r), _p(partial), _p(w1d.detach().contiguous()), k, _p(prelu), _p(gate), _pa(out),
                                                  B, H, W, _stream()), "eca_finish")
        return out
    u = torch.empty_like(o) if save else None
    _lib.check(lib().paif_eca_finish_fwd(_p(o), _p(r), _p(partial), _p(w1d.detach().contiguous()), k, _p(prelu), _p(gate), _p(out),
                                         _p(u), B, H, W, _stream()), "eca_finish")
    return (out, u, gate) if save else out


def eca_layer_fwd(x, w1d, k):
    B, H, W, C = x.shape
    assert C == 32 and x.dtype == torch.float32
    L = lib()
    chunks = L.paif_conv2d_blocks(1, H, W)
    partial = torch.empty((B, chunks, 32), device=x.device, dtype=torch.float32)
    _lib.check(L.paif_channel_sum_chunks_fwd(_p(x), _p(partial), chunks, B, H, W, _stream()), "channel_sum_chunks")
    one = torch.ones(1, device=x.device, dtype=torch.float32)
    return eca_finish(x, torch.zeros_like(x), partial, w1d, k, one)


def eca_bwd(dout, u, o, gate, w1d, k, prelu, want_partial=False):
    B, H, W, _ = o.shape
    L = lib()
    partial = torch.empty((B, L.paif_eca_bwd_blocks(H, W), 32), device=o.device, dtype=torch.float32)
    coef = torch.empty((B, 32), device=o.device, dtype=torch.float32)
    d_o, d_r = torch.empty_like(o), torch.empty_like(o)
    _lib.check(L.paif_eca_bwd_input(_p(dout), _p(u), _p(o), _p(gate), _p(w1d.detach().contiguous()), k, _p(prelu), _p(partial), _p(coef),
                                    _p(d_o), _p(d_r), B, H, W, _stream()), "eca_bwd")
    return (d_o, d_r, partial) if want_partial else (d_o, d_r)


def spa_blend_bwd(dagg, w, ir, vis, s, add_ir=None, add_vis=None, want_dpre=False):
    B, H, W, _ = ir.shape
    dpre = torch.empty((B, H, W), device=ir.device, dtype=torch.float32)
    d_ir, d_vis = torch.empty_like(ir), torch.empty_like(vis)
    _lib.check(lib().paif_spa_blend_bwd_input(_p(dagg), _p(w.detach().contiguous()), _p(ir), _p(vis), _p(s), _p(add_ir), _p(add_vis),
                                              _p(dpre), _p(d_ir), _p(d_vis), B, H, W, _stream()), "spa_blend_bwd")
    return (d_ir, d_vis, dpre) if want_dpre else (d_ir, d_vis)


def dwconv_bwd(dt, w, k, dil, aux=None, add=None):
    B, H, W, _ = dt.shape
    out = torch.empty_like(dt)
    _lib.check(lib().paif_dwconv_bwd_input(_p(dt), _p(w.detach().contiguous()), _p(aux), _p(add), _p(out), k, dil, B, H, W, _stream()),
               "dwconv_bwd")
    return out


def guided_filter_bwd(guide, y, ab, dlf, eps=(0.001, 0.0001), add=None):
    B, H, W, _ = y.shape
    dev = y.device
    if isinstance(ab, GfTape):
        t_my, t_mgy, dy = torch.empty_like(y), torch.empty_like(y), torch.empty_like(y)
        t_g = torch.empty((B, H, W, 4), device=dev, dtype=torch.float32)
        _lib.check(lib().paif_guided_filter_bwd_input_mc(_p(guide), _p(y), _p(ab.mc), _p(ab.stats), _p(dlf), _p(add), _p(t_my), _p(t_mgy),
                                                         _p(t_g), _p(dy), B, H, W, _stream()), "guided_filter_bwd_mc")
        return dy
    gstat = torch.empty(lib().paif_guided_filter_fused_workspace_floats(B, H, W), device=dev, dtype=torch.float32)
    t_my, t_mgy = torch.empty_like(y), torch.empty_like(y)
    t_g = torch.empty((B, H, W, 4), device=dev, dtype=torch.float32)
    dy = torch.empty_like(y)
    _lib.check(lib().paif_guided_filter_bwd_input(_p(guide), _p(y), _p(ab), _p(dlf), eps[0], eps[1], _p(add), _p(gstat), _p(t_my),
                                                  _p(t_mgy), _p(t_g), _p(dy), B, H, W, _stream()), "guided_filter_bwd")
    return dy


def stem_bwd(dfeat, feat, w, prelu):
    B, H, W, _ = feat.shape
    dimg = torch.empty((B, 1, H, W), device=feat.device, dtype=torch.float32)
    _lib.check(lib().paif_stem_bwd_input(_p(dfeat), _p(feat), _p(w.detach().contiguous()), _p(prelu), _p(dimg), B, H, W, _stream()), "stem_bwd")
    return dimg


def tail_bwd(dfused, fused, z, w, prelu):
    B, _, H, W = fused.shape
    dt16 = torch.empty((B, H, W, 16), device=fused.device, dtype=torch.float32)
    _lib.check(lib().paif_tail_bwd_input(_p(dfused.contiguous()), _p(fused), _p(z), _p(w.detach().contiguous()), _p(prelu), _p(dt16), B, H, W,
                                         _stream()), "tail_bwd")
    return dt16


def stem_out_pack(w1, w2):
    assert tuple(w1.shape) == (16, 32, 3, 3) and tuple(w2.shape) == (1, 16, 3, 3)
    L = lib()
    wpk = torch.empty(L.paif_stem_out_pack_floats(), device=w1.device, dtype=torch.float32)
    _lib.check(L.paif_stem_out_pack(_p(w1.detach().contiguous()), _p(w2.detach().contiguous()), _p(wpk), _stream()), "stem_out_pack")
    return wpk


def stem_out_fused(x, wpk, prelu):
    B, H, W, C = x.shape
    assert C == 32 and x.dtype in (torch.bfloat16, torch.float32)
    fused = torch.empty((B, 1, H, W), device=x.device, dtype=torch.float32)
    if _ACT_BF16[0] is torch.float16:
        flag = f16_guard_flag(x.device)
        _lib.check(lib().paif_stem_out_fwd_guard(_pa(x), int(x.dtype == torch.float32), _p(wpk), _p(prelu), _p(fused),
                                                 ctypes.c_void_p(flag.data_ptr()), B, H, W, _stream()), "stem_out_fused")
        return fused
    fn = lib().paif_stem_out_fwd_bf16 if x.dtype == torch.bfloat16 else lib().paif_stem_out_fwd_f32
    _lib.check(fn(_pa(x), _p(wpk), _p(prelu), _p(fused), B, H, W, _stream()), "stem_out_fused")
    return fused


def tail(x16, w, prelu, save=False):
    B, H, W, C = x16.shape
    assert C == 16
    fused = torch.empty((B, 1, H, W), device=x16.device, dtype=torch.float32)
    if x16.dtype in H16:
        assert not save
        fn = lib().paif_tail_fwd_f16 if x16.dtype == torch.float16 else lib().paif_tail_fwd_bf16
        _lib.check(fn(_pa(x16), _p(w.detach().contiguous()), _p(prelu), _p(fused), B, H, W, _stream()), "tail")
        return fused
    z = torch.empty((B, 1, H, W), device=x16.device, dtype=torch.float32) if save else None
    _lib.check(lib().paif_tail_fwd(_p(x16), _p(w.detach().contiguous()), _p(prelu), _p(fused), _p(z), B, H, W, _stream()), "tail")
    return (fused, z) if save else fused


def add(a, b):
    assert a.shape == b.shape
    if a.dtype in H16 or b.dtype in H16:
        dt = a.dtype if a.dtype in H16 else b.dtype
        a, b = cast_storage(a, dt), cast_storage(b, dt)
        out = torch.empty_like(a)
        fn = lib().paif_add_fwd_f16 if dt == torch.float16 else lib().paif_add_fwd_bf16
        _lib.check(fn(_pa(a), _pa(b), _pa(out), a.numel(), _stream()), "add")
        return out
    out = torch.empty_like(a)
    _lib.check(lib().paif_add_fwd(_p(a), _p(b), _p(out), a.numel(), _stream()), "add")
    return out


_GEMM2_PACKS = {}


def _gemm2_pack(w, prec):
    key = (w.data_ptr(), w._version, tuple(w.shape), str(w.device), CONFIG.get("weights_generation", 0))
    ent = _GEMM2_PACKS.get(id(w))
    if ent is None or ent[0]() is not w or ent[1] != key:
        ent = (weakref.ref(w, lambda _, i=id(w): _GEMM2_PACKS.pop(i, None)), key, {})
        _GEMM2_PACKS[id(w)] = ent
    pk = ent[2].get(prec)
    if pk is None:
        if torch.cuda.is_available() and torch.cuda.is_current_stream_capturing():
            raise RuntimeError("the pre-split image of a %s GEMM weight (%s) is missing while a hipGraph is being captured: run one eager "
                               "step in this arithmetic first" % (tuple(w.shape), prec))
        N, K = w.shape
        L = lib()
        pk = torch.empty(L.paif_gemm2_packed_bytes(N, K, _PREC_CODE[prec]), device=w.device, dtype=torch.uint8)
        _lib.check(L.paif_gemm2_pack_weight(_p(w.detach()), ctypes.c_void_p(pk.data_ptr()), N, K, _PREC_CODE[prec], _stream()), "gemm2_pack")
        ent[2][prec] = pk
    return pk


def gemm(a, w, scale=None, shift=None, act=ACT_NONE, res=None, out=None, out_cols=None, col_offset=0,
         a_cols=None, a_mask=None, a_scale=None):
    N = w.shape[0]
    lda = a.shape[-1]
    if a_cols is None:
        K, aptr = lda, _p(a)
    else:
        _p(a)
        c0, K = a_cols
# ... 831 lines not shown
```

Baseline: 2459.

## Fuse ECA channel pooling into conv1 and apply gate in conv2 epilogue

Reworks the ECA block for fp16 maps. The first conv now writes per-tile channel sums of PReLU(r) from its epilogue. A small gate kernel then derives the global-mean gate, using weight linearity and border corrections from those sums instead of pooling the conv2 output. The second conv applies the input PReLU in LDS and gate*o+r with PReLU in its epilogue, which removes the separate pool partials and the eca_finish pass over the full map. The cost is more per-lane reductions, extra stores and a new gate kernel on the critical path between the convs, and the numerics are tied to the fp16 rounding path.

```diff
diff --git a/include/paif_hip.h b/include/paif_hip.h
--- a/include/paif_hip.h
+++ b/include/paif_hip.h
@@ -86,6 +86,8 @@
   int reverse_tiles;
   int storage;
   float* cpool;
+  float* eca_sums;
+  const float* eca_gate;
 } paif_conv_desc;
 #define PAIF_ST_F32 0
 #define PAIF_ST_BF16 1
@@ -122,6 +124,9 @@
 
 int paif_conv2d_blocks(int B, int H, int W);
 int paif_conv2d_fwd(const paif_conv_desc* d, int B, int H, int W, paif_stream_t stream);
+int paif_conv2d_eca_eligible(int B, int H, int W);
+int paif_eca_gate_f16(const float* sums, const float* r, const float* wpk, const float* prelu, const float* w1d, int k, float* gate, int B, int H,
+                      int W, paif_stream_t stream);
 int paif_conv2d_can_cpool(const paif_conv_desc* d, int B, int H, int W);
 int paif_channel_pool1_fwd(const float* x, float* comp_off, int B, int H, int W, paif_stream_t stream);
 int paif_channel_pool1_fwd_bf16(const float* x, float* comp_off, int B, int H, int W, paif_stream_t stream);
diff --git a/paif_amd/_lib.py b/paif_amd/_lib.py
--- a/paif_amd/_lib.py
+++ b/paif_amd/_lib.py
@@ -15,7 +15,7 @@
         ("in_act", c_int), ("in_prelu", F), ("scale", F), ("shift", F), ("act", c_int), ("prelu", F),
         ("alpha", c_float), ("res", F * 3), ("out", F), ("cout", c_int), ("pool_partial", F),
         ("precision", c_int), ("aux_out", F), ("in_aux", F), ("in_scale", F), ("in_alpha", c_float), ("epi_aux", F),
-        ("epi_dact", c_int), ("reverse_tiles", c_int), ("storage", c_int), ("cpool", F),
+        ("epi_dact", c_int), ("reverse_tiles", c_int), ("storage", c_int), ("cpool", F), ("eca_sums", F), ("eca_gate", F),
     ]
 
 
@@ -44,6 +44,8 @@
     "paif_guided_filter_fused_fwd_hf16_y16": (c_int, [F, F, F, c_float, c_float, F, c_int, c_int, c_int, F]),
     "paif_conv2d_blocks": (c_int, [c_int, c_int, c_int]),
     "paif_conv2d_fwd": (c_int, [POINTER(ConvDesc), c_int, c_int, c_int, F]),
+    "paif_conv2d_eca_eligible": (c_int, [c_int, c_int, c_int]),
+    "paif_eca_gate_f16": (c_int, [F, F, F, F, F, c_int, F, c_int, c_int, c_int, F]),
     "paif_conv2d_is_persistent": (c_int, [POINTER(ConvDesc), c_int, c_int, c_int]),
     "paif_conv2d_can_cpool": (c_int, [POINTER(ConvDesc), c_int, c_int, c_int]),
     "paif_rdb_fused_wpk_floats": (c_size_t, []),
diff --git a/paif_amd/csrc/conv_dma.h b/paif_amd/csrc/conv_dma.h
--- a/paif_amd/csrc/conv_dma.h
+++ b/paif_amd/csrc/conv_dma.h
@@ -21,11 +21,21 @@
   int in_relu;
 };
 
+struct EcaArgs {
+  int eca;
+  const float* in_prelu;
+  float* eca_sums;
+  const float* eca_gate;
+};
+
 bool eligible(int nsrc, int nres, int B, int H, int W, float alpha);
 bool eligible16(int nsrc, int nres, int B, int H, int W, float alpha);
 bool eligible7(int nsrc, int nres, int B, int H, int W, float alpha);
 bool eligible_d2(int nsrc, int nres, int B, int H, int W, float alpha);
 bool can_cpool(int nsrc, int nres, int kh, int cout, int dil);
-int launch(const Args& a, hipStream_t st);
+bool eligible_eca(int B, int H, int W);
+int launch(const Args& a, hipStream_t st, const EcaArgs* e = nullptr);
+int launch_eca_gate(const float* sums, const void* r, const void* wpk, const float* prelu, const float* w1d, int k, float* gate, int B, int H,
+                    int W, hipStream_t st);
 
 }
diff --git a/paif_amd/csrc/conv_dma.hip b/paif_amd/csrc/conv_dma.hip
--- a/paif_amd/csrc/conv_dma.hip
+++ b/paif_amd/csrc/conv_dma.hip
@@ -45,6 +45,7 @@
 #define CD_VMWAIT(n) asm volatile("s_waitcnt vmcnt(%0)" ::"n"((n) > VMCAP ? VMCAP : (n)) : "memory")
 #define CD_RD128(dst, addr, off) asm volatile("ds_read_b128 %0, %1 offset:%2" : "=v"(dst) : "v"(addr), "n"(off) : "memory")
 #define CD_WR32(addr, val, off) asm volatile("ds_write_b32 %0, %1 offset:%2" ::"v"(addr), "v"(val), "n"(off) : "memory")
+#define CD_WR128(addr, val, off) asm volatile("ds_write_b128 %0, %1 offset:%2" ::"v"(addr), "v"(val), "n"(off) : "memory")
 
 __device__ __forceinline__ void dma16(__amdgpu_buffer_rsrc_t rsrc, unsigned voff, unsigned lds_off) {
   __builtin_amdgcn_raw_ptr_buffer_load_lds(rsrc, (__attribute__((address_space(3))) void*)(uintptr_t)lds_off, 16, voff, 0, 0, 0);
@@ -61,8 +62,10 @@
   static constexpr int n1 = DPW * (PF - 1);
 };
 
-template <int NSRC, int NRES, int F, bool CP = false, int DIL = 1, int IA = 0>
-__global__ __launch_bounds__(256, 1) void conv3x3_h16_dma(Args a, int ntiles, int tilesX, int tilesY) {
+template <int NSRC, int NRES, int F, bool CP, int EC, int DIL, int IA>
+__device__ __forceinline__ void conv3x3_body(const Args& a, const EcaArgs& e, int ntiles, int tilesX, int tilesY) {
+  static_assert(EC == 0 || (NSRC == 1 && DIL == 1 && F == 2 && !CP && NRES == (EC == 2 ? 1 : 0) && IA == (EC == 2 ? 1 : 0)),
+                "the ECA forms: fp16, one source, dilation 1; conv1 without residual maps, conv2 with one and the input PReLU");
   typedef Geo<DIL> G;
   constexpr int TWH = G::TWH, NPIX = G::NPIX, DPW = G::DPW, SLOT = G::SLOT, PF = G::PF, NSLOT = G::NSLOT, ROWB = G::ROWB, PARK_OFF = G::PARK_OFF;
   typedef Sched<NSRC, NRES, PF, DPW> SC;
@@ -110,6 +113,8 @@
   const __amdgpu_buffer_rsrc_t rs_out = __builtin_amdgcn_make_buffer_rsrc(a.out, 0, a.B * H * W * opitch, RSRC_W3);
   const __amdgpu_buffer_rsrc_t rs_null = __builtin_amdgcn_make_buffer_rsrc(a.out, 0, 0, RSRC_W3);
   const __amdgpu_buffer_rsrc_t rs_cp = __builtin_amdgcn_make_buffer_rsrc(CP ? (void*)a.cpool : a.out, 0, CP ? a.B * H * W * 16 - 8 : 0, RSRC_W3);
+  const __amdgpu_buffer_rsrc_t rs_eca = __builtin_amdgcn_make_buffer_rsrc(EC == 1 ? (void*)e.eca_sums : (EC == 2 ? (void*)e.eca_gate : a.out), 0,
+                                                                          EC == 1 ? a.B * tilesX * tilesY * 512 : (EC == 2 ? a.B * 128 : 0), RSRC_W3);
 
   u32x4 bw[NSRC][9][2];
   {
@@ -130,6 +135,7 @@
     esh[j] = ((a.shift && c < a.cout) ? a.shift[c] : 0.f) * a.alpha;
   }
   const float e_slope = a.act == 1 ? *a.prelu : (a.act == 2 ? 0.f : 1.f);
+  const float in_slope = (EC == 1 || IA == 1) ? *e.in_prelu : 0.f;
 
   int d_rel[DPW];
   int d_rc[DPW];
@@ -167,10 +173,16 @@
   const unsigned o_lane = 8 * (l & 3) < a.cout ? (unsigned)((l >> 2) * opitch + (l & 3) * 16) : OOB;
 
   u32x4 rr[U][NRES > 0 ? NRES : 1][4];
+  u32x4 gg[EC == 2 ? U : 1][2];
   auto issue_res = [&](auto settag, int k) {
     constexpr int SET = decltype(settag)::value;
     int b, y0, x0;
     const bool ok = tile_of(k, b, y0, x0);
+    if constexpr (EC == 2) {
+      const unsigned goff = ok ? (unsigned)((b * 32 + 8 * (l & 3)) * 4) : OOB;
+      gg[SET][0] = __builtin_amdgcn_raw_buffer_load_b128(rs_eca, goff, 0, 0);
+      gg[SET][1] = __builtin_amdgcn_raw_buffer_load_b128(rs_eca, goff, 16, 0);
+    }
 #pragma unroll
     for (int it = 0; it < 4; ++it) {
       const int y = y0 + wb + (it >> 1) * DIL, x = x0 + (it & 1) * 16 + (l >> 2);
@@ -192,12 +204,22 @@
   for (int it = 0; it < 4; ++it) t[it][0] = t[it][1] = u32x4{0, 0, 0, 0};
   float ev[8];
   float pmx = 0.f, psm = 0.f;
+  float esum[8];
+#pragma unroll
+  for (int j = 0; j < 8; ++j) esum[j] = 0.f;
   int cur = NSLOT - PF;
 
   auto epi = [&](auto mtag, auto settag, bool pok, int pb, int py0, int px0) {
     constexpr int M = decltype(mtag)::value, SETP = decltype(settag)::value;
     constexpr int it = M / 9, j = M % 9;
-    if constexpr (j < 8) {
+    if constexpr (j < 8 && EC == 2) {
+      const unsigned raw = j < 4 ? t[it][0][j & 3] : t[it][1][j & 3];
+      typedef _Float16 h16x8 __attribute__((ext_vector_type(8)));
+      typedef float f32x8 __attribute__((ext_vector_type(8)));
+      const float r = __builtin_convertvector(__builtin_bit_cast(h16x8, rr[SETP][0][it]), f32x8)[j];
+      const float v = __builtin_fmaf(__uint_as_float(raw), __uint_as_float(gg[SETP][j >> 2][j & 3]), r);
+      ev[j] = __builtin_fmaf(e_slope, fminf(v, 0.f), fmaxf(v, 0.f));
+    } else if constexpr (j < 8) {
       const unsigned raw = j < 4 ? t[it][0][j & 3] : t[it][1][j & 3];
       float v = __builtin_fmaf(__uint_as_float(raw), esc[j], esh[j]);
       v = __builtin_fmaf(e_slope, fminf(v, 0.f), fmaxf(v, 0.f));
@@ -208,6 +230,13 @@
         else v += __uint_as_float((j & 1) ? (u & 0xffff0000u) : (u << 16));
       }
       ev[j] = v;
+      if constexpr (EC == 1) {
+        const int y = py0 + wb + (it >> 1), x = px0 + (it & 1) * 16 + (l >> 2);
+        const float in = (pok && y < H && x < W) ? 1.f : 0.f;
+        const _Float16 h = (_Float16)v;
+        const _Float16 a16 = h >= (_Float16)0 ? h : (_Float16)(in_slope * (float)h);
+        esum[j] = __builtin_fmaf((float)a16, in, it == 0 ? 0.f : esum[j]);
+      }
       if constexpr (CP) {
         pmx = j == 0 ? v : fmaxf(pmx, v);
         psm = j == 0 ? v : psm + v;
@@ -233,6 +262,46 @@
     }
   };
 
+  auto eca_store = [&](bool pok, int pb, int py0, int px0) {
+    float sv[8];
+#pragma unroll
+    for (int j = 0; j < 8; ++j) {
+      float v = esum[j];
+      v += paif::dpp_f<0x128>(v);
+      v += paif::dpp_f<0x124>(v);
+      const auto s16 = __builtin_amdgcn_permlane16_swap(__float_as_uint(v), __float_as_uint(v), false, false);
+      v = __uint_as_float(s16[0]) + __uint_as_float(s16[1]);
+      const auto s32 = __builtin_amdgcn_permlane32_swap(__float_as_uint(v), __float_as_uint(v), false, false);
+      sv[j] = __uint_as_float(s32[0]) + __uint_as_float(s32[1]);
+    }
+    const unsigned soff = (unsigned)((((pb * tilesY + py0 / TH) * tilesX + px0 / TW) * 4 + w) * 128);
+    const unsigned loff = (pok && l < 4) ? (unsigned)l * 32u : OOB;
+    u32x4 s0 = {__float_as_uint(sv[0]), __float_as_uint(sv[1]), __float_as_uint(sv[2]), __float_as_uint(sv[3])};
+    u32x4 s1 = {__float_as_uint(sv[4]), __float_as_uint(sv[5]), __float_as_uint(sv[6]), __float_as_uint(sv[7])};
+    __builtin_amdgcn_raw_buffer_store_b128(s0, rs_eca, loff, soff, 0);
+    __builtin_amdgcn_raw_buffer_store_b128(s1, rs_eca, loff, soff + 16, 0);
+    asm volatile("s_nop 2" : "+v"(s0), "+v"(s1));
+  };
+  auto prelu_stage = [&](unsigned sb) {
+    static_assert(IA != 1 || DPW == 6, "the input PReLU is written for the dilation-1 stage (6 DMAs per wave)");
+    u32x4 c[DPW];
+#pragma unroll
+    for (int i = 0; i < DPW; ++i) CD_RD128(c[i], sb + (unsigned)((w * DPW + i) * 1024) + (unsigned)l * 16u, 0);
+    asm volatile("s_waitcnt lgkmcnt(0)" : "+v"(c[0]), "+v"(c[1]), "+v"(c[2]), "+v"(c[3]), "+v"(c[4]), "+v"(c[5]) ::"memory");
+    typedef _Float16 h16x8 __attribute__((ext_vector_type(8)));
+    typedef float f32x8 __attribute__((ext_vector_type(8)));
+    const f32x8 z = {0.f, 0.f, 0.f, 0.f, 0.f, 0.f, 0.f, 0.f};
+    const f32x8 sl = {in_slope, in_slope, in_slope, in_slope, in_slope, in_slope, in_slope, in_slope};
+#pragma unroll
+    for (int i = 0; i < DPW; ++i) {
+      const f32x8 x = __builtin_convertvector(__builtin_bit_cast(h16x8, c[i]), f32x8);
+      const f32x8 y = __builtin_elementwise_fma(sl, __builtin_elementwise_min(x, z), __builtin_elementwise_max(x, z));
+      const u32x4 o = __builtin_bit_cast(u32x4, __builtin_convertvector(y, h16x8));
+      CD_WR128(sb + (unsigned)((w * DPW + i) * 1024) + (unsigned)l * 16u, o, 0);
+    }
+    asm volatile("s_waitcnt lgkmcnt(0)" ::: "memory");
+  };
+
   auto stage = [&](auto ktag, auto stag, auto virt, int k) {
     constexpr int K = decltype(ktag)::value, S = decltype(stag)::value;
     constexpr bool VIRT = decltype(virt)::value;
@@ -243,6 +312,7 @@
     unsigned ad[3][2];
     if constexpr (!VIRT) {
       CD_VMWAIT(SC::n1);
+      if constexpr (IA == 1) prelu_stage(sb);
       asm volatile("s_barrier" ::: "memory");
 #pragma unroll
       for (int dx = 0; dx < 3; ++dx)
@@ -266,7 +336,7 @@
     if constexpr (VIRT) {
       if constexpr (S == 0) {
 #pragma unroll
-        for (int it = 0; it < NSTORE; ++it) __builtin_amdgcn_raw_buffer_store_b128(u32x4{0, 0, 0, 0}, rs_null, 0, 0, 0);
+        for (int it = 0; it < NSTORE + (EC == 1 ? 2 : 0); ++it) __builtin_amdgcn_raw_buffer_store_b128(u32x4{0, 0, 0, 0}, rs_null, 0, 0, 0);
       }
     } else {
       int pb = 0, py0 = 0, px0 = 0;
@@ -324,6 +394,7 @@
       group(std::integral_constant<int, 3>{});
       group(std::integral_constant<int, 4>{});
       group(std::integral_constant<int, 5>{});
+      if constexpr (EC == 1 && S == 0) eca_store(pok, pb, py0, px0);
       if constexpr (S == NSRC - 1) {
         asm volatile("s_nop 15\n\ts_nop 7" ::: "memory");
 #pragma unroll
@@ -353,6 +424,7 @@
     CD_M(12) CD_M(13) CD_M(14) CD_M(15) CD_M(16) CD_M(17) CD_M(18) CD_M(19) CD_M(20) CD_M(21) CD_M(22) CD_M(23)
     CD_M(24) CD_M(25) CD_M(26) CD_M(27) CD_M(28) CD_M(29) CD_M(30) CD_M(31) CD_M(32) CD_M(33) CD_M(34) CD_M(35)
 #undef CD_M
+    if constexpr (EC == 1) eca_store(pok, pb, py0, px0);
   };
 
   auto vstage = [&](auto jtag) {
@@ -390,6 +462,15 @@
     }
   }
   CD_VMWAIT(0);
+}
+
+template <int NSRC, int NRES, int F, bool CP = false, int DIL = 1, int IA = 0>
+__global__ __launch_bounds__(256, 1) void conv3x3_h16_dma(Args a, int ntiles, int tilesX, int tilesY) {
+  conv3x3_body<NSRC, NRES, F, CP, 0, DIL, IA>(a, EcaArgs{}, ntiles, tilesX, tilesY);
+}
+template <int NSRC, int NRES, int F, bool CP, int EC, int DIL, int IA>
+__global__ __launch_bounds__(256, 1) void conv3x3_h16_dma(Args a, EcaArgs e, int ntiles, int tilesX, int tilesY) {
+  conv3x3_body<NSRC, NRES, F, CP, EC, DIL, IA>(a, e, ntiles, tilesX, tilesY);
 }
 
 namespace k7 {
@@ -408,7 +489,6 @@
 static_assert(4 * DPW * 64 >= NPIX * 4, "7x7: DMA instructions do not cover the halo tile");
 }
 
-#define CD_WR128(addr, val, off) asm volatile("ds_write_b128 %0, %1 offset:%2" ::"v"(addr), "v"(val), "n"(off) : "memory")
 
 template <int F>
 __global__ __launch_bounds__(256, 1) void conv7x7_h16_dma(Args a, int ntiles, int tilesX, int tilesY) {
@@ -679,6 +759,154 @@
   return 0;
 }
 
+int launch_eca(const Args& a, const EcaArgs& ea, hipStream_t st) {
+  const int tilesX = (a.W + TW - 1) / TW, tilesY = (a.H + TH - 1) / TH;
+  if (ea.eca == 1) hipLaunchKernelGGL((conv3x3_h16_dma<1, 0, 2, false, 1, 1, 0>), dim3(256), dim3(256), 0, st, a, ea, a.B * tilesX * tilesY, tilesX, tilesY);
+  else hipLaunchKernelGGL((conv3x3_h16_dma<1, 1, 2, false, 2, 1, 1>), dim3(256), dim3(256), 0, st, a, ea, a.B * tilesX * tilesY, tilesX, tilesY);
+  hipError_t e = hipGetLastError();
+  if (e != hipSuccess) {
+    paif::set_error("conv2d(h16 dma, ECA): launch failed: %s", hipGetErrorString(e));
+    return (int)e;
+  }
+  return 0;
+}
+
+__global__ __launch_bounds__(1024) void eca_gate_kernel(const float4* __restrict__ sums, const unsigned short* __restrict__ r,
+                                                        const unsigned short* __restrict__ wpk, const float* __restrict__ prelu,
+                                                        const float* __restrict__ w1d, int k, int tiles_per_img, int H, int W, float inv_hw,
+                                                        float* __restrict__ gate) {
+  __shared__ float4 part[32][32];
+  __shared__ float bsum[4][64][33];
+  __shared__ float corner[4][32];
+  __shared__ float tot[5][32];
+  __shared__ float mpart[32][33];
+  __shared__ float mean[32];
+  const int b = blockIdx.x, tid = threadIdx.x;
+  const float slope = *prelu;
+  auto a16 = [&](unsigned short h) { return (float)(_Float16)paif::prelu_f((float)__builtin_bit_cast(_Float16, h), slope); };
+  const size_t img = (size_t)b * H * W;
+  {
+    const int q = tid & 31, pt = tid >> 5;
+    float4 acc = make_float4(0.f, 0.f, 0.f, 0.f);
+#pragma unroll 8
+    for (int t = pt; t < tiles_per_img; t += 32) {
+      const float4 v = sums[((size_t)b * tiles_per_img + t) * 32 + q];
+      acc.x += v.x; acc.y += v.y; acc.z += v.z; acc.w += v.w;
+    }
+    part[pt][q] = acc;
+  }
+  {
+    const int set = tid >> 8, q8 = tid & 3, i = (tid & 255) >> 2;
+    const int n = set < 2 ? W : H;
+    float acc[8] = {0.f, 0.f, 0.f, 0.f, 0.f, 0.f, 0.f, 0.f};
+#pragma unroll 4
+    for (int p = i; p < n; p += 64) {
+      const int y = set == 0 ? 0 : (set == 1 ? H - 1 : p), x = set < 2 ? p : (set == 2 ? 0 : W - 1);
+      const uint4 u = *reinterpret_cast<const uint4*>(r + (img + (size_t)y * W + x) * 32 + 8 * q8);
+      const unsigned uu[4] = {u.x, u.y, u.z, u.w};
+#pragma unroll
+      for (int d = 0; d < 4; ++d) {
+        acc[2 * d] += a16((unsigned short)(uu[d] & 0xffffu));
+        acc[2 * d + 1] += a16((unsigned short)(uu[d] >> 16));
+      }
+    }
+#pragma unroll
+    for (int j = 0; j < 8; ++j) bsum[set][i][8 * q8 + j] = acc[j];
+  }
+  if (tid < 128) {
+    const int ci = tid >> 5, c = tid & 31;
+    const int y = ci < 2 ? 0 : H - 1, x = (ci & 1) ? W - 1 : 0;
+    corner[ci][c] = a16(r[(img + (size_t)y * W + x) * 32 + c]);
+  }
+  __syncthreads();
+  __shared__ float4 part2[4][32];
+  __shared__ float bsum2[4][4][32];
+  if (tid < 128) {
+    const int q = tid & 31, g = tid >> 5;
+    float4 a = part[g * 8][q];
+#pragma unroll
+    for (int k2 = 1; k2 < 8; ++k2) {
+      const float4 v = part[g * 8 + k2][q];
+      a.x += v.x; a.y += v.y; a.z += v.z; a.w += v.w;
+    }
+    part2[g][q] = a;
+  } else if (tid < 640) {
+    const int u = tid - 128, set = u >> 7, g = (u >> 5) & 3, c = u & 31;
+    float a = 0.f;
+#pragma unroll
+    for (int i = 0; i < 16; ++i) a += bsum[set][g * 16 + i][c];
+    bsum2[set][g][c] = a;
+  }
+  __syncthreads();
+  if (tid < 32) {
+    const int c = tid;
+    float t = 0.f;
+#pragma unroll
+    for (int g = 0; g < 4; ++g)
+#pragma unroll
+      for (int wv = 0; wv < 4; ++wv) {
+        const float4 v = part2[g][wv * 8 + (c >> 2)];
+        t += (c & 3) == 0 ? v.x : ((c & 3) == 1 ? v.y : ((c & 3) == 2 ? v.z : v.w));
+      }
+    tot[0][c] = t;
+  } else if (tid < 160) {
+    const int set = (tid - 32) >> 5, c = tid & 31;
+    tot[1 + set][c] = ((bsum2[set][0][c] + bsum2[set][1][c]) + bsum2[set][2][c]) + bsum2[set][3][c];
+  }
+  __syncthreads();
+  {
+    const int co = tid & 31, c = tid >> 5;
+    const int hh = (c & 15) >> 3, ks = c >> 4, j = c & 7;
+    float m = 0.f;
+#pragma unroll
+    for (int tap = 0; tap < 9; ++tap) {
+      const int dy = tap / 3 - 1, dx = tap % 3 - 1;
+      float sv = tot[0][c];
+      if (dy == 1) sv -= tot[1][c];
+      if (dy == -1) sv -= tot[2][c];
+      if (dx == 1) sv -= tot[3][c];
+      if (dx == -1) sv -= tot[4][c];
+      if (dy != 0 && dx != 0) sv += corner[(dy == 1 ? 0 : 2) + (dx == 1 ? 0 : 1)][c];
+      const unsigned short wh = wpk[((tap * 2 + ks) * 2 + 0) * 512 + (co + 32 * hh) * 8 + j];
+      m = fmaf((float)__builtin_bit_cast(_Float16, wh), sv, m);
+    }
+    mpart[c][co] = m;
+  }
+  __syncthreads();
+  if (tid < 32) {
+    float m = 0.f;
+#pragma unroll
+    for (int c = 0; c < 32; ++c) m += mpart[c][tid];
+    mean[tid] = m * inv_hw;
+  }
+  __syncthreads();
+  if (tid < 32) {
+    const int c = tid;
+    float y = 0.f;
+    const int pad = (k - 1) / 2;
+    for (int j = 0; j < k; ++j) {
+      const int cc = c + j - pad;
+      if (cc >= 0 && cc < 32) y = fmaf(mean[cc], w1d[j], y);
+    }
+    gate[b * 32 + c] = 1.0f / (1.0f + expf(-y));
+  }
+}
+
+}
+
+bool eligible_eca(int B, int H, int W) { return eligible(1, 0, B, H, W, 1.f) && eligible(1, 1, B, H, W, 1.f); }
+
+int launch_eca_gate(const float* sums, const void* r, const void* wpk, const float* prelu, const float* w1d, int k, float* gate, int B, int H,
+                    int W, hipStream_t st) {
+  const int tiles = ((H + TH - 1) / TH) * ((W + TW - 1) / TW);
+  hipLaunchKernelGGL(eca_gate_kernel, dim3(B), dim3(1024), 0, st, reinterpret_cast<const float4*>(sums), reinterpret_cast<const unsigned short*>(r),
+                     reinterpret_cast<const unsigned short*>(wpk), prelu, w1d, k, tiles, H, W, 1.0f / ((float)H * (float)W), gate);
+  hipError_t e = hipGetLastError();
+  if (e != hipSuccess) {
+    paif::set_error("eca_gate: launch failed: %s", hipGetErrorString(e));
+    return (int)e;
+  }
+  return 0;
 }
 
 bool eligible(int nsrc, int nres, int B, int H, int W, float alpha) {
@@ -707,10 +935,22 @@
   return kh == 3 && cout == 32 && ((dil == 1 && nsrc == 3 && (nres == 1 || nres == 3)) || (dil == 2 && nsrc == 1 && (nres == 1 || nres == 3)));
 }
 
-int launch(const Args& a, hipStream_t st) {
+int launch(const Args& a, hipStream_t st, const EcaArgs* e) {
   if (a.cpool && !can_cpool(a.nsrc, a.nres, a.kh, a.cout, a.dil)) {
     paif::set_error("conv2d(dma): no fused ChannelPool for this form");
     return PAIF_ENOSUP;
+  }
+  if (e && e->eca) {
+    const bool ok = a.kh == 3 && a.dil == 1 && a.f16 && a.nsrc == 1 && a.cout == 32 && !a.cpool && !a.in_relu && e->in_prelu &&
+                    eligible_eca(a.B, a.H, a.W) &&
+                    ((e->eca == 1 && a.nres == 0 && e->eca_sums) ||
+                     (e->eca == 2 && a.nres == 1 && e->eca_gate && a.act == 1 && !a.scale && !a.shift && a.alpha == 1.f));
+    if (!ok) {
+      paif::set_error("conv2d(h16 dma): the ECA forms are fp16 3x3 dilation 1, one source: conv1 (sums) without residual maps, conv2 (gate) "
+                      "with one, output PReLU, no affine");
+      return PAIF_ENOSUP;
+    }
+    return launch_eca(a, *e, st);
   }
   if (a.kh == 7) return launch_7(a, st);
   if (a.dil == 2) {
diff --git a/paif_amd/csrc/conv_mfma.hip b/paif_amd/csrc/conv_mfma.hip
--- a/paif_amd/csrc/conv_mfma.hip
+++ b/paif_amd/csrc/conv_mfma.hip
@@ -44,6 +44,8 @@
   int reverse;
   int st;
   int wl0;
+  float* eca_sums;
+  const float* eca_gate;
 };
 
 template <bool HOOKS>
@@ -1470,7 +1472,9 @@
 
 enum ConvVariant { CV_PLAIN, CV_HOOKS, CV_WS, CV_RES, CV_MS, CV_DMA };
 static inline int res_count(const ConvArgs& a) { return a.res[0] ? (a.res[1] ? (a.res[2] ? 3 : 2) : 1) : 0; }
+static inline int eca_mode(const ConvArgs& a) { return a.eca_sums ? 1 : (a.eca_gate ? 2 : 0); }
 static inline ConvVariant bf16x3_variant(const ConvArgs& a, int kh, int dil) {
+  if (eca_mode(a)) return CV_DMA;
   if (needs_hooks(a)) return CV_HOOKS;
   if (dil == 1 && st_h16(a) && a.wl0 && a.in_act == 0 && !a.pool_partial &&
       ((kh == 3 && a.cout == 32 && paif_conv_dma::eligible(a.nsrc, res_count(a), a.B, a.H, a.W, a.alpha)) ||
@@ -1491,7 +1495,7 @@
 }
 
 static inline bool variant_can_cpool(const ConvArgs& a, int kh, int dil) {
-  if (a.cout != 32 || needs_hooks(a)) return false;
+  if (a.cout != 32 || needs_hooks(a) || eca_mode(a)) return false;
   if (bf16x3_variant(a, kh, dil) == CV_DMA) return paif_conv_dma::can_cpool(a.nsrc, res_count(a), kh, a.cout, dil);
   return true;
 }
@@ -1507,7 +1511,13 @@
       d.f16 = paif::st_f16(ST) ? 1 : 0;
       d.cpool = a.cpool;
       d.dil = DIL; d.in_relu = a.in_act == 2 ? 1 : 0;
-      return paif_conv_dma::launch(d, st);
+      paif_conv_dma::EcaArgs e{};
+      e.eca = eca_mode(a); e.in_prelu = a.in_prelu; e.eca_sums = a.eca_sums; e.eca_gate = a.eca_gate;
+      if (e.eca == 2 && a.in_act != 1) {
+        paif::set_error("conv2d(h16 dma): the gated ECA conv takes the input PReLU");
+        return PAIF_ENOSUP;
+      }
+      return paif_conv_dma::launch(d, st, &e);
     }
     case CV_HOOKS:
       if constexpr (ST == 0) return launch_bf16x3_h<KH, DIL, true>(a, st);
@@ -1797,6 +1807,15 @@
 
 int paif_conv2d_blocks(int B, int H, int W) { return B * ((H + TH - 1) / TH) * ((W + TW - 1) / TW); }
 
+int paif_conv2d_eca_eligible(int B, int H, int W) { return B > 0 && H > 0 && W > 0 && paif_conv_dma::eligible_eca(B, H, W) ? 1 : 0; }
+
+int paif_eca_gate_f16(const float* sums, const float* r, const float* wpk, const float* prelu, const float* w1d, int k, float* gate, int B, int H,
+                      int W, paif_stream_t stream) {
+  PAIF_REQUIRE(sums && r && wpk && prelu && w1d && gate && B > 0 && H > 0 && W > 0, PAIF_EINVAL, "eca_gate: bad arguments");
+  PAIF_REQUIRE(k >= 1 && k <= 9 && (k & 1), PAIF_ENOSUP, "eca_gate: k=%d", k);
+  return paif_conv_dma::launch_eca_gate(sums, r, wpk, prelu, w1d, k, gate, B, H, W, paif::as_stream(stream));
+}
+
 size_t paif_conv_wpk_floats(int nsrc, int cin, int kh) { return (size_t)nsrc * kh * kh * (cin / 8) * 256; }
 
 int paif_conv2d_is_persistent(const paif_conv_desc* d, int B, int H, int W) {
@@ -1821,6 +1840,7 @@
   a.B = B; a.H = H; a.W = W;
   a.nblk = B * ((W + TW - 1) / TW) * ((H + TH - 1) / TH);
   a.st = d->storage; a.wl0 = (d->precision == PAIF_CONV_BF16 || d->precision == PAIF_CONV_F16) ? 1 : 0; a.alpha = d->alpha;
+  a.eca_sums = d->eca_sums; a.eca_gate = d->eca_gate;
   return variant_can_cpool(a, d->kh, d->dil) ? 1 : 0;
 }
 
@@ -1833,6 +1853,7 @@
   a.B = B; a.H = H; a.W = W;
   a.nblk = B * ((W + TW - 1) / TW) * ((H + TH - 1) / TH);
   a.st = d->storage; a.wl0 = (d->precision == PAIF_CONV_BF16 || d->precision == PAIF_CONV_F16) ? 1 : 0; a.alpha = d->alpha;
+  a.eca_sums = d->eca_sums; a.eca_gate = d->eca_gate;
   const int code = kernel_st(a);
   if (d->precision == PAIF_CONV_BF16X6 && d->cin == 32) {
     snprintf(buf, buflen, "conv_mfma_bf16x6<%d, %d, %s, 0>", d->kh, d->dil, needs_hooks(a) ? "true" : "false");
@@ -1853,6 +1874,8 @@
   switch (bf16x3_variant(a, d->kh, d->dil)) {
     case CV_DMA:
       if (d->kh == 7) snprintf(buf, buflen, "conv7x7_h16_dma<%d>", a.st >= 3 ? 2 : 1);
+      else if (eca_mode(a)) snprintf(buf, buflen, "conv3x3_h16_dma<%d, %d, %d, false, %d, %d, %d>", d->nsrc, res_count(a), a.st >= 3 ? 2 : 1, eca_mode(a),
+                                     d->dil, eca_mode(a) == 2 ? 1 : 0);
       else snprintf(buf, buflen, "conv3x3_h16_dma<%d, %d, %d, %s, %d, %d>", d->nsrc, res_count(a), a.st >= 3 ? 2 : 1, d->cpool ? "true" : "false",
                     d->dil, d->dil == 2 ? 2 : 0);
       break;
@@ -1884,6 +1907,11 @@
   a.nsrc = d->nsrc; a.in_act = d->in_act; a.act = d->act; a.cout = d->cout;
   a.aux_out = d->aux_out; a.in_aux = d->in_aux; a.in_scale = d->in_scale; a.in_alpha = d->in_alpha;
   a.epi_aux = d->epi_aux; a.epi_dact = d->epi_dact;
+  a.eca_sums = d->eca_sums; a.eca_gate = d->eca_gate;
+  PAIF_REQUIRE(!(d->eca_sums && d->eca_gate), PAIF_EINVAL, "conv2d: eca_sums and eca_gate belong to different convs");
+  PAIF_REQUIRE(!(d->eca_sums || d->eca_gate) || (d->precision == PAIF_CONV_F16 && d->storage == PAIF_ST_F16 && d->kh == 3 && d->dil == 1 &&
+                                                 d->cin == 32 && d->in_prelu && paif_conv_dma::eligible_eca(B, H, W)),
+               PAIF_ENOSUP, "conv2d: the ECA forms take fp16 maps, a 3x3 dilation-1 conv and an LDS-DMA-eligible shape (paif_conv2d_eca_eligible)");
   PAIF_REQUIRE(d->in_act >= 0 && d->in_act <= 5, PAIF_EINVAL, "conv2d: in_act=%d", d->in_act);
   PAIF_REQUIRE(!(d->in_act == 3 || d->in_act == 4) || (d->in_aux && d->nsrc == 1), PAIF_EINVAL,
                "conv2d: in_act=%d needs in_aux and a single source", d->in_act);
diff --git a/paif_amd/operations_m.py b/paif_amd/operations_m.py
--- a/paif_amd/operations_m.py
+++ b/paif_amd/operations_m.py
@@ -490,6 +490,8 @@
     def forward_nhwc(self, x, res=(), tape=None):
         a = self.relu.weight
         w1 = self._packs.get("w1", [self.conv1.weight], lambda: ops.pack_conv_weight(self.conv1.weight, 1, 32, 3))
+        if tape is None and ops.eca_two_pass_eligible(x, self.k):
+            return self._add_res(ops.eca_block_f16(x, w1, self.conv2.wpk(1, 32), a, self.se.conv.weight, self.k), res)
         r = ops.conv2d([x], w1, 3, 1)
         o, partial = ops.conv2d([r], self.conv2.wpk(1, 32), self.k, 1, in_act=ops.ACT_PRELU, in_prelu=a, pool=True)
         if tape is None:
diff --git a/paif_amd/ops.py b/paif_amd/ops.py
--- a/paif_amd/ops.py
+++ b/paif_amd/ops.py
@@ -694,7 +694,7 @@
 
 def conv2d(srcs, wpk, kh, dil=1, cin=32, cout=32, in_act=ACT_NONE, in_prelu=None, scale=None, shift=None,
            act=ACT_NONE, prelu=None, alpha=1.0, res=(), pool=False, want_aux=False, in_aux=None, in_scale=None,
-           in_alpha=1.0, epi_dact=0, epi_aux=None, out=None, out_f32=False, cpool=None):
+           in_alpha=1.0, epi_dact=0, epi_aux=None, out=None, out_f32=False, cpool=None, eca_sums=None, eca_gate=None):
     B, H, W, C = srcs[0].shape
     assert C == cin and 1 <= len(srcs) <= 3
     res = [r for r in res if r is not None]
@@ -757,6 +757,7 @@
     aux = torch.empty_like(out) if want_aux else None
     d.aux_out, d.in_aux, d.in_scale, d.in_alpha = _p(aux), _p(in_aux), _p(in_scale), in_alpha
     d.epi_aux, d.epi_dact = _p(epi_aux), epi_dact
+    d.eca_sums, d.eca_gate = _p(eca_sums), _p(eca_gate)
     pool_after = None
     if cpool is not None:
         comp, coff = cpool
@@ -858,6 +859,31 @@
     return (out, u, gate) if save else out
 
 
+def eca_two_pass_eligible(x, k):
+    B, H, W, _ = x.shape
+    return x.dtype == torch.float16 and k == 3 and bool(lib().paif_conv2d_eca_eligible(B, H, W))
+
+
+def eca_gate_f16(r, sums, wpk2, prelu, w1d, k):
+    B, H, W, _ = r.shape
+    gate = torch.empty((B, 32), device=r.device, dtype=torch.float32)
+    tag = "eca_gate_kernel"
+    e0 = TIMER.start(tag) if TIMER is not None else None
+    _lib.check(lib().paif_eca_gate_f16(_p(sums), _pa(r), _p(wpk2.data), _p(prelu), _p(w1d.detach().contiguous()), k, _p(gate), B, H, W, _stream()),
+               "eca_gate")
+    if e0 is not None:
+        TIMER.stop(tag, e0, 0, sums.numel() * 4 + 2 * (2 * W + 2 * H) * 64)
+    return gate
+
+
+def eca_block_f16(x, w1, wpk2, prelu, w1d, k):
+    B, H, W, _ = x.shape
+    sums = torch.empty((lib().paif_conv2d_blocks(B, H, W), 4, 32), device=x.device, dtype=torch.float32)
+    r = conv2d([x], w1, 3, 1, in_prelu=prelu, eca_sums=sums)
+    gate = eca_gate_f16(r, sums, wpk2, prelu, w1d, k)
+    return conv2d([r], wpk2, 3, 1, in_act=ACT_PRELU, in_prelu=prelu, act=ACT_PRELU, prelu=prelu, res=(r,), eca_gate=gate)
+
+
 def eca_layer_fwd(x, w1d, k):
     B, H, W, C = x.shape
     assert C == 32 and x.dtype == torch.float32
```

New measurement: 2539, median of 6. +3.3%, better.
